# cslab-ntua/sparsex

Hardware: NVIDIA B200
Metric: csx_spmv_gflops (higher is better)
Workload: dtype f64

## Files before the change

### __graft_entry__.py

```python
import os
import subprocess
import sys

ROOT = os.path.dirname(os.path.abspath(__file__))
if ROOT not in sys.path:
    sys.path.insert(0, ROOT)


def build():
    csrc = os.path.join(ROOT, "sparsex_b200", "csrc")
    subprocess.check_call(["make", "-C", csrc, "-j4"])
    subprocess.check_call(["make", "-C", os.path.join(ROOT, "oracle"), "libcsx_oracle.so"])
    if os.path.isdir("/root/reference"):
        for script in ("build_ref.py", "build_refenc.py"):
            ref = os.path.join(ROOT, "oracle", script)
            if os.path.exists(ref):
                subprocess.check_call([sys.executable, ref])
    subprocess.check_call(["make", "-s", "-C", os.path.join(ROOT, "tests", "emul")], stderr=subprocess.DEVNULL)
    subprocess.check_call(["make", "-s", "-C", os.path.join(ROOT, "tests", "emul"), "-f", "trans.mk"], stderr=subprocess.DEVNULL)
    import sparsex_b200
    sparsex_b200.lib()
    if os.path.isdir("/root/reference/src/examples"):
        from tests.test_reference_examples import build_examples, build_test_program
        build_examples()
        build_test_program()


def smoke():
    import numpy as np
    import torch
    import sparsex_b200
    from oracle.pyoracle import OracleMatrix
    from tests.matrices import poisson2d

    assert torch.cuda.is_available(), "smoke() needs a GPU"
    rowptr, colind, values, n = poisson2d(96)
    rng = np.random.default_rng(0)
    x = rng.uniform(-1, 1, n)
    for opts in ({}, {"spx.preproc.xform": "none"}, {"spx.matrix.symmetric": "true"}):
        A = sparsex_b200.CsxMatrix.tune_csr(rowptr, colind, values, n, n, opts).upload(0)
        O = OracleMatrix.from_csr(rowptr, colind, values, n, n).tune(opts)
        for p in range(A.nparts):
            assert np.array_equal(A.partition(p).ctl, O.parts[p].ctl), "ctl mismatch vs oracle"
        dx = torch.from_numpy(x).cuda()
        dy = torch.empty(n, dtype=torch.float64, device="cuda")
        A.spmv(0.5, dx, dy)
        torch.cuda.synchronize()
        yref = O.spmv(0.5, x)
        err = np.abs(dy.cpu().numpy() - yref).max() / np.abs(yref).max()
        assert err < 1e-12, err
        print("smoke ok", opts, "rel err %.2e" % err)


if __name__ == "__main__":
    build()
    if len(sys.argv) > 1 and sys.argv[1] == "smoke":
        smoke()
```

### include/csx_b200.h

```cpp
#ifndef CSX_B200_H
#define CSX_B200_H

#include <stddef.h>
#include <stdint.h>

#ifdef __cplusplus
extern "C" {
#endif

typedef struct csxb_matrix csxb_matrix_t;

csxb_matrix_t *csxb_tune_csr(const int32_t *rowptr, const int32_t *colind, const double *values,
                             int64_t nrows, int64_t ncols, const char *options,
                             int part_lo, int part_hi, char *err, size_t errlen);
csxb_matrix_t *csxb_tune_mmf(const char *path, const char *options, int part_lo, int part_hi,
                             char *err, size_t errlen);
csxb_matrix_t *csxb_tune_csr_slab(const int32_t *rowptr, const int32_t *colind, const double *values,
                                  int64_t slab_rows, int64_t nrows_total, int64_t ncols, int64_t row_start,
                                  int part, const char *options, char *err, size_t errlen);
void csxb_destroy(csxb_matrix_t *m);

enum { CSXB_NROWS = 0, CSXB_NCOLS = 1, CSXB_NNZ = 2, CSXB_SYMMETRIC = 3, CSXB_NPARTS = 4,
       CSXB_NPARTS_TOTAL = 5, CSXB_PART_LO = 6, CSXB_FULL_COLIND = 7,
       CSXB_SYM_HALO_LO = 8, CSXB_SYM_HALO_HI = 9,
       CSXB_HOST_CAP = 10, CSXB_HOST_CALLS = 11,
       CSXB_DEVICE = 12  };
int64_t csxb_info(const csxb_matrix_t *m, int what);

enum { CSXB_P_NNZ = 0, CSXB_P_NROWS = 1, CSXB_P_NCOLS = 2, CSXB_P_ROW_START = 3, CSXB_P_CTL_SIZE = 4,
       CSXB_P_ROW_JUMPS = 5, CSXB_P_ID_MAP_LEN = 6, CSXB_P_MAP_LEN = 7, CSXB_P_DVALUES_LEN = 8,
       CSXB_P_ROWS_INFO_LEN = 9, CSXB_P_SAMPLING_UNDEFINED = 10,
       CSXB_P_COL_MIN = 11, CSXB_P_COL_MAX = 12  };
int64_t csxb_part_info(const csxb_matrix_t *m, int part, int what);
enum { CSXB_A_VALUES = 0, CSXB_A_CTL = 1, CSXB_A_ID_MAP = 2, CSXB_A_ROWS_INFO = 3, CSXB_A_DVALUES = 4,
       CSXB_A_MAP_CPUS = 5, CSXB_A_MAP_POS = 6 };
int csxb_part_copy(const csxb_matrix_t *m, int part, int what, void *dst);
const char *csxb_part_log(const csxb_matrix_t *m, int part);

int csxb_upload(csxb_matrix_t *m, int device, int free_host);
const char *csxb_last_error(void);
int csxb_layout_stats(csxb_matrix_t *m, int64_t *out, int max_owners);

enum { CSXB_B_VALUES = 0, CSXB_B_CTL = 1, CSXB_B_TABLES = 2, CSXB_B_X = 3, CSXB_B_Y = 4, CSXB_B_TOTAL = 5,
       CSXB_B_LAUNCHES = 6  };
int64_t csxb_traffic(const csxb_matrix_t *m, int what);

int csxb_spmv(csxb_matrix_t *m, double alpha, const double *d_x, double beta, double *d_y,
              int overwrite, void *stream);

int csxb_spmv_host(csxb_matrix_t *m, double alpha, const double *h_x, double beta, double *h_y,
                   int overwrite);

enum { CSXB_T_COL_LO = 0, CSXB_T_COL_HI = 1, CSXB_T_DEVICE_BYTES = 2, CSXB_T_ALG_BYTES = 3, CSXB_T_LAUNCHES = 4,
       CSXB_T_HEAVY_COLS = 5, CSXB_T_SEGMENTS = 6, CSXB_T_BUILD_US = 7 };
int csxb_transpose_prepare(csxb_matrix_t *m);
int csxb_spmv_t(csxb_matrix_t *m, double alpha, const double *d_x, double beta, double *d_y, int overwrite,
                void *stream);
int csxb_spmv_t_host(csxb_matrix_t *m, double alpha, const double *h_x, double beta, double *h_y, int overwrite);
int64_t csxb_transpose_info(const csxb_matrix_t *m, int what);
int csxb_decode_coords_t(const csxb_matrix_t *m, int32_t *rows, int32_t *cols);

int csxb_save(csxb_matrix_t *m, const char *path);
csxb_matrix_t *csxb_load(const char *path, char *err, size_t errlen);
int csxb_get_entry(csxb_matrix_t *m, int64_t row, int64_t col, double *value);
int csxb_set_entry(csxb_matrix_t *m, int64_t row, int64_t col, double value);

typedef struct csxb_group csxb_group_t;
csxb_group_t *csxb_group_create(csxb_matrix_t *whole, const int *devices, int ndev, int free_host, char *err, size_t errlen);
void csxb_group_destroy(csxb_group_t *g);
int csxb_group_size(const csxb_group_t *g);
csxb_matrix_t *csxb_group_member(csxb_group_t *g, int i);
int csxb_group_device(const csxb_group_t *g, int i);
int csxb_group_spmv(csxb_group_t *g, double alpha, const double *x, double beta, double *y, int overwrite);
int csxb_group_spmv_t(csxb_group_t *g, double alpha, const double *x, double beta, double *y, int overwrite);
int csxb_group_save(csxb_group_t *g, const char *path);
int csxb_group_get_entry(csxb_group_t *g, int64_t row, int64_t col, double *value);
int csxb_group_set_entry(csxb_group_t *g, int64_t row, int64_t col, double value);
int csxb_group_set_perm(csxb_group_t *g, const int32_t *perm, int64_t n);

int csxb_rcm_csr(const int32_t *rowptr, const int32_t *colind, int64_t nrows, int64_t ncols, int32_t *perm,
                 int64_t *bandwidth);
int csxb_rcm_edges(const int32_t *eu, const int32_t *ev, int64_t nedges, int64_t n, int64_t start, int32_t *perm,
                   int64_t *bandwidth);
int csxb_set_perm(csxb_matrix_t *m, const int32_t *perm, int64_t n);
int64_t csxb_get_perm(const csxb_matrix_t *m, int32_t *perm);
int csxb_permute_csr(const int32_t *rowptr, const int32_t *colind, const double *values, int64_t nrows,
                     const int32_t *perm, int32_t *out_rowptr, int32_t *out_colind, double *out_values);

int csxb_vec_axpby(double *d_out, const double *d_a, const double *d_b, double alpha, double beta, int64_t n, void *stream);
int csxb_vec_dot(const double *d_a, const double *d_b, int64_t n, double *result, void *stream);

typedef struct csxb_xchg csxb_xchg_t;
csxb_xchg_t *csxb_xchg_create(csxb_matrix_t *m, int rank, int world);
int csxb_xchg_handle(csxb_xchg_t *x, void *handle64);
int csxb_xchg_connect(csxb_xchg_t *x, const void *handles, const int64_t *row_lo, const int64_t *row_n,
                      const int64_t *win_lo, const int64_t *win_hi);
int csxb_xchg_connect_ptr(csxb_xchg_t *x, void *const *bases, const int64_t *row_lo, const int64_t *row_n,
                          const int64_t *win_lo, const int64_t *win_hi);
void *csxb_xchg_base(csxb_xchg_t *x);
double *csxb_xchg_vector(csxb_xchg_t *x, int which);
int csxb_xchg_spmv(csxb_xchg_t *x, double alpha, void *stream);
int64_t csxb_xchg_status(csxb_xchg_t *x, int what);
void csxb_xchg_destroy(csxb_xchg_t *x);

int csxb_decode_coords(const csxb_matrix_t *m, int part, int32_t *rows, int32_t *cols);

#ifdef __cplusplus
}
#endif
#endif
```

### sparsex_b200/csrc/engine.cu

```cuda
#include <cuda_runtime.h>

#include <chrono>
#include <memory>

#include <climits>
#include <cstdio>
#include <cstdlib>
#include <cstring>
#include <sstream>
#include <string>
#include <type_traits>
#include <vector>

#include "../../include/csx_b200.h"
#include "csx_host.hpp"
#include "gpu_layout.hpp"
#include "part_dev.cuh"
#include "stream_kernel.cuh"

#include "gather_kernel.cuh"

__device__ __forceinline__ unsigned long long ld_acquire_sys(const unsigned long long *p) {
  unsigned long long v;
  asm volatile("ld.acquire.sys.global.u64 %0, [%1];" : "=l"(v) : "l"(p) : "memory");
// ... 97 lines not shown
}
__global__ void csx_xchg_sync_kernel(const __grid_constant__ XchgDev X, int dbg) {
  const int lane = threadIdx.x;
  const unsigned long long k = *reinterpret_cast<const volatile unsigned long long *>(X.step);
  if (!(dbg & 2)) __threadfence_system();
  if (lane < X.nwait) st_release_sys(X.peer_flags[lane] + X.rank, k + 1);
  if (lane == 0) *reinterpret_cast<volatile unsigned long long *>(X.step) = k + 1;
  if (lane < X.nwait) {
    const unsigned long long *f = X.flags + X.wait_rank[lane];
    const long long t0 = clock64();
    while (ld_acquire_sys(f) < k + 1) {
      if (clock64() - t0 > 6000000000ll) { atomicExch(X.error, 1ull); break; }
    }
  }
}

struct DecodeGatherOp {
  int *rows, *cols;
  int myrow;
  __device__ __forceinline__ void add(uint32_t vi, int col) { rows[vi] = myrow; cols[vi] = col; }
};
__global__ void __launch_bounds__(CTA_THREADS) csx_decode_bt_kernel(const __grid_constant__ PartDev P, int *rows, int *cols) {
  const long long lrow = (long long)blockIdx.x * CTA_THREADS + threadIdx.x;
  if (lrow >= P.nrows) return;
  const long long g = P.row_start + lrow;
  for (int c = 0; c < P.nbt; c++) {
    const BtDev &T = P.bt[c];
    if (T.image) continue;
    const long long J = g / T.G;
    const int f = (int)(g - J * T.G) * T.sf;
    for (uint32_t e = T.ptr[J - T.j0]; e < T.ptr[J - T.j0 + 1]; e++) {
      const uint2 b = T.ent[e];
      if (b.y & BT_IMAGE) continue;
      for (int l = 0; l < T.nloop; l++) { rows[b.x + f + l * T.sl] = (int)g; cols[b.x + f + l * T.sl] = (int)b.y + l; }
    }
  }
}
__global__ void __launch_bounds__(CTA_THREADS) csx_decode_gather_kernel(const __grid_constant__ PartDev P, int *rows, int *cols) {
  const long long tile = blockIdx.x;
  const uint32_t b = __ldg(P.tile_xoff + tile), e = __ldg(P.tile_xoff + tile + 1);
  for (int k = 0; k < P.rpt; k++) {
    const long long lrow = (tile * P.rpt + k) * CTA_THREADS + threadIdx.x;
    if (lrow >= P.nrows) return;
    DecodeGatherOp op{rows, cols, (int)(P.row_start + lrow)};
    for (uint32_t j = b; j < e; j++) {
      const uint4 d = __ldg(P.xdesc + j);
      if (d.w & XD_TRANSPOSED) continue;
      gather_desc<false>(d, P.ktab, op.myrow, op);
    }
  }
}

__device__ __forceinline__ int sk_vectors(const SkIO &io, const double *&x, double *&y) {
  x = io.x; y = io.y;
  if (io.step) {
    const unsigned long long k = *reinterpret_cast<const volatile unsigned long long *>(io.step);
    x = io.vec[k & 1]; y = io.vec[(k & 1) ^ 1];
    return (int)((k & 1) ^ 1);
  }
  return 0;
}
template <int R, uint32_t KM, int BC, int BRC>
__global__ void __launch_bounds__(SK_WARPS * 32, 4) csx_stream_kernel(const __grid_constant__ PartDev P, const __grid_constant__ SkIO io,
                                                                     double alpha, double beta, int overwrite) {
  __shared__ double sacc[SK_WARPS][SK_WIN];
  __shared__ uint4 sid[64];
  const int lane = threadIdx.x & 31, warp = threadIdx.x >> 5;
  if (threadIdx.x < 64) {
    const IdEntry &ie = P.idtab[threadIdx.x];
    sid[threadIdx.x] = make_uint4(ie.kind_align, ie.delta, ie.sl, ie.recip);
  }
  __syncthreads();
  const uint32_t ch = P.sk_c0 + blockIdx.x * SK_WARPS + warp;
  if (ch >= P.sk_c1) return;
  const double *x; double *y;
  const int ypar = sk_vectors(io, x, y);
  sk_chunk<R, KM, BC, BRC, false>(P, ch, sacc[warp], sid, lane, x, y, alpha, beta, overwrite, nullptr, nullptr, &io, ypar);
}
__global__ void __launch_bounds__(SK_WARPS * 32) csx_stream_decode_kernel(const __grid_constant__ PartDev P, int *rows, int *cols) {
  __shared__ double sacc[SK_WARPS][SK_WIN];
  __shared__ uint4 sid[64];
  const int lane = threadIdx.x & 31, warp = threadIdx.x >> 5;
  if (threadIdx.x < 64) {
    const IdEntry &ie = P.idtab[threadIdx.x];
    sid[threadIdx.x] = make_uint4(ie.kind_align, ie.delta, ie.sl, ie.recip);
  }
  __syncthreads();
  const uint32_t ch = P.sk_c0 + blockIdx.x * SK_WARPS + warp;
  if (ch >= P.sk_c1) return;
  sk_chunk<8, SKM_ROWLOCAL | SKM_BROW | SKM_BCOL, 0, 0, true>(P, ch, sacc[warp], sid, lane, nullptr, nullptr, 0.0, 0.0, 1,
                                                               rows + P.val_base, cols + P.val_base);
}
__global__ void __launch_bounds__(256) csx_stream_fixup_kernel(const __grid_constant__ PartDev P, const __grid_constant__ SkIO io,
                                                                double alpha, double beta, int overwrite, long long clip_lo,
                                                                long long clip_hi) {
  const double *x; double *y;
  const int ypar = sk_vectors(io, x, y);
  const long long tid = (long long)blockIdx.x * blockDim.x + threadIdx.x, nth = (long long)gridDim.x * blockDim.x;
  for (long long i = P.sk_f0 + tid; i < P.sk_f1; i += nth) {
    double s = 0.0;
    for (uint32_t j = P.sk_fix_ptr[i]; j < P.sk_fix_ptr[i + 1]; j++) s += P.sk_scratch[P.sk_fix_idx[j]];
    const long long g = P.row_start + P.sk_fix_rows[i];
    const double v = y[g] + alpha * s;
    y[g] = v;
    sk_push(io, ypar, g, v);
  }
  for (uint32_t g = P.sk_g0 + blockIdx.x; g < P.sk_g1; g += gridDim.x) {
    const long long lo = max(P.sk_gaps[2 * g], clip_lo), hi = min(P.sk_gaps[2 * g + 1], clip_hi);
    for (long long r = lo + threadIdx.x; r < hi; r += blockDim.x) {
      double *yp = y + P.row_start + r;
      const double v = overwrite ? 0.0 : beta * *yp;
      *yp = v;
      sk_push(io, ypar, P.row_start + r, v);
    }
  }
}

__global__ void __launch_bounds__(256) csx_t_segment_kernel(const uint2 *__restrict__ ent, const uint32_t *__restrict__ seg,
                                                            uint32_t nseg, const double *__restrict__ values,
                                                            const double *__restrict__ x, double *__restrict__ scratch) {
  const uint32_t s = blockIdx.x * 8 + (threadIdx.x >> 5);
  if (s >= nseg) return;
  t_segment_warp(ent, seg, values, x, scratch, s, (int)(threadIdx.x & 31));
}

static thread_local std::string g_last_error;
static int fail(const std::string &m) { g_last_error = m; return -1; }
#define CUDA_TRY(call)                                                                         \
  do {                                                                                         \
    cudaError_t e_ = (call);                                                                   \
    if (e_ != cudaSuccess)                                                                     \
      return fail(std::string(#call) + ": " + cudaGetErrorString(e_));                         \
  } while (0)

struct TransState {
  TransLayout lay;
  PartDev P;
  const uint2 *hent = nullptr;
  const uint32_t *hseg = nullptr;
  int64_t dev_bytes = 0, alg_bytes = 0, launches = 0, build_us = 0;
  double *d_x = nullptr, *d_y = nullptr;
};

struct csxb_matrix {
  CsxMatrix host;
  DeviceLayout layout;
  bool uploaded = false;
  int device = -1;
  std::vector<void *> allocs;
  std::vector<PartDev> pdev;
  double *d_values = nullptr;
  double *d_x = nullptr, *d_y = nullptr;
  int64_t covered_rows_end = 0;
  int64_t sym_halo_lo = 0, sym_halo_hi = 0;
  struct Slab {
    int part; int64_t tile0, tile1;
    uint32_t chunk0, chunk1, f0, f1, g0, g1;
    int64_t x_lo, x_hi, row_lo, row_hi, y_lo, y_hi, yup_hi;
  };
  std::vector<Slab> slabs;
  std::vector<cudaEvent_t> slab_ev;
  cudaStream_t s_h2d = nullptr, s_run = nullptr, s_d2h = nullptr;
  int host_calls = 0;
  double host_tune_s[2] = {0.0, 0.0};
  size_t host_cap = 0;
  int64_t bytes[7] = {0, 0, 0, 0, 0, 0, 0};
  std::vector<std::string> logs;
  std::vector<RowIndex> row_index;
  std::unique_ptr<TransState> trans;
  ~csxb_matrix() {
    if (!allocs.empty() || d_x || d_y || s_h2d) {
      int cur = -1;
      cudaGetDevice(&cur);
      if (device >= 0) cudaSetDevice(device);
      for (void *p : allocs) cudaFree(p);
      if (d_x) cudaFree(d_x);
      if (d_y) cudaFree(d_y);
      for (cudaEvent_t e : slab_ev) cudaEventDestroy(e);
      if (s_h2d) { cudaStreamDestroy(s_h2d); cudaStreamDestroy(s_run); cudaStreamDestroy(s_d2h); }
      if (cur >= 0) cudaSetDevice(cur);
    }
  }
};

static std::string parse_options(const char *options, TuneOptions &o) {
  if (!options) return "";
  std::stringstream ss(options);
  std::string kv;
  while (std::getline(ss, kv, ';')) {
    if (kv.empty()) continue;
    size_t eq = kv.find('=');
    if (eq == std::string::npos) return "malformed option \"" + kv + "\"";
    std::string e = o.set(kv.substr(0, eq), kv.substr(eq + 1));
    if (!e.empty()) return e;
  }
  return "";
}
static void put_err(char *err, size_t n, const std::string &m) {
  g_last_error = m;
  if (err && n) { strncpy(err, m.c_str(), n - 1); err[n - 1] = 0; }
}

csxb_matrix_t *csxb_tune_coo_internal(const CooHost &coo, const char *options, int part_lo, int part_hi, char *err, size_t errlen) {
  TuneOptions o;
  std::string e = parse_options(options, o);
  if (!e.empty()) { put_err(err, errlen, e); return nullptr; }
  if (part_hi < 0) { part_lo = 0; part_hi = o.nr_threads; }
  csxb_matrix *m = new csxb_matrix;
  e = tune_coo(coo, o, part_lo, part_hi, m->host);
  if (!e.empty()) { put_err(err, errlen, e); delete m; return nullptr; }
  return m;
}

extern "C" {

csxb_matrix_t *csxb_tune_csr(const int32_t *rowptr, const int32_t *colind, const double *values, int64_t nrows,
                             int64_t ncols, const char *options, int part_lo, int part_hi, char *err, size_t errlen) {
  TuneOptions o;
  std::string e = parse_options(options, o);
  if (e.empty() && (!rowptr || !colind || !values || nrows < 0 || ncols < 0)) e = "invalid CSR arguments";
  if (e.empty() && rowptr[0] != 0) e = "CSR arrays must be zero-based";
  if (!e.empty()) { put_err(err, errlen, e); return nullptr; }
  if (part_hi < 0) { part_lo = 0; part_hi = o.nr_threads; }
  csxb_matrix *m = new csxb_matrix;
  CsrView v{rowptr, colind, values, nrows, ncols};
  e = tune_csr(v, o, part_lo, part_hi, m->host);
  if (!e.empty()) { put_err(err, errlen, e); delete m; return nullptr; }
  return m;
}

csxb_matrix_t *csxb_tune_csr_slab(const int32_t *rowptr, const int32_t *colind, const double *values, int64_t slab_rows,
                                  int64_t nrows_total, int64_t ncols, int64_t row_start, int part, const char *options, char *err,
                                  size_t errlen) {
  TuneOptions o;
  std::string e = parse_options(options, o);
  if (e.empty() && (!rowptr || !colind || !values || slab_rows < 0 || ncols < 0)) e = "invalid CSR arguments";
  if (e.empty() && rowptr[0] != 0) e = "CSR arrays must be zero-based";
  if (!e.empty()) { put_err(err, errlen, e); return nullptr; }
  csxb_matrix *m = new csxb_matrix;
  CsrView v{rowptr, colind, values, slab_rows, ncols};
  e = tune_csr_slab(v, nrows_total, row_start, part, o, m->host);
  if (!e.empty()) { put_err(err, errlen, e); delete m; return nullptr; }
  return m;
}

csxb_matrix_t *csxb_tune_mmf(const char *path, const char *options, int part_lo, int part_hi, char *err, size_t errlen) {
  TuneOptions o;
  std::string e = parse_options(options, o);
  CooHost coo;
  if (e.empty()) e = path ? read_mmf(path, coo) : "invalid file name";
  if (!e.empty()) { put_err(err, errlen, e); return nullptr; }
  if (part_hi < 0) { part_lo = 0; part_hi = o.nr_threads; }
  csxb_matrix *m = new csxb_matrix;
  e = tune_coo(coo, o, part_lo, part_hi, m->host);
  if (!e.empty()) { put_err(err, errlen, e); delete m; return nullptr; }
  return m;
}

void csxb_destroy(csxb_matrix_t *m) { delete m; }

int64_t csxb_info(const csxb_matrix_t *m, int what) {
  switch (what) {
    case CSXB_NROWS: return m->host.nrows;
    case CSXB_NCOLS: return m->host.ncols;
    case CSXB_NNZ: return m->host.nnz;
    case CSXB_SYMMETRIC: return m->host.symmetric;
    case CSXB_NPARTS: return (int64_t)m->host.parts.size();
    case CSXB_NPARTS_TOTAL: return m->host.nparts_total;
    case CSXB_PART_LO: return m->host.part_lo;
    case CSXB_FULL_COLIND: return m->host.full_colind;
    case CSXB_SYM_HALO_LO: return m->sym_halo_lo;
    case CSXB_SYM_HALO_HI: return m->sym_halo_hi;
    case CSXB_HOST_CAP: return (int64_t)m->host_cap;
    case CSXB_HOST_CALLS: return m->host_calls;
    case CSXB_DEVICE: return m->uploaded ? m->device : -1;
  }
  return -1;
}

int64_t csxb_part_info(const csxb_matrix_t *m, int part, int what) {
  if (part < 0 || (size_t)part >= m->host.parts.size()) return -1;
  const CsxPartition &p = m->host.parts[part];
  switch (what) {
    case CSXB_P_NNZ: return p.nnz;
    case CSXB_P_NROWS: return p.nrows;
    case CSXB_P_NCOLS: return p.ncols;
    case CSXB_P_ROW_START: return p.row_start;
    case CSXB_P_CTL_SIZE: return (int64_t)p.ctl.size();
    case CSXB_P_ROW_JUMPS: return p.row_jumps;
    case CSXB_P_ID_MAP_LEN: return (int64_t)p.id_map.size();
    case CSXB_P_MAP_LEN: return (int64_t)p.map_cpus.size();
    case CSXB_P_DVALUES_LEN: return (int64_t)p.dvalues.size();
    case CSXB_P_ROWS_INFO_LEN: return (int64_t)p.rows_info.size();
    case CSXB_P_SAMPLING_UNDEFINED: return p.sampling_undefined;
    case CSXB_P_COL_MIN: return p.col_min;
    case CSXB_P_COL_MAX: return p.col_max;
  }
  return -1;
}

int csxb_part_copy(const csxb_matrix_t *m, int part, int what, void *dst) {
  if (part < 0 || (size_t)part >= m->host.parts.size() || !dst) return fail("invalid argument");
  const CsxPartition &p = m->host.parts[part];
  switch (what) {
    case CSXB_A_VALUES:
      if (p.values.size() != (size_t)p.nnz) return fail("host values were released at upload");
      memcpy(dst, p.values.data(), p.values.size() * 8); break;
    case CSXB_A_CTL: memcpy(dst, p.ctl.data(), p.ctl.size()); break;
    case CSXB_A_ID_MAP: { int64_t *d = (int64_t *)dst; for (size_t i = 0; i < p.id_map.size(); i++) d[i] = p.id_map[i]; break; }
    case CSXB_A_ROWS_INFO: {
      struct R { int64_t rowptr, valptr; int32_t span, pad; } *d = (R *)dst;
      for (size_t i = 0; i < p.rows_info.size(); i++) d[i] = R{p.rows_info[i].rowptr, p.rows_info[i].valptr, p.rows_info[i].span, 0};
      break;
    }
    case CSXB_A_DVALUES: memcpy(dst, p.dvalues.data(), p.dvalues.size() * 8); break;
    case CSXB_A_MAP_CPUS: memcpy(dst, p.map_cpus.data(), p.map_cpus.size() * 4); break;
    case CSXB_A_MAP_POS: memcpy(dst, p.map_pos.data(), p.map_pos.size() * 4); break;
    default: return fail("unknown array");
  }
  return 0;
}

const char *csxb_part_log(const csxb_matrix_t *m, int part) {
  if (part < 0 || (size_t)part >= m->host.parts.size()) return "";
  return m->host.parts[part].encoding_log.c_str();
}

const char *csxb_last_error(void) { return g_last_error.c_str(); }

int csxb_layout_stats(csxb_matrix_t *m, int64_t *out, int max_owners) {
  CsxMatrix &H = m->host;
  std::vector<int64_t> saved;
  for (auto &p : H.parts) { saved.push_back(p.nrows); if (H.symmetric) p.nrows = (int64_t)p.dvalues.size(); }
  DeviceLayout L;
  std::string e = build_layout(H, L);
  for (size_t i = 0; i < H.parts.size(); i++) H.parts[i].nrows = saved[i];
  if (!e.empty()) return fail("layout: " + e);
  for (size_t q = 0; q < L.parts.size() && (int)q < max_owners; q++) {
    const PartLayout &pl = L.parts[q];
    int64_t *o = out + 12 * q;
    o[0] = pl.nrows; o[1] = pl.ntiles; o[2] = (int64_t)pl.xdesc.size(); o[3] = (int64_t)pl.sk_chunks.size();
    o[4] = (int64_t)pl.sk_uoffs.size(); o[5] = (int64_t)pl.sk_fix_idx.size(); o[6] = (int64_t)pl.sk_gaps.size();
    for (int t = 0; t < 5; t++) o[7 + t] = 0;
    for (const BlockTable &T : pl.bt) {
      int t = T.G == 1 && T.nloop == 1 ? 4 : (T.image ? (T.sl == 1 ? 3 : 1) : (T.sl == 1 ? 0 : 2));
      o[7 + t] += (int64_t)T.ent.size();
    }
  }
  return (int)L.parts.size();
}

}

template <class T>
static int dev_copy(csxb_matrix *m, const T *src, size_t n, T **dst, size_t extra_zero = 0) {
  void *p = nullptr;
  size_t bytes = (n + extra_zero) * sizeof(T);
  CUDA_TRY(cudaMalloc(&p, bytes ? bytes : 16));
  m->allocs.push_back(p);
  if (n) CUDA_TRY(cudaMemcpy(p, src, n * sizeof(T), cudaMemcpyHostToDevice));
  if (extra_zero) CUDA_TRY(cudaMemset((char *)p + n * sizeof(T), 0, extra_zero * sizeof(T)));
  *dst = (T *)p;
  return 0;
}

static void build_slabs(csxb_matrix *m) {
  m->slabs.clear();
  int64_t SLAB_ROWS = m->host.slab_rows;
  if (SLAB_ROWS <= 0) {
    int64_t total_rows = 0;
    for (const PartLayout &pl : m->layout.parts) if (pl.ntiles) total_rows += pl.nrows;
    SLAB_ROWS = int64_t(1) << 19;
    while (SLAB_ROWS < (int64_t(1) << 21) && SLAB_ROWS * 16 <= total_rows) SLAB_ROWS *= 2;
  }
  for (size_t i = 0; i < m->layout.parts.size(); i++) {
    const PartLayout &pl = m->layout.parts[i];
    if (!pl.ntiles) continue;
    const int64_t tr = pl.tile_rows();
    const int64_t tiles_per = std::max<int64_t>(1, SLAB_ROWS / tr);
    uint32_t c = 0, f = 0;
    const uint32_t nc = (uint32_t)pl.sk_chunks.size(), nf = (uint32_t)pl.sk_fix_rows.size(), ng = (uint32_t)pl.sk_gaps.size();
    int64_t xmax = -1, yup = 0;
    for (int64_t t0 = 0; t0 < pl.ntiles; t0 += tiles_per) {
      csxb_matrix::Slab sl;
      sl.part = (int)i; sl.tile0 = t0; sl.tile1 = std::min(pl.ntiles, t0 + tiles_per);
      const int64_t r0 = t0 * tr, r1 = std::min(pl.nrows, sl.tile1 * tr);
      sl.row_lo = pl.row_start + r0; sl.row_hi = pl.row_start + r1;
      for (int64_t t = sl.tile0; t < sl.tile1; t++)
        if (pl.tile_cmax[t] >= pl.tile_cmin[t]) xmax = std::max<int64_t>(xmax, pl.tile_cmax[t]);
      sl.chunk0 = c;
      while (c < nc && pl.sk_first_row[c] < r1) {
        xmax = std::max<int64_t>(xmax, pl.sk_cmax[c]);
        yup = std::max<int64_t>(yup, (int64_t)pl.sk_last_row[c] + 1);
        c++;
      }
      sl.chunk1 = c;
      sl.f0 = f;
      while (f < nf && pl.sk_fix_rows[f] < r1) f++;
      sl.f1 = f;
      sl.g0 = 0;
      while (sl.g0 < ng && pl.sk_gaps[sl.g0].hi <= r0) sl.g0++;
      sl.g1 = sl.g0;
      while (sl.g1 < ng && pl.sk_gaps[sl.g1].lo < r1) sl.g1++;
      sl.x_lo = 0; sl.x_hi = xmax + 1;
      sl.y_lo = sl.row_lo; sl.y_hi = sl.row_hi;
      sl.yup_hi = pl.row_start + std::max(r1, std::min(yup, pl.nrows));
      m->slabs.push_back(sl);
    }
  }
  int64_t lo = INT64_MAX;
  for (size_t i = 0; i < m->layout.parts.size(); i++)
    for (int32_t v : m->layout.parts[i].tile_cmin) if (v != INT32_MAX) lo = std::min<int64_t>(lo, v);
  if (lo == INT64_MAX) lo = 0;
  int64_t run = lo;
  for (auto &sl : m->slabs) { sl.x_lo = lo; run = std::max(run, sl.x_hi); sl.x_hi = run; }
}

extern "C" {

int csxb_upload(csxb_matrix_t *m, int device, int free_host) {
  if (m->uploaded) return fail("matrix already uploaded");
  CsxMatrix &H = m->host;
  std::vector<int64_t> saved_nrows;
  for (auto &p : H.parts) { saved_nrows.push_back(p.nrows); if (H.symmetric) p.nrows = (int64_t)p.dvalues.size(); }
  std::string e = build_layout(H, m->layout);
  for (size_t i = 0; i < H.parts.size(); i++) H.parts[i].nrows = saved_nrows[i];
  if (!e.empty()) return fail("layout: " + e);
  int ndev = 0;
  CUDA_TRY(cudaGetDeviceCount(&ndev));
  if (device < 0 || device >= ndev) return fail("invalid device");
  CUDA_TRY(cudaSetDevice(device));
  m->device = device;
  DeviceLayout &L = m->layout;
  void *dv = nullptr, *dc = nullptr;
  CUDA_TRY(cudaMalloc(&dv, std::max<uint64_t>(L.total_values, 1) * 8));
  m->allocs.push_back(dv);
  CUDA_TRY(cudaMalloc(&dc, std::max<uint64_t>(L.total_ctl, 16)));
  m->allocs.push_back(dc);
  CUDA_TRY(cudaMemset(dc, 0, std::max<uint64_t>(L.total_ctl, 16)));
  m->d_values = (double *)dv;
  KindEntry *d_ktab = nullptr;
  if (dev_copy(m, L.ktab.data(), L.ktab.size(), &d_ktab)) return -1;
  int64_t tables = (int64_t)L.ktab.size() * 8, nnz_stored = 0, ctl_bytes = 0, rows_owned = 0, launches = 0;
  m->pdev.resize(L.parts.size());
  for (size_t i = 0; i < L.parts.size(); i++) {
    PartLayout &pl = L.parts[i];
    static CsxPartition no_part;
    CsxPartition &hp = pl.is_halo ? no_part : H.parts[i];
    PartDev &P = m->pdev[i];
    memset(&P, 0, sizeof(P));
    if (hp.nnz) CUDA_TRY(cudaMemcpy(m->d_values + pl.val_base, hp.values.data(), (size_t)hp.nnz * 8, cudaMemcpyHostToDevice));
    if (!hp.ctl.empty()) CUDA_TRY(cudaMemcpy((uint8_t *)dc + pl.ctl_base, hp.ctl.data(), hp.ctl.size(), cudaMemcpyHostToDevice));
    P.ctl = (const uint8_t *)dc + pl.ctl_base;
    P.values = m->d_values;
    P.ctl_end = (const uint8_t *)dc + std::max<uint64_t>(L.total_ctl, 16);
    P.values_end = m->d_values + std::max<uint64_t>(L.total_values, 1);
    uint32_t *tx = nullptr; XDesc *xd = nullptr;
    if (dev_copy(m, pl.tile_xoff.data(), pl.tile_xoff.size(), &tx)) return -1;
    if (dev_copy(m, pl.xdesc.data(), pl.xdesc.size(), &xd)) return -1;
    for (size_t t = 0; t < pl.bt.size(); t++) {
      const BlockTable &T = pl.bt[t];
      uint32_t *bp = nullptr; BlockImage *bi = nullptr;
      if (dev_copy(m, T.ptr.data(), T.ptr.size(), &bp)) return -1;
      if (dev_copy(m, T.ent.data(), T.ent.size(), &bi)) return -1;
      static_assert(sizeof(BlockImage) == sizeof(uint2), "block table entry layout");
      P.bt[t] = BtDev{bp, (const uint2 *)bi, (long long)T.j0, T.G, T.nloop, T.sf, T.sl, T.image, (uint32_t)((0x100000000ull + T.G - 1) / T.G)};
      tables += (int64_t)T.ptr.size() * 4 + (int64_t)T.ent.size() * 8;
    }
    P.nbt = (int)pl.bt.size();
    if (!pl.sk_chunks.empty()) {
      SkEntry *se = nullptr; uint16_t *so = nullptr; int32_t *fr = nullptr; uint32_t *fp = nullptr, *fi = nullptr; long long *gp = nullptr;
      if (dev_copy(m, pl.sk_chunks.data(), pl.sk_chunks.size(), &se)) return -1;
      if (dev_copy(m, pl.sk_uoffs.data(), pl.sk_uoffs.size(), &so)) return -1;
      if (dev_copy(m, pl.sk_fix_rows.data(), pl.sk_fix_rows.size(), &fr)) return -1;
      if (dev_copy(m, pl.sk_fix_ptr.data(), pl.sk_fix_ptr.size(), &fp)) return -1;
      if (dev_copy(m, pl.sk_fix_idx.data(), pl.sk_fix_idx.size(), &fi)) return -1;
      static_assert(sizeof(SkGap) == 16, "gap layout");
      if (dev_copy(m, reinterpret_cast<const long long *>(pl.sk_gaps.data()), pl.sk_gaps.size() * 2, &gp)) return -1;
      void *sc = nullptr;
      CUDA_TRY(cudaMalloc(&sc, std::max<size_t>(pl.sk_scratch, 2) * 8));
      m->allocs.push_back(sc);
      P.sk_chunks = (const uint4 *)se; P.sk_uoffs = so; P.sk_scratch = (double *)sc;
      P.sk_fix_rows = fr; P.sk_fix_ptr = fp; P.sk_fix_idx = fi; P.sk_gaps = gp;
      P.sk_c0 = 0; P.sk_c1 = (uint32_t)pl.sk_chunks.size();
      P.sk_f0 = 0; P.sk_f1 = (uint32_t)pl.sk_fix_rows.size();
      P.sk_g0 = 0; P.sk_g1 = (uint32_t)pl.sk_gaps.size();
      tables += (int64_t)pl.sk_chunks.size() * (int64_t)sizeof(SkEntry) + (int64_t)pl.sk_uoffs.size() * 2 +
                (int64_t)pl.sk_fix_rows.size() * 8 + (int64_t)pl.sk_fix_idx.size() * 4 + (int64_t)pl.sk_scratch * 16;
    }
    P.tile_xoff = tx; P.xdesc = (const uint4 *)xd; P.ktab = d_ktab;
    if (H.symmetric && !pl.is_halo) {
      double *dd = nullptr;
      if (dev_copy(m, hp.dvalues.data(), hp.dvalues.size(), &dd)) return -1;
      P.dvalues = dd;
      tables += (int64_t)hp.dvalues.size() * 8;
    }
    P.nrows = pl.nrows; P.row_start = pl.row_start; P.val_base = (uint32_t)pl.val_base;
    P.full_colind = L.full_colind;
    P.rpt = pl.rpt;
    memcpy(P.idtab, pl.idtab, sizeof(P.idtab));
    nnz_stored += hp.nnz; rows_owned += pl.nrows;
    if (!pl.sk_chunks.empty()) ctl_bytes += (int64_t)hp.ctl.size();
    tables += (int64_t)pl.tile_xoff.size() * 4 + (int64_t)pl.xdesc.size() * 16;
    if (pl.nrows) {
      if (!pl.sk_chunks.empty())
        launches += 1 + ((pl.sk_fix_rows.empty() && pl.sk_gaps.empty()) ? 0 : 1) + ((pl.xdesc.empty() && pl.bt.empty() && !H.symmetric) ? 0 : 1);
      else launches += 1;
    }
    if (!pl.is_halo) m->covered_rows_end = std::max<int64_t>(m->covered_rows_end, pl.row_start + pl.nrows);
    if (free_host && !pl.is_halo) std::vector<double>().swap(hp.values);
  }
  m->sym_halo_lo = L.halo_lo; m->sym_halo_hi = L.halo_hi;
  if (!H.symmetric) build_slabs(m);
  m->bytes[CSXB_B_VALUES] = nnz_stored * 8;
  m->bytes[CSXB_B_CTL] = ctl_bytes;
  m->bytes[CSXB_B_TABLES] = tables;
  int64_t cmin = H.ncols, cmax = -1;
  for (auto &p : H.parts) if (p.col_max >= p.col_min) { cmin = std::min(cmin, p.col_min); cmax = std::max(cmax, p.col_max); }
  int64_t xcols = (int)H.parts.size() == H.nparts_total ? H.ncols : std::max<int64_t>(0, cmax - cmin + 1);
  if (H.symmetric) xcols = H.ncols;
  m->bytes[CSXB_B_X] = xcols * 8;
  m->bytes[CSXB_B_Y] = rows_owned * 8;
  m->bytes[CSXB_B_TOTAL] = nnz_stored * 8 + ctl_bytes + tables + xcols * 8 + rows_owned * 8;
  m->bytes[CSXB_B_LAUNCHES] = launches;
  m->uploaded = true;
  return 0;
}

int64_t csxb_traffic(const csxb_matrix_t *m, int what) {
  if (what < 0 || what > CSXB_B_LAUNCHES) return -1;
  return m->bytes[what];
}

}

static bool gather_cache_policies(const PartLayout &pl) {
  static const int forced = getenv("CSXB_GATHER_POLICY") ? atoi(getenv("CSXB_GATHER_POLICY")) : -1;
  return forced >= 0 ? forced != 0 : pl.nnz >= 12 * pl.nrows;
}

template <int RPT> struct BtMinB { static constexpr int value = RPT == 1 ? 6 : 5; };
static thread_local size_t t_gather_dyn = 0;
constexpr size_t HOST_CAP_SMEM = 40000;
template <class K>
static size_t gather_dyn(K kernel) {
  if (t_gather_dyn > 48 * 1024) cudaFuncSetAttribute(kernel, cudaFuncAttributeMaxDynamicSharedMemorySize, (int)t_gather_dyn);
  return t_gather_dyn;
}
template <bool SYM, int RPT, int KSET, class XP>
static void launch_gather_k(const PartDev &P, const PartLayout &pl, unsigned nt, const double *x, double *y, double alpha,
                            double beta, int overwrite, cudaStream_t s, const XP &X) {
  dim3 grid(nt), block(CTA_THREADS);
  if (!pl.bt.empty()) {
    if (!pl.xdesc.empty()) {
      auto k = csx_spmv_kernel<true, SYM, RPT, KSET_ANY, BtMinB<RPT>::value, 0, XP, true>;
      k<<<grid, block, gather_dyn(k), s>>>(P, x, y, alpha, beta, overwrite, X);
    } else {
      auto k = csx_spmv_kernel<false, SYM, RPT, KSET_ANY, BtMinB<RPT>::value, 0, XP, true>;
      k<<<grid, block, gather_dyn(k), s>>>(P, x, y, alpha, beta, overwrite, X);
    }
    return;
  }
  constexpr int MB = SYM ? 4 : 8;
  const size_t dyn = 0;
  if (!pl.xdesc.empty()) csx_spmv_kernel<true, SYM, RPT, KSET, MB, 0, XP><<<grid, block, dyn, s>>>(P, x, y, alpha, beta, overwrite, X);
  else csx_spmv_kernel<false, SYM, RPT, KSET_ANY, MB, 0, XP><<<grid, block, dyn, s>>>(P, x, y, alpha, beta, overwrite, X);
}
template <bool SYM, class XP>
static void launch_gather(const PartDev &P0, const PartLayout &pl, int64_t t0, int64_t t1, const double *x, double *y,
                          double alpha, double beta, int overwrite, cudaStream_t s, const XP &X) {
  if (t1 <= t0) return;
  PartDev P = P0;
  P.tile0 = (uint32_t)t0;
  const unsigned nt = (unsigned)(t1 - t0);
  const bool diag1 = !SYM && pl.xd_diag1_only && !pl.xdesc.empty() && pl.bt.empty();
  if (pl.rpt == 4) {
    if (diag1) {
      dim3 grid(nt), block(CTA_THREADS);
      if (gather_cache_policies(pl)) {
        auto k = csx_spmv_kernel<true, false, 4, KSET_DIAG1, 8, 3, XP>;
        k<<<grid, block, gather_dyn(k), s>>>(P, x, y, alpha, beta, overwrite, X);
      } else {
        auto k = csx_spmv_kernel<true, false, 4, KSET_DIAG1, 8, 1, XP>;
        k<<<grid, block, gather_dyn(k), s>>>(P, x, y, alpha, beta, overwrite, X);
      }
    }
    else launch_gather_k<SYM, 4, KSET_ANY>(P, pl, nt, x, y, alpha, beta, overwrite, s, X);
  } else {
    if (diag1) launch_gather_k<SYM, 1, SYM ? KSET_ANY : KSET_DIAG1>(P, pl, nt, x, y, alpha, beta, overwrite, s, X);
    else launch_gather_k<SYM, 1, KSET_ANY>(P, pl, nt, x, y, alpha, beta, overwrite, s, X);
  }
}
static void launch_gather_xe(const PartDev &P0, const PartLayout &pl, const double *x, double *y, double alpha, int ypar,
                             cudaStream_t s, const XchgDev &X) {
  if (!pl.ntiles) return;
  PartDev P = P0;
  P.tile0 = 0;
  dim3 grid((unsigned)(X.nb + (X.edge_hi_begin - X.edge_lo_end))), block(CTA_THREADS);
  const bool xd = !pl.xdesc.empty(), diag1 = pl.xd_diag1_only && xd && pl.bt.empty();
  if (!pl.bt.empty()) {
    if (pl.rpt == 4) {
      if (xd) csx_spmv_xe_kernel<true, 4, KSET_ANY, BtMinB<4>::value, 0, true><<<grid, block, 0, s>>>(P, x, y, alpha, ypar, X);
      else csx_spmv_xe_kernel<false, 4, KSET_ANY, BtMinB<4>::value, 0, true><<<grid, block, 0, s>>>(P, x, y, alpha, ypar, X);
    } else {
      if (xd) csx_spmv_xe_kernel<true, 1, KSET_ANY, BtMinB<1>::value, 0, true><<<grid, block, 0, s>>>(P, x, y, alpha, ypar, X);
      else csx_spmv_xe_kernel<false, 1, KSET_ANY, BtMinB<1>::value, 0, true><<<grid, block, 0, s>>>(P, x, y, alpha, ypar, X);
    }
    return;
  }
  const size_t dyn = 0;
  if (pl.rpt == 4) {
    if (diag1 && gather_cache_policies(pl)) csx_spmv_xe_kernel<true, 4, KSET_DIAG1, 8, 3><<<grid, block, dyn, s>>>(P, x, y, alpha, ypar, X);
    else if (diag1) csx_spmv_xe_kernel<true, 4, KSET_DIAG1, 8, 1><<<grid, block, dyn, s>>>(P, x, y, alpha, ypar, X);
    else if (xd) csx_spmv_xe_kernel<true, 4, KSET_ANY><<<grid, block, dyn, s>>>(P, x, y, alpha, ypar, X);
    else csx_spmv_xe_kernel<false, 4, KSET_ANY><<<grid, block, dyn, s>>>(P, x, y, alpha, ypar, X);
  } else {
    if (diag1) csx_spmv_xe_kernel<true, 1, KSET_DIAG1><<<grid, block, dyn, s>>>(P, x, y, alpha, ypar, X);
    else if (xd) csx_spmv_xe_kernel<true, 1, KSET_ANY><<<grid, block, dyn, s>>>(P, x, y, alpha, ypar, X);
    else csx_spmv_xe_kernel<false, 1, KSET_ANY><<<grid, block, dyn, s>>>(P, x, y, alpha, ypar, X);
  }
}
static int launch_stream(const PartDev &P0, const PartLayout &pl, uint32_t c0, uint32_t c1, const SkIO &io, double alpha, double beta,
                         int overwrite, cudaStream_t s) {
  if (c1 <= c0) return 0;
  PartDev P = P0;
  P.sk_c0 = c0; P.sk_c1 = c1;
  const unsigned grid = (unsigned)((c1 - c0 + SK_WARPS - 1) / SK_WARPS);
#define SK_TRY(RR, KK, BCC, BRR)                                                                                         \
  if (sk_instance_serves(RR, (KK), BCC, BRR, pl.sk_kmask, pl.sk_rows, pl.sk_bc, pl.sk_brc)) {                            \
    csx_stream_kernel<RR, (KK), BCC, BRR><<<grid, SK_WARPS * 32, 0, s>>>(P, io, alpha, beta, overwrite);                 \
    return 0;                                                                                                            \
  }
  SK_INSTANCES(SK_TRY)
#undef SK_TRY
  return -1;
}
static void launch_fixup(const PartDev &P0, uint32_t f0, uint32_t f1, uint32_t g0, uint32_t g1, int64_t r0, int64_t r1, const SkIO &io,
                         double alpha, double beta, int overwrite, cudaStream_t s) {
  if (f1 <= f0 && g1 <= g0) return;
  PartDev P = P0;
  P.sk_f0 = f0; P.sk_f1 = f1; P.sk_g0 = g0; P.sk_g1 = g1;
  const int64_t ctas = std::max<int64_t>(((int64_t)(f1 - f0) + 255) / 256, (int64_t)(g1 - g0));
  const unsigned grid = (unsigned)std::min<int64_t>(148 * 8, ctas);
  csx_stream_fixup_kernel<<<grid, 256, 0, s>>>(P, io, alpha, beta, overwrite, (long long)r0, (long long)r1);
}
template <bool SYM, class XP>
static int run_partition(const PartDev &P, const PartLayout &pl, const SkIO &io, double alpha, double beta, int overwrite,
                         cudaStream_t s, const XP &X) {
  if (pl.sk_chunks.empty()) {
    launch_gather<SYM>(P, pl, 0, pl.ntiles, io.x, io.y, alpha, beta, overwrite, s, X);
    return 0;
  }
  if (launch_stream(P, pl, 0, (uint32_t)pl.sk_chunks.size(), io, alpha, beta, overwrite, s)) return -1;
  launch_fixup(P, 0, (uint32_t)pl.sk_fix_rows.size(), 0, (uint32_t)pl.sk_gaps.size(), 0, pl.nrows, io, alpha, beta, overwrite, s);
  if (SYM || !pl.xdesc.empty() || !pl.bt.empty()) launch_gather<SYM>(P, pl, 0, pl.ntiles, io.x, io.y, alpha, 1.0, 0, s, X);
  return 0;
}

extern "C" {

static int on_matrix_device(const csxb_matrix *m) {
  int cur = -1;
  if (cudaGetDevice(&cur) != cudaSuccess) return fail("cudaGetDevice failed");
  if (cur != m->device && cudaSetDevice(m->device) != cudaSuccess) return fail("cudaSetDevice failed");
  return 0;
}

int csxb_spmv(csxb_matrix_t *m, double alpha, const double *d_x, double beta, double *d_y, int overwrite, void *stream) {
  if (!m->uploaded) return fail("matrix not uploaded (csxb_upload)");
  if (on_matrix_device(m)) return -1;
  cudaStream_t s = (cudaStream_t)stream;
  const bool sym = m->host.symmetric;
  SkIO io;
  io.x = d_x; io.y = d_y; io.step = nullptr; io.vec[0] = io.vec[1] = nullptr; io.npush = 0;
  for (size_t i = 0; i < m->pdev.size(); i++) {
    const PartLayout &pl = m->layout.parts[i];
    int rc;
    if (pl.is_halo) { launch_gather<true>(m->pdev[i], pl, 0, pl.ntiles, d_x, d_y, alpha, 0.0, 1, s, NoXchg()); rc = 0; }
    else if (sym) rc = run_partition<true>(m->pdev[i], pl, io, alpha, beta, overwrite, s, NoXchg());
    else rc = run_partition<false>(m->pdev[i], pl, io, alpha, beta, overwrite, s, NoXchg());
    if (rc) return fail("no stream kernel for the partition's pattern set");
  }
  if (overwrite && m->host.part_lo + (int)m->host.parts.size() == m->host.nparts_total && m->covered_rows_end < m->host.nrows)
    CUDA_TRY(cudaMemsetAsync(d_y + m->covered_rows_end, 0, (size_t)(m->host.nrows - m->covered_rows_end) * 8, s));
  CUDA_TRY(cudaGetLastError());
  return 0;
}

int csxb_spmv_host(csxb_matrix_t *m, double alpha, const double *h_x, double beta, double *h_y, int overwrite) {
  if (!m->uploaded) return fail("matrix not uploaded (csxb_upload)");
  int cur = -1;
  CUDA_TRY(cudaGetDevice(&cur));
  if (cur != m->device) CUDA_TRY(cudaSetDevice(m->device));
  size_t nx = (size_t)std::max<int64_t>(m->host.ncols, 1), ny = (size_t)std::max<int64_t>(m->host.nrows, 1);
  if (!m->d_x) CUDA_TRY(cudaMalloc((void **)&m->d_x, nx * 8));
  if (!m->d_y) CUDA_TRY(cudaMalloc((void **)&m->d_y, ny * 8));
  if (!m->s_h2d) {
    CUDA_TRY(cudaStreamCreateWithFlags(&m->s_h2d, cudaStreamNonBlocking));
    CUDA_TRY(cudaStreamCreateWithFlags(&m->s_run, cudaStreamNonBlocking));
    CUDA_TRY(cudaStreamCreateWithFlags(&m->s_d2h, cudaStreamNonBlocking));
  }
  const bool last_local = m->host.part_lo + (int)m->host.parts.size() == m->host.nparts_total;
  if (m->slabs.empty()) {
    CUDA_TRY(cudaMemcpyAsync(m->d_x, h_x, (size_t)m->host.ncols * 8, cudaMemcpyHostToDevice, m->s_run));
    if (!overwrite) CUDA_TRY(cudaMemcpyAsync(m->d_y, h_y, (size_t)m->host.nrows * 8, cudaMemcpyHostToDevice, m->s_run));
    if (csxb_spmv(m, alpha, m->d_x, beta, m->d_y, overwrite, m->s_run)) return -1;
    int64_t lo = m->layout.parts.empty() ? 0 : m->layout.parts.front().row_start;
    int64_t hi = last_local ? m->host.nrows : m->covered_rows_end;
    if (!overwrite) { lo = 0; hi = m->host.nrows; }
    if (hi > lo) CUDA_TRY(cudaMemcpyAsync(h_y + lo, m->d_y + lo, (size_t)(hi - lo) * 8, cudaMemcpyDeviceToHost, m->s_run));
    CUDA_TRY(cudaStreamSynchronize(m->s_run));
  } else {
    if (m->slab_ev.size() < 2 * m->slabs.size()) {
      size_t old = m->slab_ev.size();
      m->slab_ev.resize(2 * m->slabs.size());
      for (size_t i = old; i < m->slab_ev.size(); i++) CUDA_TRY(cudaEventCreateWithFlags(&m->slab_ev[i], cudaEventDisableTiming));
    }
    static const bool trace = getenv("CSXB_HOST_TRACE") != nullptr;
    std::vector<cudaEvent_t> tev;
    if (trace) {
      tev.resize(3 * m->slabs.size() + 1);
      for (auto &e : tev) CUDA_TRY(cudaEventCreate(&e));
      CUDA_TRY(cudaEventRecord(tev.back(), m->s_h2d));
    }
    auto issue_download = [&](size_t k) -> int {
      const csxb_matrix::Slab &sl = m->slabs[k];
      if (sl.y_hi > sl.y_lo) {
        CUDA_TRY(cudaStreamWaitEvent(m->s_d2h, m->slab_ev[2 * k + 1], 0));
        CUDA_TRY(cudaMemcpyAsync(h_y + sl.y_lo, m->d_y + sl.y_lo, (size_t)(sl.y_hi - sl.y_lo) * 8, cudaMemcpyDeviceToHost, m->s_d2h));
      }
      if (trace) CUDA_TRY(cudaEventRecord(tev[3 * k + 2], m->s_d2h));
      return 0;
    };
    const auto call_t0 = std::chrono::steady_clock::now();
    const int tune_call = m->host_calls < 5 ? m->host_calls : -1;
    {
      const char *v = getenv("CSXB_HOST_SMEM");
      if (v) t_gather_dyn = (size_t)atol(v);
      else if (tune_call > 0) t_gather_dyn = (tune_call % 2 == 0) ? HOST_CAP_SMEM : 0;
      else t_gather_dyn = m->host_cap;
    }
    struct DynReset { ~DynReset() { t_gather_dyn = 0; } } dyn_reset;
    int64_t x_done = m->slabs.front().x_lo;
    int64_t y_up = 0;
    for (size_t k = 0; k < m->slabs.size(); k++) {
      const csxb_matrix::Slab &sl = m->slabs[k];
      const PartLayout &pl = m->layout.parts[sl.part];
      if (sl.x_hi > x_done) {
        CUDA_TRY(cudaMemcpyAsync(m->d_x + x_done, h_x + x_done, (size_t)(sl.x_hi - x_done) * 8, cudaMemcpyHostToDevice, m->s_h2d));
        x_done = sl.x_hi;
      }
      if (!overwrite) {
        if (k == 0 || m->slabs[k - 1].part != sl.part) y_up = sl.row_lo;
        if (sl.yup_hi > y_up) {
          CUDA_TRY(cudaMemcpyAsync(m->d_y + y_up, h_y + y_up, (size_t)(sl.yup_hi - y_up) * 8, cudaMemcpyHostToDevice, m->s_h2d));
          y_up = sl.yup_hi;
        }
      }
      CUDA_TRY(cudaEventRecord(m->slab_ev[2 * k], m->s_h2d));
      if (trace) CUDA_TRY(cudaEventRecord(tev[3 * k], m->s_h2d));
      CUDA_TRY(cudaStreamWaitEvent(m->s_run, m->slab_ev[2 * k], 0));
      if (pl.sk_chunks.empty()) {
        launch_gather<false>(m->pdev[sl.part], pl, sl.tile0, sl.tile1, m->d_x, m->d_y, alpha, beta, overwrite, m->s_run, NoXchg());
      } else {
        SkIO io;
        io.x = m->d_x; io.y = m->d_y; io.step = nullptr; io.vec[0] = io.vec[1] = nullptr; io.npush = 0;
        if (launch_stream(m->pdev[sl.part], pl, sl.chunk0, sl.chunk1, io, alpha, beta, overwrite, m->s_run)) return fail("no stream kernel for the partition's pattern set");
        launch_fixup(m->pdev[sl.part], sl.f0, sl.f1, sl.g0, sl.g1, sl.row_lo - pl.row_start, sl.row_hi - pl.row_start, io, alpha, beta, overwrite, m->s_run);
        if (!pl.xdesc.empty() || !pl.bt.empty()) launch_gather<false>(m->pdev[sl.part], pl, sl.tile0, sl.tile1, m->d_x, m->d_y, alpha, 1.0, 0, m->s_run, NoXchg());
      }
      CUDA_TRY(cudaEventRecord(m->slab_ev[2 * k + 1], m->s_run));
      if (trace) CUDA_TRY(cudaEventRecord(tev[3 * k + 1], m->s_run));
      if (issue_download(k)) return -1;
    }
    if (trace) {
      CUDA_TRY(cudaStreamSynchronize(m->s_run));
      CUDA_TRY(cudaStreamSynchronize(m->s_d2h));
      for (size_t k = 0; k < m->slabs.size(); k++) {
        float a = 0, b = 0, c = 0;
        cudaEventElapsedTime(&a, tev.back(), tev[3 * k]);
        cudaEventElapsedTime(&b, tev.back(), tev[3 * k + 1]);
        cudaEventElapsedTime(&c, tev.back(), tev[3 * k + 2]);
        const csxb_matrix::Slab &sl = m->slabs[k];
        fprintf(stderr, "[host-trace] slab %3zu rows [%lld, %lld) x to %lld: up %.3f ms, run %.3f ms, down %.3f ms\n", k,
                (long long)sl.row_lo, (long long)sl.row_hi, (long long)sl.x_hi, a, b, c);
      }
      for (auto &e : tev) cudaEventDestroy(e);
    }
    CUDA_TRY(cudaGetLastError());
    CUDA_TRY(cudaStreamSynchronize(m->s_run));
    CUDA_TRY(cudaStreamSynchronize(m->s_d2h));
    if (overwrite && last_local && m->covered_rows_end < m->host.nrows)
      for (int64_t r = m->covered_rows_end; r < m->host.nrows; r++) h_y[r] = 0.0;
    if (tune_call >= 0) {
      const double dt = std::chrono::duration<double>(std::chrono::steady_clock::now() - call_t0).count();
      if (tune_call > 0) { double &best = m->host_tune_s[tune_call % 2]; best = best == 0.0 ? dt : std::min(best, dt); }
      if (tune_call == 4) m->host_cap = m->host_tune_s[0] < m->host_tune_s[1] ? HOST_CAP_SMEM : 0;
      m->host_calls++;
    }
  }
  if (cur != m->device && cur >= 0) CUDA_TRY(cudaSetDevice(cur));
  return 0;
}

struct DeviceGuard {
  int d = -1;
  DeviceGuard() { cudaGetDevice(&d); }
  ~DeviceGuard() { if (d >= 0) cudaSetDevice(d); }
};

int csxb_transpose_prepare(csxb_matrix_t *m) {
  if (!m) return fail("invalid argument");
  if (m->host.symmetric || m->trans) return 0;
  if (!m->uploaded) return fail("matrix not uploaded (csxb_upload)");
  DeviceGuard guard;
  const auto t0 = std::chrono::steady_clock::now();
  std::unique_ptr<TransState> T(new TransState);
  std::string e = build_transpose_layout(m->host, m->layout, T->lay);
  if (!e.empty()) return fail("transposed layout: " + e);
  CUDA_TRY(cudaSetDevice(m->device));
  const TransLayout &TL = T->lay;
  const PartLayout &pl = TL.part;
  PartDev &P = T->P;
  memset(&P, 0, sizeof(P));
  KindEntry *kt = nullptr; uint32_t *tx = nullptr; XDesc *xd = nullptr;
  if (dev_copy(m, TL.ktab.data(), TL.ktab.size(), &kt) || dev_copy(m, pl.tile_xoff.data(), pl.tile_xoff.size(), &tx) ||
      dev_copy(m, pl.xdesc.data(), pl.xdesc.size(), &xd))
    return -1;
  int64_t tables = (int64_t)TL.ktab.size() * 8 + (int64_t)pl.tile_xoff.size() * 4 + (int64_t)pl.xdesc.size() * 16;
  for (size_t t = 0; t < pl.bt.size(); t++) {
    const BlockTable &B = pl.bt[t];
    uint32_t *bp = nullptr; BlockImage *bi = nullptr;
    if (dev_copy(m, B.ptr.data(), B.ptr.size(), &bp) || dev_copy(m, B.ent.data(), B.ent.size(), &bi)) return -1;
    P.bt[t] = BtDev{bp, (const uint2 *)bi, (long long)B.j0, B.G, B.nloop, B.sf, B.sl, B.image, (uint32_t)((0x100000000ull + B.G - 1) / B.G)};
    tables += (int64_t)B.ptr.size() * 4 + (int64_t)B.ent.size() * 8;
  }
  P.nbt = (int)pl.bt.size();
  int launches = pl.nrows ? 1 : 0;
  if (!pl.sk_fix_rows.empty()) {
    BlockImage *he = nullptr; uint32_t *hs = nullptr, *fp = nullptr, *fi = nullptr; int32_t *fr = nullptr;
    if (dev_copy(m, TL.hent.data(), TL.hent.size(), &he) || dev_copy(m, TL.hseg.data(), TL.hseg.size(), &hs) ||
        dev_copy(m, pl.sk_fix_rows.data(), pl.sk_fix_rows.size(), &fr) || dev_copy(m, pl.sk_fix_ptr.data(), pl.sk_fix_ptr.size(), &fp) ||
        dev_copy(m, pl.sk_fix_idx.data(), pl.sk_fix_idx.size(), &fi))
      return -1;
    void *sc = nullptr;
    CUDA_TRY(cudaMalloc(&sc, std::max<size_t>(pl.sk_scratch, 2) * 8));
    m->allocs.push_back(sc);
    T->hent = (const uint2 *)he; T->hseg = hs;
    P.sk_scratch = (double *)sc; P.sk_fix_rows = fr; P.sk_fix_ptr = fp; P.sk_fix_idx = fi;
    P.sk_f0 = 0; P.sk_f1 = (uint32_t)pl.sk_fix_rows.size();
    tables += (int64_t)TL.hent.size() * 8 + (int64_t)TL.hseg.size() * 4 + (int64_t)pl.sk_fix_rows.size() * 8 +
              (int64_t)pl.sk_fix_idx.size() * 4 + (int64_t)pl.sk_scratch * 16;
    launches += 2;
  }
  P.values = m->d_values; P.tile_xoff = tx; P.xdesc = (const uint4 *)xd; P.ktab = kt;
  P.nrows = pl.nrows; P.row_start = pl.row_start; P.rpt = pl.rpt;
  P.values_end = m->d_values + std::max<uint64_t>(m->layout.total_values, 1);
  T->dev_bytes = (int64_t)TL.ktab.size() * 8 + (int64_t)pl.tile_xoff.size() * 4 + (int64_t)pl.xdesc.size() * 16 +
                 (int64_t)TL.hent.size() * 8 + (int64_t)TL.hseg.size() * 4 + (int64_t)pl.sk_fix_rows.size() * 4 +
                 (int64_t)pl.sk_fix_ptr.size() * 4 + (int64_t)pl.sk_fix_idx.size() * 4 + (int64_t)pl.sk_scratch * 8;
  for (const BlockTable &B : pl.bt) T->dev_bytes += (int64_t)B.ptr.size() * 4 + (int64_t)B.ent.size() * 8;
  int64_t xrows = 0;
  for (const CsxPartition &p : m->host.parts) xrows += p.nrows;
  T->alg_bytes = m->bytes[CSXB_B_VALUES] + tables + 8 * xrows + 8 * pl.nrows;
  T->launches = launches;
  T->build_us = (int64_t)(std::chrono::duration<double>(std::chrono::steady_clock::now() - t0).count() * 1e6);
  m->trans = std::move(T);
  return 0;
}

int csxb_spmv_t(csxb_matrix_t *m, double alpha, const double *d_x, double beta, double *d_y, int overwrite, void *stream) {
  if (m->host.symmetric) return csxb_spmv(m, alpha, d_x, beta, d_y, overwrite, stream);
  if (!m->trans && csxb_transpose_prepare(m)) return -1;
  if (on_matrix_device(m)) return -1;
  cudaStream_t s = (cudaStream_t)stream;
  const TransState &T = *m->trans;
  const PartLayout &pl = T.lay.part;
  if (!pl.nrows) return 0;
  const uint32_t nseg = (uint32_t)(T.lay.hseg.size() - 1);
  if (nseg) csx_t_segment_kernel<<<(nseg + 7) / 8, 256, 0, s>>>(T.hent, T.hseg, nseg, m->d_values, d_x, T.P.sk_scratch);
  if (T.lay.images) launch_gather<true>(T.P, pl, 0, pl.ntiles, d_x, d_y, alpha, beta, overwrite, s, NoXchg());
  else launch_gather<false>(T.P, pl, 0, pl.ntiles, d_x, d_y, alpha, beta, overwrite, s, NoXchg());
  if (nseg) {
    SkIO io;
    io.x = d_x; io.y = d_y; io.step = nullptr; io.vec[0] = io.vec[1] = nullptr; io.npush = 0;
    launch_fixup(T.P, 0, (uint32_t)pl.sk_fix_rows.size(), 0, 0, 0, pl.nrows, io, alpha, beta, overwrite, s);
  }
  CUDA_TRY(cudaGetLastError());
  return 0;
}

int csxb_spmv_t_host(csxb_matrix_t *m, double alpha, const double *h_x, double beta, double *h_y, int overwrite) {
  if (m->host.symmetric) return csxb_spmv_host(m, alpha, h_x, beta, h_y, overwrite);
  if (!m->trans && csxb_transpose_prepare(m)) return -1;
  DeviceGuard guard;
  CUDA_TRY(cudaSetDevice(m->device));
  TransState &T = *m->trans;
  const int64_t nr = m->host.nrows, lo = T.lay.part.row_start, n = T.lay.part.nrows;
  if (!T.d_x) {
    CUDA_TRY(cudaMalloc((void **)&T.d_x, (size_t)std::max<int64_t>(nr, 1) * 8));
    m->allocs.push_back(T.d_x);
    CUDA_TRY(cudaMalloc((void **)&T.d_y, (size_t)std::max<int64_t>(m->host.ncols, 1) * 8));
    m->allocs.push_back(T.d_y);
  }
  if (!m->s_run) {
    CUDA_TRY(cudaStreamCreateWithFlags(&m->s_h2d, cudaStreamNonBlocking));
    CUDA_TRY(cudaStreamCreateWithFlags(&m->s_run, cudaStreamNonBlocking));
    CUDA_TRY(cudaStreamCreateWithFlags(&m->s_d2h, cudaStreamNonBlocking));
  }
  CUDA_TRY(cudaMemcpyAsync(T.d_x, h_x, (size_t)nr * 8, cudaMemcpyDefault, m->s_run));
  if (!overwrite && n > 0) CUDA_TRY(cudaMemcpyAsync(T.d_y + lo, h_y + lo, (size_t)n * 8, cudaMemcpyDefault, m->s_run));
  if (csxb_spmv_t(m, alpha, T.d_x, beta, T.d_y, overwrite, m->s_run)) { cudaStreamSynchronize(m->s_run); return -1; }
  if (n > 0) CUDA_TRY(cudaMemcpyAsync(h_y + lo, T.d_y + lo, (size_t)n * 8, cudaMemcpyDefault, m->s_run));
  CUDA_TRY(cudaStreamSynchronize(m->s_run));
  return 0;
}

int64_t csxb_transpose_info(const csxb_matrix_t *m, int what) {
  if (!m || !m->trans) return -1;
  const TransState &T = *m->trans;
  switch (what) {
    case CSXB_T_COL_LO: return T.lay.part.row_start;
    case CSXB_T_COL_HI: return T.lay.part.row_start + T.lay.part.nrows;
    case CSXB_T_DEVICE_BYTES: return T.dev_bytes;
    case CSXB_T_ALG_BYTES: return T.alg_bytes;
    case CSXB_T_LAUNCHES: return T.launches;
    case CSXB_T_HEAVY_COLS: return T.lay.heavy_cols;
    case CSXB_T_SEGMENTS: return (int64_t)T.lay.hseg.size() - 1;
    case CSXB_T_BUILD_US: return T.build_us;
  }
  return -1;
}

int csxb_decode_coords_t(const csxb_matrix_t *mc, int32_t *rows, int32_t *cols) {
  csxb_matrix *m = const_cast<csxb_matrix *>(mc);
  if (!m || !rows || !cols) return fail("invalid argument");
  if (m->host.symmetric) return fail("CSX-Sym has no transposed tables (A^T = A)");
  TransLayout local;
  const TransLayout *TL = m->trans ? &m->trans->lay : nullptr;
  DeviceLayout fl;
  if (!TL) {
    std::string e = build_layout(m->host, fl);
    if (e.empty()) e = build_transpose_layout(m->host, fl, local);
    if (!e.empty()) return fail("transposed layout: " + e);
    TL = &local;
  }
  int64_t n = 0;
  for (const CsxPartition &p : m->host.parts) n += p.nnz;
  std::fill(rows, rows + n, -1);
  std::fill(cols, cols + n, -1);
  decode_transpose_coords(*TL, rows, cols);
  return 0;
}

struct csxb_xchg {
  csxb_matrix *m = nullptr;
  int rank = 0, world = 1;
  void *base = nullptr;
  size_t n = 0;
  std::vector<void *> peer_base;
  XchgDev dev;
  bool connected = false;
  int64_t tail_lo = 0, tail_hi = 0;
  int parity = 0;
  int64_t issued = 0;
};
static size_t xchg_vec_bytes(size_t n) { return ((n * 8 + 255) / 256) * 256; }
static void xchg_choose_mode(csxb_xchg *h, int64_t own_lo, int64_t own_hi);

csxb_xchg_t *csxb_xchg_create(csxb_matrix_t *m, int rank, int world) {
  if (!m || !m->uploaded) { fail("matrix not uploaded (csxb_upload)"); return nullptr; }
  if (m->host.symmetric) { fail("the peer-memory exchange covers non-symmetric CSX (CSX-Sym: SymHaloReduce)"); return nullptr; }
  if (world < 1 || rank < 0 || rank >= world || world - 1 > XCHG_MAX_PEERS) { fail("invalid rank / world size"); return nullptr; }
  if (m->host.nrows != m->host.ncols) { fail("repeated SpMV with exchange needs a square matrix"); return nullptr; }
  if (cudaSetDevice(m->device) != cudaSuccess) { fail("cudaSetDevice failed"); return nullptr; }
  csxb_xchg *h = new csxb_xchg;
  h->m = m; h->rank = rank; h->world = world; h->n = (size_t)m->host.nrows;
  const size_t vb = xchg_vec_bytes(h->n), total = 2 * vb + 4096;
  if (cudaMalloc(&h->base, total) != cudaSuccess || cudaMemset(h->base, 0, total) != cudaSuccess) {
    fail("device allocation for the exchange vectors failed");
    delete h;
    return nullptr;
  }
  memset(&h->dev, 0, sizeof(h->dev));
  h->dev.vec[0] = (double *)h->base;
  h->dev.vec[1] = (double *)((char *)h->base + vb);
  unsigned long long *ctrl = (unsigned long long *)((char *)h->base + 2 * vb);
  h->dev.step = ctrl; h->dev.error = ctrl + 1; h->dev.started = ctrl + 2; h->dev.bdone = ctrl + 3; h->dev.flags = ctrl + 16;
  h->dev.rank = rank;
  if (world == 1) {
    xchg_choose_mode(h, 0, (int64_t)h->n);
    h->connected = true;
    if (m->host.part_lo + (int)m->host.parts.size() == m->host.nparts_total) { h->tail_lo = m->covered_rows_end; h->tail_hi = (int64_t)h->n; }
  }
  return h;
}

int csxb_xchg_handle(csxb_xchg_t *h, void *handle64) {
  static_assert(sizeof(cudaIpcMemHandle_t) == 64, "IPC handle size");
  cudaIpcMemHandle_t ih;
  CUDA_TRY(cudaSetDevice(h->m->device));
  CUDA_TRY(cudaIpcGetMemHandle(&ih, h->base));
  memcpy(handle64, &ih, 64);
  return 0;
}

static void xchg_choose_mode(csxb_xchg *h, int64_t own_lo, int64_t own_hi) {
  XchgDev &D = h->dev;
// ... 52 lines not shown
  h->connected = true;
  return 0;
}

int csxb_xchg_connect(csxb_xchg_t *h, const void *handles, const int64_t *row_lo, const int64_t *row_n,
                      const int64_t *win_lo, const int64_t *win_hi) {
  if (h->connected) return fail("exchange already connected");
  CUDA_TRY(cudaSetDevice(h->m->device));
  h->peer_base.assign(h->world, nullptr);
  for (int q = 0; q < h->world; q++) {
    if (q == h->rank) continue;
    cudaIpcMemHandle_t ih;
    memcpy(&ih, (const char *)handles + (size_t)q * 64, 64);
    CUDA_TRY(cudaIpcOpenMemHandle(&h->peer_base[q], ih, cudaIpcMemLazyEnablePeerAccess));
  }
  std::vector<void *> bases = h->peer_base;
  bases[h->rank] = h->base;
  return xchg_plan(h, bases, row_lo, row_n, win_lo, win_hi);
}

int csxb_xchg_connect_ptr(csxb_xchg_t *h, void *const *bases, const int64_t *row_lo, const int64_t *row_n,
                          const int64_t *win_lo, const int64_t *win_hi) {
  if (h->connected) return fail("exchange already connected");
  std::vector<void *> b(bases, bases + h->world);
  return xchg_plan(h, b, row_lo, row_n, win_lo, win_hi);
}

void *csxb_xchg_base(csxb_xchg_t *h) { return h->base; }

double *csxb_xchg_vector(csxb_xchg_t *h, int which) { return h->dev.vec[which & 1]; }

int csxb_xchg_spmv(csxb_xchg_t *h, double alpha, void *stream) {
  if (!h->connected) return fail("exchange not connected (csxb_xchg_connect)");
  csxb_matrix *m = h->m;
  if (on_matrix_device(m)) return -1;
  cudaStream_t s = (cudaStream_t)stream;
  static const int dbg = getenv("CSXB_XCHG_DEBUG") ? atoi(getenv("CSXB_XCHG_DEBUG")) : 0;
  XchgDev X = h->dev;
  const bool copy_push = (dbg & 4) != 0;
  SkIO io;
  io.x = nullptr; io.y = nullptr; io.step = h->dev.step; io.vec[0] = h->dev.vec[0]; io.vec[1] = h->dev.vec[1];
  for (size_t i = 0; i < m->pdev.size(); i++) {
    const PartLayout &pl = m->layout.parts[i];
    if (X.mode == 1) { launch_gather_xe(m->pdev[i], pl, X.vec[h->parity], X.vec[h->parity ^ 1], alpha, h->parity ^ 1, s, X); continue; }
    const bool gather_last = pl.sk_chunks.empty() || !pl.xdesc.empty() || !pl.bt.empty();
    XchgDev Xp = X;
    io.npush = 0;
    if (copy_push) Xp.npush = 0;
    else if (!gather_last) {
      Xp.npush = 0;
      io.npush = X.npush;
      for (int p = 0; p < X.npush; p++) {
        io.push_lo[p] = X.push_lo[p]; io.push_hi[p] = X.push_hi[p];
        io.push_vec[p][0] = X.push_vec[p][0]; io.push_vec[p][1] = X.push_vec[p][1];
      }
    }
    if (run_partition<false>(m->pdev[i], pl, io, alpha, 0.0, 1, s, Xp)) return fail("no stream kernel for the partition's pattern set");
  }
  if (copy_push && h->dev.npush) csx_xchg_push_kernel<<<148 * 8, 256, 0, s>>>(h->dev);
  if (h->tail_hi > h->tail_lo)
    csx_xchg_zero_tail_kernel<<<(unsigned)std::min<int64_t>(148, (h->tail_hi - h->tail_lo + 255) / 256), 256, 0, s>>>(h->dev, h->tail_lo, h->tail_hi, h->dev.mode == 1 ? (h->parity ^ 1) : -1);
  if (!(dbg & 1) && h->dev.mode == 0) csx_xchg_sync_kernel<<<1, 32, 0, s>>>(h->dev, dbg);
  CUDA_TRY(cudaGetLastError());
  h->parity ^= 1;
  h->issued++;
  return 0;
}

int64_t csxb_xchg_status(csxb_xchg_t *h, int what) {
  unsigned long long v[2] = {0, 0};
  if (cudaSetDevice(h->m->device) != cudaSuccess) return -1;
  if (cudaMemcpy(v, h->dev.step, 16, cudaMemcpyDeviceToHost) != cudaSuccess) return -1;
  if (what == 0 && h->dev.mode == 1) { cudaDeviceSynchronize(); return h->issued; }
  if (what == 2) return h->dev.mode;
  if (what == 3) return h->dev.nb;
  return what == 0 ? (int64_t)v[0] : (int64_t)v[1];
}

void csxb_xchg_destroy(csxb_xchg_t *h) {
  if (!h) return;
  cudaSetDevice(h->m->device);
  cudaDeviceSynchronize();
  for (int q = 0; q < (int)h->peer_base.size(); q++)
    if (q != h->rank && h->peer_base[q]) cudaIpcCloseMemHandle(h->peer_base[q]);
  if (h->base) cudaFree(h->base);
  delete h;
}

__global__ void __launch_bounds__(256) csx_vec_axpby_kernel(double *__restrict__ out, const double *a, const double *b, double alpha,
                                                            double beta, long long n) {
  const long long stride = (long long)gridDim.x * blockDim.x;
  for (long long i = (long long)blockIdx.x * blockDim.x + threadIdx.x; i < n; i += stride) {
    const double bv = b ? b[i] : 0.0;
    out[i] = alpha * a[i] + beta * bv;
  }
}
__global__ void __launch_bounds__(256) csx_vec_dot_kernel(const double *__restrict__ a, const double *__restrict__ b, long long n,
                                                          double *__restrict__ partial) {
  __shared__ double warp_part[8];
  double s = 0.0;
  const long long stride = (long long)gridDim.x * blockDim.x;
  for (long long i = (long long)blockIdx.x * blockDim.x + threadIdx.x; i < n; i += stride) s = fma(a[i], b[i], s);
  s = warp_sum(s);
  if ((threadIdx.x & 31) == 0) warp_part[threadIdx.x >> 5] = s;
  __syncthreads();
  if (threadIdx.x == 0) {
    double t = 0.0;
    for (int w = 0; w < 8; w++) t += warp_part[w];
    partial[blockIdx.x] = t;
  }
}

int csxb_vec_axpby(double *d_out, const double *d_a, const double *d_b, double alpha, double beta, int64_t n, void *stream) {
  if (n <= 0) return 0;
  const unsigned grid = (unsigned)std::min<int64_t>((n + 255) / 256, 148 * 8);
  csx_vec_axpby_kernel<<<grid, 256, 0, (cudaStream_t)stream>>>(d_out, d_a, d_b, alpha, beta, (long long)n);
  CUDA_TRY(cudaGetLastError());
  return 0;
}

int csxb_vec_dot(const double *d_a, const double *d_b, int64_t n, double *result, void *stream) {
  *result = 0.0;
  if (n <= 0) return 0;
  const unsigned grid = (unsigned)std::min<int64_t>((n + 255) / 256, 148 * 4);
  static thread_local double *d_part[64] = {nullptr};
  static thread_local double *h_part[64] = {nullptr};
  int dev = 0;
  CUDA_TRY(cudaGetDevice(&dev));
  if (dev < 0 || dev >= 64) return fail("device index out of range");
  if (!d_part[dev]) {
    CUDA_TRY(cudaMalloc((void **)&d_part[dev], 148 * 4 * sizeof(double)));
    CUDA_TRY(cudaMallocHost((void **)&h_part[dev], 148 * 4 * sizeof(double)));
  }
  double *d_partial = d_part[dev], *h_partial = h_part[dev];
  cudaStream_t s = (cudaStream_t)stream;
  csx_vec_dot_kernel<<<grid, 256, 0, s>>>(d_a, d_b, (long long)n, d_partial);
  CUDA_TRY(cudaMemcpyAsync(h_partial, d_partial, grid * sizeof(double), cudaMemcpyDeviceToHost, s));
  CUDA_TRY(cudaStreamSynchronize(s));
  double t = 0.0;
  for (unsigned i = 0; i < grid; i++) t += h_partial[i];
  *result = t;
  return 0;
}

int csxb_save(csxb_matrix_t *m, const char *path) {
  if (!m || !path) return fail("invalid argument");
  CsxMatrix &H = m->host;
  for (size_t i = 0; i < H.parts.size(); i++) {
    CsxPartition &p = H.parts[i];
    if ((int64_t)p.values.size() == p.nnz) continue;
    if (!m->uploaded) return fail("partition values are neither on the host nor on a device");
    CUDA_TRY(cudaSetDevice(m->device));
    p.values.resize((size_t)p.nnz);
    CUDA_TRY(cudaMemcpy(p.values.data(), m->d_values + m->layout.parts[i].val_base, (size_t)p.nnz * 8, cudaMemcpyDeviceToHost));
  }
  std::string e = save_matrix(H, path);
  return e.empty() ? 0 : fail(e);
}

csxb_matrix_t *csxb_load(const char *path, char *err, size_t errlen) {
  if (!path) { put_err(err, errlen, "invalid file name"); return nullptr; }
  csxb_matrix *m = new csxb_matrix;
  std::string e;
  try { e = load_matrix(path, m->host); } catch (std::exception &ex) { e = std::string("cannot load the container: ") + ex.what(); }
  if (!e.empty()) { put_err(err, errlen, e); delete m; return nullptr; }
  return m;
}

int csxb_set_perm(csxb_matrix_t *m, const int32_t *perm, int64_t n) {
  if (!m || n < 0 || (n && (!perm || n != m->host.nrows))) return fail("invalid permutation");
  m->host.permutation.assign(perm, perm + n);
  return 0;
}
int64_t csxb_get_perm(const csxb_matrix_t *m, int32_t *perm) {
  if (!m) return -1;
  if (perm) std::copy(m->host.permutation.begin(), m->host.permutation.end(), perm);
  return (int64_t)m->host.permutation.size();
}

static int locate_entry(csxb_matrix *m, int64_t row, int64_t col, size_t &part, int64_t &idx, bool &diag) {
  CsxMatrix &H = m->host;
  if (row < 0 || row >= H.nrows || col < 0 || col >= H.ncols) return fail("index out of bounds");
  diag = false;
  if (H.symmetric) {
    if (col > row) std::swap(row, col);
    diag = row == col;
  }
  if (m->row_index.size() != H.parts.size()) m->row_index.assign(H.parts.size(), RowIndex());
  for (size_t i = 0; i < H.parts.size(); i++) {
    CsxPartition &p = H.parts[i];
    const int64_t owned = H.symmetric ? (int64_t)p.dvalues.size() : p.nrows;
    if (row < p.row_start || row >= p.row_start + owned) continue;
    part = i;
    if (diag) { idx = row - p.row_start; return 0; }
    RowIndex &ri = m->row_index[i];
    if (ri.ctl_off.empty()) {
      std::string e = build_row_index(p, H.full_colind, ri);
      if (!e.empty()) return fail(e);
    }
    idx = find_entry(p, H.full_colind, ri, row - p.row_start, col);
    return idx < 0 ? 1 : 0;
  }
  return 1;
}

int csxb_get_entry(csxb_matrix_t *m, int64_t row, int64_t col, double *value) {
  size_t part; int64_t idx; bool diag;
  const int rc = locate_entry(m, row, col, part, idx, diag);
  if (rc) return rc;
  CsxPartition &p = m->host.parts[part];
  if (diag) { *value = p.dvalues[(size_t)idx]; return 0; }
  if ((int64_t)p.values.size() == p.nnz) { *value = p.values[(size_t)idx]; return 0; }
  if (!m->uploaded) return fail("partition values are neither on the host nor on a device");
  CUDA_TRY(cudaSetDevice(m->device));
  CUDA_TRY(cudaMemcpy(value, m->d_values + m->layout.parts[part].val_base + idx, 8, cudaMemcpyDeviceToHost));
  return 0;
}

int csxb_set_entry(csxb_matrix_t *m, int64_t row, int64_t col, double value) {
  size_t part; int64_t idx; bool diag;
  const int rc = locate_entry(m, row, col, part, idx, diag);
  if (rc) return rc;
  CsxPartition &p = m->host.parts[part];
  if (diag) p.dvalues[(size_t)idx] = value;
  else if ((int64_t)p.values.size() == p.nnz) p.values[(size_t)idx] = value;
  if (m->uploaded) {
    CUDA_TRY(cudaSetDevice(m->device));
    double *dst = diag ? const_cast<double *>(m->pdev[part].dvalues) + idx : m->d_values + m->layout.parts[part].val_base + idx;
    CUDA_TRY(cudaMemcpy(dst, &value, 8, cudaMemcpyHostToDevice));
  }
  return 0;
}

int csxb_decode_coords(const csxb_matrix_t *mc, int part, int32_t *rows, int32_t *cols) {
  csxb_matrix *m = const_cast<csxb_matrix *>(mc);
  if (!m->uploaded) return fail("matrix not uploaded (csxb_upload)");
  if (part < 0 || (size_t)part >= m->pdev.size()) return fail("invalid partition");
  CUDA_TRY(cudaSetDevice(m->device));
  const PartLayout &pl = m->layout.parts[part];
  size_t n = (size_t)m->layout.total_values;
  int *dr = nullptr, *dcl = nullptr;
  CUDA_TRY(cudaMalloc((void **)&dr, std::max<size_t>(n, 1) * 4));
  CUDA_TRY(cudaMalloc((void **)&dcl, std::max<size_t>(n, 1) * 4));
  CUDA_TRY(cudaMemset(dr, 0xff, std::max<size_t>(n, 1) * 4));
  CUDA_TRY(cudaMemset(dcl, 0xff, std::max<size_t>(n, 1) * 4));
  if (pl.ntiles && !pl.xdesc.empty()) csx_decode_gather_kernel<<<(unsigned)pl.ntiles, CTA_THREADS>>>(m->pdev[part], dr, dcl);
  if (!pl.bt.empty()) csx_decode_bt_kernel<<<(unsigned)((pl.nrows + CTA_THREADS - 1) / CTA_THREADS), CTA_THREADS>>>(m->pdev[part], dr, dcl);
  if (!pl.sk_chunks.empty())
    csx_stream_decode_kernel<<<(unsigned)((pl.sk_chunks.size() + SK_WARPS - 1) / SK_WARPS), SK_WARPS * 32>>>(m->pdev[part], dr, dcl);
  CUDA_TRY(cudaGetLastError());
  CUDA_TRY(cudaMemcpy(rows, dr + pl.val_base, (size_t)pl.nnz * 4, cudaMemcpyDeviceToHost));
  CUDA_TRY(cudaMemcpy(cols, dcl + pl.val_base, (size_t)pl.nnz * 4, cudaMemcpyDeviceToHost));
  cudaFree(dr); cudaFree(dcl);
  return 0;
}

}

#include "device_group.inl"
```

### sparsex_b200/csrc/gather_kernel.cuh

```cuda
#pragma once
#include "part_dev.cuh"

template <bool SYM, class Op>
__device__ __forceinline__ void gather_desc(const uint4 d, const KindEntry *__restrict__ ktab, int myrow, Op &op) {
  const uint32_t meta = d.w, kind = (meta >> 24) & 0xf, size = (meta >> 16) & 0xff;
  const int r = (int)d.y, c = (int)d.z;
  const uint32_t voff = d.x;
  const uint32_t delta = (meta & XD_DELTA1) ? 1u : __ldg(&ktab[meta & 0xffff].delta);
  if (!SYM || !(meta & XD_TRANSPOSED)) {
    const int t = myrow - r;
    if (t < 0) return;
    const uint32_t k = (uint32_t)t / delta;
    if (k * delta != (uint32_t)t || k >= size) return;
    op.add(voff + k, kind == K_VERT ? c : (kind == K_DIAG ? c + t : c - t));
  } else if (kind == K_VERT) {
    if (myrow != c) return;
    for (uint32_t k = 0; k < size; k++) op.add(voff + k, r + (int)(k * delta));
  } else if (kind == K_HORIZ) {
    const int u = myrow - c;
    if (u < 0) return;
    const uint32_t k = (uint32_t)u / delta;
    if (k * delta != (uint32_t)u || k >= size) return;
    op.add(voff + k, r);
  } else if (kind == K_BCOL) {
    const uint32_t align = (__ldg(&ktab[meta & 0xffff].kind_align) >> 8) & 0xff;
    const uint32_t j = (uint32_t)(myrow - c);
    if (myrow < c || j >= align) return;
    for (uint32_t a = 0; a * align < size; a++) op.add(voff + a * align + j, r + (int)a);
  } else if (kind == K_BROW) {
    const uint32_t align = (__ldg(&ktab[meta & 0xffff].kind_align) >> 8) & 0xff;
    const uint32_t j = (uint32_t)(myrow - c);
    if (myrow < c || j * align >= size) return;
    for (uint32_t a = 0; a < align; a++) op.add(voff + j * align + a, r + (int)a);
  } else {
    const int u = kind == K_DIAG ? myrow - c : c - myrow;
    if (u < 0) return;
    const uint32_t k = (uint32_t)u / delta;
    if (k * delta != (uint32_t)u || k >= size) return;
    op.add(voff + k, r + u);
  }
}

template <bool SYM>
__device__ __forceinline__ bool desc_touches(const uint4 d, const KindEntry *__restrict__ ktab, int row_lo, int row_hi) {
  const uint32_t meta = d.w, kind = (meta >> 24) & 0xf, size = (meta >> 16) & 0xff;
  const int r = (int)d.y, c = (int)d.z;
  const uint32_t delta = (meta & XD_DELTA1) ? 1u : __ldg(&ktab[meta & 0xffff].delta);
  const int span = (int)((size - 1) * delta);
  int lo, hi;
  if (!SYM || !(meta & XD_TRANSPOSED)) { lo = r; hi = r + span; }
  else if (kind == K_VERT) { lo = hi = c; }
  else if (kind == K_DIAG || kind == K_HORIZ) { lo = c; hi = c + span; }
  else if (kind == K_ADIAG) { lo = c - span; hi = c; }
  else {
    const uint32_t align = (__ldg(&ktab[meta & 0xffff].kind_align) >> 8) & 0xff;
    lo = c; hi = c + (int)(kind == K_BCOL ? align : size / align) - 1;
  }
  return lo <= row_hi && hi >= row_lo;
}

template <bool SYM>
__device__ __forceinline__ bool linear_probe(const uint4 d, const KindEntry *__restrict__ ktab, int myrow, uint32_t &vi, int &xi) {
  const uint32_t meta = d.w, kind = (meta >> 24) & 0xf, size = (meta >> 16) & 0xff;
  const int r = (int)d.y, c = (int)d.z;
  const bool tr = SYM && (meta & XD_TRANSPOSED);
  int t = !tr ? myrow - r : (kind == K_ADIAG ? c - myrow : myrow - c);
  if (t < 0) return false;
  uint32_t k = (uint32_t)t;
  if (!(meta & XD_DELTA1)) {
    uint32_t delta = __ldg(&ktab[meta & 0xffff].delta);
    k = (uint32_t)t / delta;
    if (k * delta != (uint32_t)t) return false;
  }
  if (k >= size) return false;
  vi = d.x + k;
  xi = !tr ? (kind == K_VERT ? c : (kind == K_DIAG ? c + t : c - t)) : (kind == K_HORIZ ? r : r + t);
  return true;
}

template <bool COH>
__device__ __forceinline__ double ldx(const double *p) {
#ifndef CSXB_EMUL
  if (COH) return __ldcg(p);
#endif
  return __ldg(p);
}
template <bool COH>
struct SpmvGatherOp {
  const double *__restrict__ values;
  const double *x;
  double acc;
  __device__ __forceinline__ void add(uint32_t vi, int xi) { acc += __ldg(values + vi) * ldx<COH>(x + xi); }
};

template <int NL, bool COH>
__device__ __forceinline__ double bt_row(const BtDev &T, const double *__restrict__ vals, const double *__restrict__ x, uint32_t e0,
                                         uint32_t e1) {
  constexpr int N = NL > 0 ? NL : 1;
  const int sl = T.sl;
  double a0 = 0.0, a1 = 0.0;
  uint32_t e = e0;
  if (NL > 0) {
    uint2 n0{0u, 0u}, n1{0u, 0u};
    if (e + 1 < e1) { n0 = __ldg(T.ent + e); n1 = __ldg(T.ent + e + 1); }
    for (; e + 1 < e1; e += 2) {
      const uint2 b0 = n0, b1 = n1;
      if (e + 3 < e1) { n0 = __ldg(T.ent + e + 2); n1 = __ldg(T.ent + e + 3); }
      const double *v0 = vals + b0.x, *v1 = vals + b1.x, *x0 = x + (b0.y & ~BT_IMAGE), *x1 = x + (b1.y & ~BT_IMAGE);
      double va[N], xa[N], vb[N], xb[N];
#pragma unroll
      for (int l = 0; l < N; l++) { va[l] = __ldg(v0 + l * sl); xa[l] = ldx<COH>(x0 + l); vb[l] = __ldg(v1 + l * sl); xb[l] = ldx<COH>(x1 + l); }
#pragma unroll
      for (int l = 0; l < N; l++) { a0 += va[l] * xa[l]; a1 += vb[l] * xb[l]; }
    }
  }
  for (; e < e1; e++) {
    const uint2 b = __ldg(T.ent + e);
    const double *vp = vals + b.x, *xp = x + (b.y & ~BT_IMAGE);
    if (NL > 0) {
      double va[N], xa[N];
#pragma unroll
      for (int l = 0; l < N; l++) { va[l] = __ldg(vp + l * sl); xa[l] = ldx<COH>(xp + l); }
#pragma unroll
      for (int l = 0; l < N; l++) a0 += va[l] * xa[l];
    } else {
      for (int l = 0; l < T.nloop; l++) a0 += __ldg(vp + l * sl) * ldx<COH>(xp + l);
    }
  }
  return a0 + a1;
}

constexpr int XCHG_MAX_PEERS = 15;
struct XchgDev {
  double *vec[2];
  unsigned long long *step;
  unsigned long long *flags;
  unsigned long long *error;
  int rank, nwait, npush;
  int wait_rank[XCHG_MAX_PEERS];
  unsigned long long *peer_flags[XCHG_MAX_PEERS];
  long long push_lo[XCHG_MAX_PEERS], push_hi[XCHG_MAX_PEERS];
  double *push_vec[XCHG_MAX_PEERS][2];
  int mode;
  int nb;
  int split;
  int edge_lo_end, edge_hi_begin;
  unsigned long long *started, *bdone;
};
struct NoXchg {};

enum { KSET_ANY = 0, KSET_DIAG1 = 1 };
template <bool XD, bool SYM, int RPT, int KSET, int VAR, bool PUSH, class XP, bool BT = false, bool COH = false>
__device__ __forceinline__ void spmv_tile(const PartDev &P, const double *__restrict__ x, double *__restrict__ y, double alpha,
                                          double beta, int overwrite, const long long tile, const long long row_block, const XP &X,
                                          const unsigned long long xk) {
  const int lane = threadIdx.x & 31, warp = threadIdx.x >> 5;
  const long long lrow0 = ((row_block * (CTA_THREADS / 32) + warp) * RPT) * 32;
  if (lrow0 >= P.nrows) return;
  double acc[RPT];
#pragma unroll
  for (int k = 0; k < RPT; k++) acc[k] = 0.0;

  unsigned long long pol_stream = 0, pol_keep = 0;
#ifndef CSXB_EMUL
  if (VAR == 3) {
    asm volatile("createpolicy.fractional.L2::evict_first.b64 %0, 1.0;" : "=l"(pol_stream));
    asm volatile("createpolicy.fractional.L2::evict_last.b64 %0, 1.0;" : "=l"(pol_keep));
  }
#endif
  if (XD) {
    const uint32_t b = __ldg(P.tile_xoff + tile), e = __ldg(P.tile_xoff + tile + 1);
    const int grow0 = (int)(P.row_start + lrow0);
    const double *__restrict__ values = P.values;
    for (uint32_t base = b; base < e; base += 32) {
      const uint32_t j = base + lane;
      bool hit = false;
      if (j < e) {
        const uint4 d = __ldg(P.xdesc + j);
        if (KSET == KSET_DIAG1) hit = (int)d.y <= grow0 + 32 * RPT - 1 && (int)d.y + (int)((d.w >> 16) & 0xff) > grow0;
        else hit = desc_touches<SYM>(d, P.ktab, grow0, grow0 + 32 * RPT - 1);
      }
      uint32_t mask = __ballot_sync(FULL, hit);
      while (mask) {
        const uint4 d = __ldg(P.xdesc + base + __ffs(mask) - 1);
        mask &= mask - 1;
        if (KSET == KSET_DIAG1) {
          const int t0 = grow0 + lane - (int)d.y;
          const uint32_t size = (d.w >> 16) & 0xff;
          const double *__restrict__ vp = values + ((long long)d.x + t0);
          const double *__restrict__ xp = x + ((long long)(int)d.z + t0);
#ifndef CSXB_EMUL
          if (VAR == 3 && RPT == 4) {
            double v0, v1, v2, v3, x0, x1, x2, x3;
            asm volatile(
                "{\n\t.reg .pred p0, p1, p2, p3;\n\t"
                "setp.lt.u32 p0, %8, %12;\n\tsetp.lt.u32 p1, %9, %12;\n\tsetp.lt.u32 p2, %10, %12;\n\tsetp.lt.u32 p3, %11, %12;\n\t"
                "mov.f64 %0, 0d0000000000000000;\n\tmov.f64 %1, 0d0000000000000000;\n\t"
                "mov.f64 %2, 0d0000000000000000;\n\tmov.f64 %3, 0d0000000000000000;\n\t"
                "mov.f64 %4, 0d0000000000000000;\n\tmov.f64 %5, 0d0000000000000000;\n\t"
                "mov.f64 %6, 0d0000000000000000;\n\tmov.f64 %7, 0d0000000000000000;\n\t"
                "@p0 ld.global.nc.L1::no_allocate.L2::cache_hint.f64 %0, [%13], %15;\n\t@p0 ld.global.nc.L2::cache_hint.f64 %4, [%14], %16;\n\t"
                "@p1 ld.global.nc.L1::no_allocate.L2::cache_hint.f64 %1, [%13+256], %15;\n\t@p1 ld.global.nc.L2::cache_hint.f64 %5, [%14+256], %16;\n\t"
                "@p2 ld.global.nc.L1::no_allocate.L2::cache_hint.f64 %2, [%13+512], %15;\n\t@p2 ld.global.nc.L2::cache_hint.f64 %6, [%14+512], %16;\n\t"
                "@p3 ld.global.nc.L1::no_allocate.L2::cache_hint.f64 %3, [%13+768], %15;\n\t@p3 ld.global.nc.L2::cache_hint.f64 %7, [%14+768], %16;\n\t}"
                : "=d"(v0), "=d"(v1), "=d"(v2), "=d"(v3), "=d"(x0), "=d"(x1), "=d"(x2), "=d"(x3)
                : "r"((uint32_t)t0), "r"((uint32_t)(t0 + 32)), "r"((uint32_t)(t0 + 64)), "r"((uint32_t)(t0 + 96)), "r"(size),
                  "l"(vp), "l"(xp), "l"(pol_stream), "l"(pol_keep));
            acc[0] += v0 * x0; acc[1 % RPT] += v1 * x1; acc[2 % RPT] += v2 * x2; acc[3 % RPT] += v3 * x3;
            continue;
          }
          if (VAR == 1 && RPT == 4) {
            double v0, v1, v2, v3, x0, x1, x2, x3;
            asm volatile(
                "{\n\t.reg .pred p0, p1, p2, p3;\n\t"
                "setp.lt.u32 p0, %8, %12;\n\tsetp.lt.u32 p1, %9, %12;\n\tsetp.lt.u32 p2, %10, %12;\n\tsetp.lt.u32 p3, %11, %12;\n\t"
                "mov.f64 %0, 0d0000000000000000;\n\tmov.f64 %1, 0d0000000000000000;\n\t"
                "mov.f64 %2, 0d0000000000000000;\n\tmov.f64 %3, 0d0000000000000000;\n\t"
                "mov.f64 %4, 0d0000000000000000;\n\tmov.f64 %5, 0d0000000000000000;\n\t"
                "mov.f64 %6, 0d0000000000000000;\n\tmov.f64 %7, 0d0000000000000000;\n\t"
                "@p0 ld.global.nc.f64 %0, [%13];\n\t@p0 ld.global.nc.f64 %4, [%14];\n\t"
                "@p1 ld.global.nc.f64 %1, [%13+256];\n\t@p1 ld.global.nc.f64 %5, [%14+256];\n\t"
                "@p2 ld.global.nc.f64 %2, [%13+512];\n\t@p2 ld.global.nc.f64 %6, [%14+512];\n\t"
                "@p3 ld.global.nc.f64 %3, [%13+768];\n\t@p3 ld.global.nc.f64 %7, [%14+768];\n\t}"
                : "=d"(v0), "=d"(v1), "=d"(v2), "=d"(v3), "=d"(x0), "=d"(x1), "=d"(x2), "=d"(x3)
                : "r"((uint32_t)t0), "r"((uint32_t)(t0 + 32)), "r"((uint32_t)(t0 + 64)), "r"((uint32_t)(t0 + 96)), "r"(size),
                  "l"(vp), "l"(xp));
            acc[0] += v0 * x0; acc[1 % RPT] += v1 * x1; acc[2 % RPT] += v2 * x2; acc[3 % RPT] += v3 * x3;
            continue;
          }
#endif
          double v[RPT], xv[RPT];
#pragma unroll
          for (int k = 0; k < RPT; k++) {
            v[k] = 0.0; xv[k] = 0.0;
            if ((uint32_t)(t0 + k * 32) < size) { v[k] = __ldg(vp + k * 32); xv[k] = ldx<COH>(xp + k * 32); }
          }
#pragma unroll
          for (int k = 0; k < RPT; k++) acc[k] += v[k] * xv[k];
          continue;
        }
        if (!(SYM && (d.w & XD_TRANSPOSED) && (((d.w >> 24) & 0xf) == K_VERT || ((d.w >> 24) & 0xf) >= K_BROW))) {
          double v[RPT], xv[RPT];
#pragma unroll
          for (int k = 0; k < RPT; k++) {
            uint32_t vi; int xi;
            v[k] = 0.0; xv[k] = 0.0;
            if (linear_probe<SYM>(d, P.ktab, grow0 + k * 32 + lane, vi, xi)) { v[k] = __ldg(values + vi); xv[k] = ldx<COH>(x + xi); }
          }
#pragma unroll
          for (int k = 0; k < RPT; k++) acc[k] += v[k] * xv[k];
        } else {
#pragma unroll
          for (int k = 0; k < RPT; k++) {
            SpmvGatherOp<COH> op{values, x, 0.0};
            gather_desc<SYM>(d, P.ktab, grow0 + k * 32 + lane, op);
            acc[k] += op.acc;
          }
        }
      }
    }
  }

  for (int c = 0; BT && c < P.nbt; c++) {
    const BtDev &T = P.bt[c];
#pragma unroll 1
    for (int k = 0; k < RPT; k++) {
      const long long lrow = lrow0 + k * 32 + lane;
      if (lrow < P.nrows) {
        const uint32_t g = (uint32_t)(P.row_start + lrow);
        uint32_t J = g;
        if (T.G != 1) { J = __umulhi(g, T.magic); if (J * (uint32_t)T.G > g) J--; }
        const int f = (int)(g - J * (uint32_t)T.G) * T.sf;
        const uint32_t *pp = T.ptr + ((long long)J - T.j0);
        const uint32_t e0 = __ldg(pp), e1 = __ldg(pp + 1);
        switch (T.nloop) {
          case 1: acc[k] += bt_row<1, COH>(T, P.values + f, x, e0, e1); break;
          case 2: acc[k] += bt_row<2, COH>(T, P.values + f, x, e0, e1); break;
          case 3: acc[k] += bt_row<3, COH>(T, P.values + f, x, e0, e1); break;
          case 4: acc[k] += bt_row<4, COH>(T, P.values + f, x, e0, e1); break;
          default: acc[k] += bt_row<0, COH>(T, P.values + f, x, e0, e1);
        }
      }
    }
  }

#pragma unroll
  for (int k = 0; k < RPT; k++) {
    const long long lrow = lrow0 + k * 32 + lane;
    if (lrow < P.nrows) {
      const long long g = P.row_start + lrow;
      double a = acc[k];
      if (SYM && P.dvalues) a += __ldg(P.dvalues + lrow) * ldx<COH>(x + g);
      const double r = overwrite ? alpha * a : alpha * a + beta * y[g];
      y[g] = r;
      if constexpr (PUSH) {
        for (int p = 0; p < X.npush; p++)
          if (g >= X.push_lo[p] && g < X.push_hi[p]) X.push_vec[p][(xk & 1) ^ 1][g] = r;
      }
    }
  }
}


__device__ __forceinline__ void t_segment_warp(const uint2 *__restrict__ ent, const uint32_t *__restrict__ seg,
                                               const double *__restrict__ values, const double *__restrict__ x,
                                               double *__restrict__ scratch, uint32_t s, int lane) {
  const uint32_t e0 = __ldg(seg + s), e1 = __ldg(seg + s + 1);
  double a0 = 0.0, a1 = 0.0;
  uint32_t e = e0 + (uint32_t)lane;
  for (; e + 32 < e1; e += 64) {
    const uint2 b0 = __ldg(ent + e), b1 = __ldg(ent + e + 32);
    const double v0 = __ldg(values + b0.x), x0 = __ldg(x + (b0.y & ~BT_IMAGE));
    const double v1 = __ldg(values + b1.x), x1 = __ldg(x + (b1.y & ~BT_IMAGE));
    a0 += v0 * x0;
    a1 += v1 * x1;
  }
  if (e < e1) {
    const uint2 b = __ldg(ent + e);
    a0 += __ldg(values + b.x) * __ldg(x + (b.y & ~BT_IMAGE));
  }
  const double a = warp_sum(a0 + a1);
  if (lane == 0) scratch[s] = a;
}
```

### sparsex_b200/csrc/gpu_layout.cpp

```cpp
#include <algorithm>
#include <climits>
#include <cstring>
#include <map>

#include "gpu_layout.hpp"

namespace spxb {
namespace {

inline uint64_t get_varint(const uint8_t *ctl, uint64_t &p) {
  uint64_t v = 0;
  unsigned shift = 0;
  for (;;) {
    uint8_t b = ctl[p++];
    v |= (uint64_t)(b & 0x7f) << shift;
    if (!(b & 0x80)) break;
    shift += 7;
  }
  return v;
}

}

bool classify(long pid, KindEntry &ke) {
  int type = (int)(pid / PATTERN_ID_OFFSET);
  uint32_t d = (uint32_t)(pid % PATTERN_ID_OFFSET);
  uint32_t kind, align = 0, delta = d;
  if (type == T_NONE) {
    if (d == 8) kind = K_DELTA8; else if (d == 16) kind = K_DELTA16; else if (d == 32) kind = K_DELTA32;
    else if (d == 64) kind = K_DELTA64; else return false;
    delta = d / 8;
  } else if (type == T_HORIZ) kind = K_HORIZ;
  else if (type == T_VERT) kind = K_VERT;
  else if (type == T_DIAG) kind = K_DIAG;
  else if (type == T_ADIAG) kind = K_ADIAG;
  else if (is_brow(type)) {
    align = blk_align(type);
    if (align == 1) { kind = K_HORIZ; delta = 1; align = 0; }
    else kind = K_BROW;
  } else if (is_bcol(type)) {
    align = blk_align(type);
    if (align == 1) { kind = K_VERT; delta = 1; align = 0; }
    else kind = K_BCOL;
  } else return false;
  if (delta == 0) return false;
  ke.kind_align = kind | (align << 8);
  ke.delta = delta;
  return true;
}

namespace {

struct Pending { int64_t part; int64_t tile; XDesc d; };

inline int tile_rpt(int64_t nrows, int forced, bool block_tables) {
  return forced ? forced : ((nrows >= (int64_t(1) << 20) && !block_tables) ? 4 : 1);
}

struct SkUnit {
  uint64_t off, end;
  uint32_t size, ntasks;
  int64_t row, reach;
  int64_t cmin, cmax;
  int64_t val;
  int64_t cursor_before;
  bool multi_bcol;
  bool round_end;
};

class SkBuilder {
 public:
  SkBuilder(PartLayout &L, int64_t nrows) : L_(L), nrows_(nrows) {}
  void add(const SkUnit &u0) {
    SkUnit u = u0;
    u.round_end = false;
    while (!open_.empty() && !fits(u)) {
      std::vector<SkUnit> rest = split(u);
      for (const SkUnit &w : rest) add(w);
    }
    if (open_.empty()) { wrow_ = (first_ && u.row + u.reach <= 64) ? 0 : u.row; rounds_ = 1; round_start_ = 0; }
    else if (round_closes(u)) { open_.back().round_end = true; rounds_++; round_start_ = open_.size(); }
    open_.push_back(u);
  }
  void finish() {
    if (!open_.empty()) close(open_.size(), 0, false);
    open_.clear();
    std::stable_sort(fixes_.begin(), fixes_.end(),
                     [](const std::pair<int32_t, uint32_t> &a, const std::pair<int32_t, uint32_t> &b) { return a.first < b.first; });
    for (size_t i = 0; i < fixes_.size(); i++) {
      if (i == 0 || fixes_[i].first != fixes_[i - 1].first) { L_.sk_fix_rows.push_back(fixes_[i].first); L_.sk_fix_ptr.push_back((uint32_t)i); }
      L_.sk_fix_idx.push_back(fixes_[i].second);
    }
    L_.sk_fix_ptr.push_back((uint32_t)fixes_.size());
  }
  void discard() {
    open_.clear(); fixes_.clear();
    L_.sk_chunks.clear(); L_.sk_uoffs.clear(); L_.sk_gaps.clear(); L_.sk_scratch = 0;
    L_.sk_first_row.clear(); L_.sk_last_row.clear(); L_.sk_cmin.clear(); L_.sk_cmax.clear();
    L_.sk_fix_rows.clear(); L_.sk_fix_ptr.clear(); L_.sk_fix_idx.clear();
  }

 private:
  bool round_closes(const SkUnit &u) const {
    const size_t units = open_.size() - round_start_;
    uint32_t tasks = 0, elems = 0;
    for (size_t i = round_start_; i < open_.size(); i++) { tasks += open_[i].ntasks; elems += open_[i].size; }
    if (units == (size_t)SK_ROUND_UNITS || tasks + u.ntasks > (uint32_t)SK_MAX_TASKS || elems + u.size > (uint32_t)SK_MAX_ELEMS) return true;
    if (units < 16 || tasks == 0) return false;
    const uint32_t fill = tasks - 32 * ((tasks - 1) / 32);
    return fill >= 24 && fill + u.ntasks > 32 && (SK_ROUND_UNITS - units) * tasks < 8 * units;
  }
  bool fits(const SkUnit &u) const {
    if (rounds_ == SK_MAX_ROUNDS && round_closes(u)) return false;
    return u.end - open_.front().off <= (uint64_t)SK_MAX_BYTES && u.row + u.reach - wrow_ <= SK_WROWS - 1 &&
           u.row - wrow_ <= SK_WROWS - 2;
  }
  std::vector<SkUnit> split(const SkUnit &next) {
    size_t b = open_.size();
    if (next.row == open_.back().row) {
      for (size_t i = open_.size() - 1; i > 0; i--)
        if (open_[i].row != open_[i - 1].row) { if (4 * i >= 3 * open_.size()) b = i; break; }
    }
    close(b, b < open_.size() ? open_[b].row : next.row, true);
    std::vector<SkUnit> rest(open_.begin() + (long)b, open_.end());
    open_.clear();
    return rest;
  }
  void close(size_t b, int64_t next_row, bool has_next) {
    const int64_t ra = open_[0].row, rl = open_[b - 1].row;
    int64_t touch_hi = 0, cmin = INT64_MAX, cmax = -1;
    bool multib = false;
    for (size_t i = 0; i < b; i++) {
      touch_hi = std::max(touch_hi, open_[i].row + open_[i].reach);
      cmin = std::min(cmin, open_[i].cmin); cmax = std::max(cmax, open_[i].cmax);
      multib |= open_[i].multi_bcol;
    }
    int64_t own_lo = first_ ? 0 : prev_own_hi_;
    if (first_ && wrow_ != 0) { L_.sk_gaps.push_back(SkGap{0, ra}); own_lo = ra; }
    const int64_t own_hi = has_next ? (next_row > rl ? next_row : rl + 1) : nrows_;
    const bool head = !first_ && own_lo > ra;
    const int64_t f_lo = own_lo - wrow_, f_hi = std::min(own_hi, wrow_ + SK_WROWS) - wrow_;
    if (own_hi > wrow_ + SK_WROWS) L_.sk_gaps.push_back(SkGap{wrow_ + SK_WROWS, own_hi});
    const int64_t t_hi = touch_hi >= own_hi ? touch_hi - wrow_ + 1 : f_hi;
    const uint32_t slot = L_.sk_scratch;
    L_.sk_scratch += (uint32_t)(head ? 1 : 0) + (uint32_t)(t_hi - f_hi);
    if (head) fixes_.push_back(std::make_pair((int32_t)ra, slot));
    for (int64_t i = 0; i < t_hi - f_hi; i++) fixes_.push_back(std::make_pair((int32_t)(own_hi + i), slot + (head ? 1u : 0u) + (uint32_t)i));
    SkEntry e;
    const uint64_t off0 = open_[0].off;
    e.w[0] = (uint32_t)off0; e.w[1] = (uint32_t)open_[0].val; e.w[2] = (uint32_t)open_[0].cursor_before;
    e.w[3] = (uint32_t)(int32_t)wrow_; e.w[4] = (uint32_t)L_.sk_uoffs.size(); e.w[5] = slot;
    e.w[6] = (uint32_t)(b - 1) | ((uint32_t)(ra - wrow_) << 8) | ((uint32_t)f_lo << 16) | ((uint32_t)((off0 >> 32) & 0x3f) << 24) |
             ((uint32_t)head << 30) | ((uint32_t)multib << 31);
    e.w[7] = (uint32_t)f_hi | ((uint32_t)t_hi << 9);
    L_.sk_chunks.push_back(e);
    {
      uint32_t rt = 0;
      for (size_t i = 0; i < b; i++) {
        rt += open_[i].ntasks;
        L_.sk_stat[2] += open_[i].ntasks; L_.sk_stat[3] += open_[i].size;
        if (open_[i].round_end || i + 1 == b) { L_.sk_stat[0]++; L_.sk_stat[1] += (rt + 31) / 32; rt = 0; }
      }
    }
    for (size_t i = 0; i < b; i++)
      L_.sk_uoffs.push_back((uint16_t)((open_[i].off - off0) | ((open_[i].round_end || i + 1 == b) ? 0x8000u : 0u)));
    L_.sk_first_row.push_back((int32_t)wrow_);
    L_.sk_last_row.push_back((int32_t)std::max(touch_hi, wrow_ + f_hi - 1));
    L_.sk_cmin.push_back(cmin == INT64_MAX ? INT32_MAX : (int32_t)cmin);
    L_.sk_cmax.push_back((int32_t)cmax);
    prev_own_hi_ = own_hi;
    first_ = false;
  }
  PartLayout &L_;
  int64_t nrows_;
  std::vector<SkUnit> open_;
  std::vector<std::pair<int32_t, uint32_t>> fixes_;
  int64_t wrow_ = 0, prev_own_hi_ = 0;
  int rounds_ = 1;
  size_t round_start_ = 0;
  bool first_ = true;
};

struct BtEnt { int64_t q; int tab; int64_t grp; BlockImage b; };
bool block_table_shape(const DeviceLayout &L, int t, BlockTable &T) {
  if (t == 0) { T.G = L.bc_rows; T.nloop = L.bc_align; T.sf = L.bc_align; T.sl = 1; }
  else if (t == 1) { T.G = L.bc_align; T.nloop = L.bc_rows; T.sf = 1; T.sl = L.bc_align; T.image = 1; }
  else if (t == 2) { T.G = L.br_align; T.nloop = L.br_cols; T.sf = 1; T.sl = L.br_align; }
  else if (t == 3) { T.G = L.br_align ? std::max(L.br_img_cols, 1) : 0; T.nloop = L.br_align; T.sf = L.br_align; T.sl = 1; T.image = 1; }
  else { T.G = 1; T.nloop = 1; T.sf = 0; T.sl = 0; }
  if (T.G <= 0) { T.G = 1; return false; }
  return true;
}
void sort_block_tables(const DeviceLayout &shape, std::vector<PartLayout> &parts, const std::vector<BtEnt> &btents) {
  for (size_t q = 0; q < parts.size(); q++) {
    PartLayout &L = parts[q];
    if (!L.nrows) continue;
    L.bt.resize(BT_MAX);
    for (int t = 0; t < BT_MAX; t++) {
      BlockTable &T = L.bt[t];
      if (!block_table_shape(shape, t, T)) continue;
      T.j0 = L.row_start / T.G;
      T.ptr.assign((size_t)((L.row_start + L.nrows - 1) / T.G - T.j0 + 1) + 1, 0);
    }
  }
  for (const BtEnt &e : btents) {
    BlockTable &T = parts[e.q].bt[e.tab];
    T.ptr[(size_t)(e.grp - T.j0) + 1]++;
  }
  std::vector<std::vector<uint32_t>> at(parts.size() * BT_MAX);
  for (size_t q = 0; q < parts.size(); q++)
    for (int t = 0; t < BT_MAX && !parts[q].bt.empty(); t++) {
      BlockTable &T = parts[q].bt[t];
      for (size_t j = 1; j < T.ptr.size(); j++) T.ptr[j] += T.ptr[j - 1];
      if (!T.ptr.empty()) T.ent.resize(T.ptr.back());
      at[q * BT_MAX + t].assign(T.ptr.begin(), T.ptr.end());
    }
  for (const BtEnt &e : btents) {
    BlockTable &T = parts[e.q].bt[e.tab];
    T.ent[at[(size_t)e.q * BT_MAX + e.tab][(size_t)(e.grp - T.j0)]++] = e.b;
  }
  for (size_t q = 0; q < parts.size(); q++) {
    std::vector<BlockTable> keep;
    for (BlockTable &T : parts[q].bt) if (!T.ent.empty()) keep.push_back(std::move(T));
    parts[q].bt.swap(keep);
  }
}
std::string distribute_descs(std::vector<PartLayout> &parts, const std::vector<Pending> &pend) {
  std::vector<std::vector<uint32_t>> cnt(parts.size());
  for (size_t q = 0; q < parts.size(); q++) cnt[q].assign((size_t)parts[q].ntiles + 1, 0);
  for (const Pending &e : pend) cnt[e.part][e.tile + 1]++;
  for (size_t q = 0; q < parts.size(); q++) {
    PartLayout &L = parts[q];
    for (int64_t t = 0; t < L.ntiles; t++) cnt[q][t + 1] += cnt[q][t];
    if (cnt[q][L.ntiles] >= 0x80000000u) return "cross-row unit table too large";
    L.xdesc.resize(cnt[q][L.ntiles]);
    for (int64_t t = 0; t <= L.ntiles; t++) L.tile_xoff[t] = cnt[q][t];
  }
  std::vector<std::vector<uint32_t>> fill(cnt);
  for (const Pending &e : pend) {
    parts[e.part].xdesc[fill[e.part][e.tile]++] = e.d;
    if (((e.d.meta >> 24) & 0xf) != K_DIAG || !(e.d.meta & XD_DELTA1) || (e.d.meta & XD_TRANSPOSED))
      parts[e.part].xd_diag1_only = false;
  }
  return "";
}

bool block_image_fits(const DeviceLayout &L, uint32_t kind, int64_t delta, int64_t grow, int64_t start_col) {
  if (kind == K_BCOL) return delta % L.bc_rows == 0 && grow % L.bc_rows == 0 && start_col % L.bc_align == 0;
  return delta % L.br_cols == 0 && grow % L.br_align == 0 && (L.br_img_cols <= 1 || start_col % L.br_img_cols == 0);
}
template <class OwnerEnd, class Put>
bool block_images(const DeviceLayout &L, uint32_t kind, uint32_t voff, int64_t grow, int64_t start_col, int64_t delta,
                  OwnerEnd owner_end, Put put) {
  if (kind == K_BCOL) {
    const int64_t A = L.bc_align, R0 = L.bc_rows;
    for (int64_t k = 0; k * R0 < delta; k++)
      for (int64_t g = start_col; g < start_col + A;) {
        const int64_t e = owner_end(g, start_col + A);
        if (e < 0) return false;
        put(1, g / A, BlockImage{voff + (uint32_t)(k * R0 * A), (uint32_t)(grow + k * R0) | BT_IMAGE}, g);
        g = e;
      }
    return true;
  }
  const int64_t A = L.br_align, G = std::max(L.br_img_cols, 1);
  for (int64_t j = 0; j < delta; j += G)
    for (int64_t g = start_col + j; g < start_col + j + G;) {
      const int64_t e = owner_end(g, start_col + j + G);
      if (e < 0) return false;
      put(3, g / G, BlockImage{voff + (uint32_t)(j * A), (uint32_t)grow | BT_IMAGE}, g);
      g = e;
    }
  return true;
}

}

std::string build_layout(const CsxMatrix &m, DeviceLayout &out) {
  out = DeviceLayout();
  out.symmetric = m.symmetric;
  out.full_colind = m.full_colind;
  const size_t np = m.parts.size();
  if (m.symmetric && np && (int)np != m.nparts_total) {
    const int64_t first_row = m.parts.front().row_start;
    int64_t lo = first_row;
    for (auto &p : m.parts) if (p.col_max >= p.col_min) lo = std::min(lo, p.col_min);
    out.halo_lo = lo; out.halo_hi = first_row;
  }
  const bool has_halo = out.halo_hi > out.halo_lo;
  const size_t nq = np + (has_halo ? 1 : 0);
  out.parts.resize(nq);
  auto q_start = [&](size_t q) { return q < np ? m.parts[q].row_start : out.halo_lo; };
  auto q_rows = [&](size_t q) { return q < np ? m.parts[q].nrows : out.halo_hi - out.halo_lo; };
  auto q_tile = [&](size_t q) { return (int64_t)CTA_THREADS * tile_rpt(q_rows(q), m.rows_per_thread, out.bc_align || out.br_align); };
  auto owner_of = [&](int64_t grow) -> int64_t {
    for (size_t q = 0; q < nq; q++)
      if (grow >= q_start(q) && grow < q_start(q) + q_rows(q)) return (int64_t)q;
    return -1;
  };
  std::map<std::pair<uint32_t, uint32_t>, uint32_t> kindex;
  auto kind_index = [&](const KindEntry &ke) -> int64_t {
    auto key = std::make_pair(ke.kind_align, ke.delta);
    auto it = kindex.find(key);
    if (it == kindex.end()) {
      if (out.ktab.size() >= 65535) return -1;
      it = kindex.insert(std::make_pair(key, (uint32_t)out.ktab.size())).first;
      out.ktab.push_back(ke);
    }
    return it->second;
  };
  std::vector<Pending> pend;
  auto list_rows = [&](const XDesc &d, int64_t lo, int64_t hi, std::vector<Pending> &to) -> bool {
    int64_t g = lo;
    while (g <= hi) {
      const int64_t q = owner_of(g);
      if (q < 0) return false;
      const int64_t rel = g - q_start((size_t)q), qt = q_tile((size_t)q);
      to.push_back(Pending{q, rel / qt, d});
      g = std::min(q_start((size_t)q) + (rel / qt + 1) * qt, q_start((size_t)q) + q_rows((size_t)q));
    }
    return true;
  };
  {
    constexpr int CAND = 17;
    std::map<uint32_t, std::vector<int64_t>> bc_cov, br_cov, bri_cov;
    auto cov = [&](std::map<uint32_t, std::vector<int64_t>> &mp, uint32_t a) -> std::vector<int64_t> & {
      std::vector<int64_t> &v = mp[a];
      if (v.empty()) v.assign(CAND, 0);
      return v;
    };
    for (size_t pi = 0; pi < np; pi++) {
      const CsxPartition &cp = m.parts[pi];
      KindEntry tab[64];
      size_t nid = 0;
      bool any = false;
      for (; nid < cp.id_map.size() && cp.id_map[nid] != -1 && nid < 64; nid++) {
        if (!classify(cp.id_map[nid], tab[nid])) return "unsupported pattern id " + std::to_string(cp.id_map[nid]);
        any |= (tab[nid].kind_align & 0xff) >= K_BROW;
      }
      if (!any) continue;
      const uint8_t *ctl = cp.ctl.data();
      uint64_t p = 0, end = cp.ctl.size();
      int64_t row = 0, col = 0;
      while (p + 2 <= end) {
        const uint8_t flags = ctl[p++], size = ctl[p++];
        if (flags & 0x80) { row += (flags & 0x40) ? (int64_t)get_varint(ctl, p) : 1; col = 0; }
        if (m.full_colind) { uint32_t c; memcpy(&c, ctl + p, 4); p += 4; col = c; }
        else col = (int64_t)((uint64_t)col + get_varint(ctl, p));
        const uint32_t id = flags & 0x3f;
        if (id >= nid || size == 0) return "ctl stream uses an unmapped unit id";
        const uint32_t kind = tab[id].kind_align & 0xff, align = (tab[id].kind_align >> 8) & 0xff, delta = tab[id].delta;
        const int64_t grow = cp.row_start + row;
        if (kind <= K_DELTA64) {
          for (int k = 1; k < size; k++) { uint64_t d = 0; memcpy(&d, ctl + p, delta); p += delta; col += (int64_t)d; }
        } else if (kind == K_HORIZ) col += (int64_t)(size - 1) * delta;
        else if (kind == K_BCOL) {
          std::vector<int64_t> &v = cov(bc_cov, align);
          if (!m.symmetric || col % align == 0)
            for (int r = 2; r < CAND; r++) if (delta % r == 0 && grow % r == 0) v[r] += size;
        } else if (kind == K_BROW) {
          if (grow % align == 0) {
            std::vector<int64_t> &v = cov(br_cov, align), &vi = cov(bri_cov, align);
            for (int r = 1; r < CAND; r++) {
              if (delta % r == 0) v[r] += size;
              if (delta % r == 0 && col % r == 0) vi[r] += size;
            }
          }
        }
      }
    }
    auto pick = [&](std::map<uint32_t, std::vector<int64_t>> &mp, int rmin, int &A, int &R0) {
      int64_t best = 0;
      for (auto &kv : mp)
        for (int r = CAND - 1; r >= rmin; r--)
          if ((int64_t)r * kv.first >= 4 && kv.second[r] > best + best / 64) { best = kv.second[r]; A = (int)kv.first; R0 = r; }
    };
    pick(bc_cov, 2, out.bc_align, out.bc_rows);
    pick(br_cov, 1, out.br_align, out.br_cols);
    if (out.br_align) {
      const std::vector<int64_t> &vi = bri_cov[(uint32_t)out.br_align];
      out.br_img_cols = 1;
      for (int r = CAND - 1; r >= 2; r--)
        if (out.br_cols % r == 0 && vi[r] >= br_cov[(uint32_t)out.br_align][out.br_cols] - br_cov[(uint32_t)out.br_align][out.br_cols] / 64) { out.br_img_cols = r; break; }
    }
    if (getenv("CSXB_NO_BLOCK_TABLES")) out.bc_align = out.bc_rows = out.br_align = out.br_cols = out.br_img_cols = 0;
  }
  std::vector<BtEnt> btents;
  struct BlockTmp { XDesc d; uint32_t kind, align, other; int64_t cmin, cmax; };
  std::vector<BlockTmp> blocks;

  uint64_t vbase = 0, cbase = 0;
  for (size_t pi = 0; pi < nq; pi++) {
    PartLayout &L = out.parts[pi];
    L.nrows = q_rows(pi); L.row_start = q_start(pi);
    L.val_base = vbase; L.ctl_base = cbase;
    L.rpt = tile_rpt(L.nrows, m.rows_per_thread, out.bc_align || out.br_align);
    const int64_t TILE_ROWS = L.tile_rows();
    L.ntiles = (L.nrows + TILE_ROWS - 1) / TILE_ROWS;
    L.tile_xoff.assign((size_t)L.ntiles + 1, 0);
    L.tile_cmin.assign((size_t)L.ntiles, INT32_MAX);
    L.tile_cmax.assign((size_t)L.ntiles, -1);
    memset(L.idtab, 0, sizeof(L.idtab));
    if (pi >= np) { L.is_halo = true; continue; }
    const CsxPartition &cp = m.parts[pi];
    L.nnz = cp.nnz; L.ctl_size = (int64_t)cp.ctl.size();
    vbase += (uint64_t)cp.nnz;
    cbase += ((uint64_t)cp.ctl.size() + CTL_PAD + 15) & ~uint64_t(15);
    if (m.symmetric)
      for (int64_t t = 0; t < L.ntiles; t++) {
        L.tile_cmin[t] = (int32_t)(cp.row_start + t * TILE_ROWS);
        L.tile_cmax[t] = (int32_t)(cp.row_start + std::min<int64_t>(cp.nrows, (t + 1) * TILE_ROWS) - 1);
      }
    uint32_t id2k[64];
    KindEntry truetab[64];
    bool in_table[64];
    size_t nid = 0;
    for (; nid < cp.id_map.size() && cp.id_map[nid] != -1; nid++) {
      if (nid >= 64) return "too many unit kinds";
      KindEntry ke;
      if (!classify(cp.id_map[nid], ke)) return "unsupported pattern id " + std::to_string(cp.id_map[nid]);
      truetab[nid] = ke;
      const uint32_t kd = ke.kind_align & 0xff, al = (ke.kind_align >> 8) & 0xff;
      in_table[nid] = (kd == K_BCOL && (int)al == out.bc_align) || (kd == K_BROW && (int)al == out.br_align);
      L.idtab[nid] = in_table[nid] ? IdEntry{K_VERT, 1, 1, 65536} : IdEntry{ke.kind_align, ke.delta, 1, 65536};
      const int64_t ki = kind_index(ke);
      if (ki < 0) return "too many distinct unit kinds on one device";
      id2k[nid] = (uint32_t)ki;
    }
// ... 96 lines not shown
        for (int64_t t = row / TILE_ROWS; t <= (row + span) / TILE_ROWS; t++) {
          L.tile_cmin[t] = std::min<int32_t>(L.tile_cmin[t], (int32_t)wlo);
          L.tile_cmax[t] = std::max<int32_t>(L.tile_cmax[t], (int32_t)whi);
        }
      }

      const bool to_table = goes_to_xdt(kind) || in_table[id];
      {
        const IdEntry &ie = L.idtab[id];
        SkUnit su;
        su.off = unit_off; su.end = p; su.size = size;
        su.ntasks = sk_unit_tasks(ie.kind_align & 0xff, size, ie.delta, ie.sl, ie.recip);
        su.row = row; su.reach = to_table ? 0 : span;
        su.cmin = cmin; su.cmax = cmax; su.val = v; su.cursor_before = cursor_before;
        su.multi_bcol = kind == K_BCOL && su.ntasks > 1;
        su.round_end = false;
        if (L.sk_uoffs.size() >= 0xfffffff0ull) return "unit-offset table too large";
        sk.add(su);
      }
      XDesc d;
      d.voff = (uint32_t)(L.val_base + (uint64_t)v);
      d.row = (int32_t)(cp.row_start + row);
      d.col = (int32_t)start_col;
      d.meta = id2k[id] | ((uint32_t)size << 16) | (kind << 24);
      if (delta == 1) d.meta |= XD_DELTA1;
      if (!to_table) {
        L.has_flat = true;
        L.flat_elems += size;
        if (singles_ok && singles.size() + size <= element_cap) {
          for (int k = 0; k < size; k++) {
            int64_t er = row, ec = start_col;
            if (kind <= K_DELTA64) ec = ecols[k];
            else if (kind == K_HORIZ) ec = start_col + (int64_t)k * delta;
            else if (kind == K_BROW) { er = row + k % (int)align; ec = start_col + k / (int)align; }
            else { er = row + k / (int)align; ec = start_col + k % (int)align; }
            singles.push_back(Single{(int32_t)er, (int32_t)ec, (uint32_t)(v + k)});
          }
        } else {
          singles_ok = false;
        }
        if (m.symmetric) {
          XDesc td = d;
          td.meta |= XD_TRANSPOSED;
          if (kind <= K_DELTA64) {
            for (int k = 0; k < size; k++) {
              XDesc e;
              e.voff = d.voff + (uint32_t)k; e.row = d.row; e.col = (int32_t)ecols[k];
              e.meta = (uint32_t)k_single | (1u << 16) | ((uint32_t)K_DIAG << 24) | XD_DELTA1 | XD_TRANSPOSED;
              if (!list_rows(e, ecols[k], ecols[k], simg)) return "symmetric update targets a row that is not on this device";
            }
          } else if (kind == K_HORIZ) {
            if (!list_rows(td, cmin, cmax, simg)) return "symmetric update targets a row that is not on this device";
          } else {
            blocks.push_back(BlockTmp{td, kind, align, delta, cmin, cmax});
          }
        }
      } else if (in_table[id]) {
        const int64_t grow = cp.row_start + row;
        const bool fits = kind == K_BCOL ? (m.symmetric ? block_image_fits(out, kind, delta, grow, start_col)
                                                        : ((int64_t)delta % out.bc_rows == 0 && grow % out.bc_rows == 0))
                                         : ((int64_t)delta % out.br_cols == 0 && grow % out.br_align == 0);
        if (!fits) {
          for (int k = 0; k < size; k++) {
            const int64_t er = grow + (kind == K_BROW ? k % (int)align : k / (int)align);
            const int64_t ec = start_col + (kind == K_BROW ? k / (int)align : k % (int)align);
            btents.push_back(BtEnt{(int64_t)pi, 4, er, BlockImage{d.voff + (uint32_t)k, (uint32_t)ec}});
            if (m.symmetric) {
              const int64_t q = owner_of(ec);
              if (q < 0) return "symmetric update targets a row that is not on this device";
              btents.push_back(BtEnt{q, 4, ec, BlockImage{d.voff + (uint32_t)k, (uint32_t)er | BT_IMAGE}});
            }
          }
        } else {
          if (kind == K_BCOL) {
            const int64_t A = out.bc_align, R0 = out.bc_rows;
            for (int64_t k = 0; k * R0 < (int64_t)delta; k++)
              btents.push_back(BtEnt{(int64_t)pi, 0, (grow + k * R0) / R0, BlockImage{d.voff + (uint32_t)(k * R0 * A), (uint32_t)start_col}});
          } else {
            const int64_t A = out.br_align, C0 = out.br_cols;
            for (int64_t k = 0; k * C0 < (int64_t)delta; k++)
              btents.push_back(BtEnt{(int64_t)pi, 2, grow / A, BlockImage{d.voff + (uint32_t)(k * C0 * A), (uint32_t)(start_col + k * C0)}});
          }
          if (m.symmetric && kind == K_BROW && !block_image_fits(out, kind, delta, grow, start_col)) {
            XDesc td = d;
            td.meta |= XD_TRANSPOSED;
            if (!list_rows(td, cmin, cmax, pend)) return "symmetric update targets a row that is not on this device";
          } else if (m.symmetric) {
            auto owner_end = [&](int64_t g, int64_t hi) -> int64_t {
              const int64_t q = owner_of(g);
              return q < 0 ? -1 : std::min(hi, q_start((size_t)q) + q_rows((size_t)q));
            };
            auto put = [&](int tab, int64_t grp, BlockImage b, int64_t g) { btents.push_back(BtEnt{owner_of(g), tab, grp, b}); };
            if (!block_images(out, kind, d.voff, grow, start_col, delta, owner_end, put))
              return "symmetric update targets a row that is not on this device";
          }
        }
      } else {
        for (int64_t t = row / TILE_ROWS; t <= (row + span) / TILE_ROWS; t++) pend.push_back(Pending{(int64_t)pi, t, d});
        if (m.symmetric) {
          XDesc td = d;
          td.meta |= XD_TRANSPOSED;
          if (!list_rows(td, cmin, cmax, pend)) return "symmetric update targets a row that is not on this device";
        }
      }
      v += size;
    }
    if (v != cp.nnz) return "ctl stream covers " + std::to_string(v) + " values, expected " + std::to_string(cp.nnz);
    if (L.has_flat) sk.finish(); else sk.discard();
    if (L.has_flat && singles_ok && (int64_t)singles.size() == L.flat_elems && singles.size() > single_cap) {
      for (const Single &sg : singles) {
        const uint32_t vo = (uint32_t)(L.val_base + (uint64_t)sg.v);
        const int64_t grow = cp.row_start + sg.row;
        btents.push_back(BtEnt{(int64_t)pi, 4, grow, BlockImage{vo, (uint32_t)sg.col}});
        if (m.symmetric) {
          const int64_t q = owner_of(sg.col);
          if (q < 0) return "symmetric update targets a row that is not on this device";
          btents.push_back(BtEnt{q, 4, sg.col, BlockImage{vo, (uint32_t)grow | BT_IMAGE}});
        }
      }
      sk.discard();
      simg.clear();
      blocks.resize(blocks_before);
      L.has_flat = false;
      L.flat_elems = 0;
    } else if (L.has_flat && singles_ok && (int64_t)singles.size() == L.flat_elems) {
      for (const Single &sg : singles) {
        XDesc d;
        d.voff = (uint32_t)(L.val_base + (uint64_t)sg.v);
        d.row = (int32_t)(cp.row_start + sg.row);
        d.col = (int32_t)sg.col;
        d.meta = (uint32_t)k_single | (1u << 16) | ((uint32_t)K_DIAG << 24) | XD_DELTA1;
        pend.push_back(Pending{(int64_t)pi, sg.row / TILE_ROWS, d});
        if (m.symmetric) {
          XDesc td = d;
          td.meta |= XD_TRANSPOSED;
          if (!list_rows(td, sg.col, sg.col, pend)) return "symmetric update targets a row that is not on this device";
        }
      }
      sk.discard();
      simg.clear();
      blocks.resize(blocks_before);
      L.has_flat = false;
      L.flat_elems = 0;
    }
    pend.insert(pend.end(), simg.begin(), simg.end());
  }
  out.total_values = vbase;
  out.total_ctl = cbase;
  if (vbase >= (uint64_t(1) << 32)) return "more than 2^32 values on one device";

  for (const BlockTmp &b : blocks)
    if (!list_rows(b.d, b.cmin, b.cmax, pend)) return "symmetric update targets a row that is not on this device";
  if (!btents.empty()) sort_block_tables(out, out.parts, btents);
  return distribute_descs(out.parts, pend);
}

std::string build_transpose_layout(const CsxMatrix &m, const DeviceLayout &fwd, TransLayout &out) {
  out = TransLayout();
  if (m.symmetric) return "CSX-Sym needs no transposed tables (A^T = A)";
  const size_t np = m.parts.size();
  if (fwd.parts.size() != np) return "the forward layout does not belong to this matrix";
  if (const char *v = getenv("CSXB_T_HEAVY")) out.heavy_min = std::max(1, atoi(v));
  if (const char *v = getenv("CSXB_T_SEG")) out.seg_len = std::max(32, atoi(v));
  int64_t clo = INT64_MAX, chi = -1;
  for (const CsxPartition &p : m.parts) if (p.col_max >= p.col_min) { clo = std::min(clo, p.col_min); chi = std::max(chi, p.col_max); }
  if ((int)np == m.nparts_total) { clo = 0; chi = m.ncols - 1; }
  if (chi < clo) { clo = 0; chi = -1; }
  out.ktab = fwd.ktab;
  std::map<std::pair<uint32_t, uint32_t>, uint32_t> kindex;
  for (size_t i = 0; i < out.ktab.size(); i++) kindex.insert(std::make_pair(std::make_pair(out.ktab[i].kind_align, out.ktab[i].delta), (uint32_t)i));
  auto kind_index = [&](uint32_t kind_align, uint32_t delta) -> int64_t {
    auto it = kindex.find(std::make_pair(kind_align, delta));
    if (it == kindex.end()) {
      if (out.ktab.size() >= 65535) return -1;
      it = kindex.insert(std::make_pair(std::make_pair(kind_align, delta), (uint32_t)out.ktab.size())).first;
      out.ktab.push_back(KindEntry{kind_align, delta});
    }
    return it->second;
  };
  const int64_t k_single = kind_index(K_DIAG, 1);
  if (k_single < 0) return "too many distinct unit kinds on one device";
  struct Emit { XDesc d; int64_t lo, hi; };
  std::vector<Emit> em;
  std::vector<BtEnt> btents;
  struct Single { int64_t row, col; uint32_t voff; };
  std::vector<Single> singles;
  for (size_t pi = 0; pi < np; pi++) {
    const CsxPartition &cp = m.parts[pi];
    KindEntry truetab[64];
    uint32_t id2k[64];
    size_t nid = 0;
    for (; nid < cp.id_map.size() && cp.id_map[nid] != -1; nid++) {
      if (nid >= 64) return "too many unit kinds";
      if (!classify(cp.id_map[nid], truetab[nid])) return "unsupported pattern id " + std::to_string(cp.id_map[nid]);
      const int64_t ki = kind_index(truetab[nid].kind_align, truetab[nid].delta);
      if (ki < 0) return "too many distinct unit kinds on one device";
      id2k[nid] = (uint32_t)ki;
    }
    const uint64_t vbase = fwd.parts[pi].val_base;
    const uint8_t *ctl = cp.ctl.data();
    uint64_t p = 0;
    const uint64_t end = cp.ctl.size();
    int64_t row = 0, col = 0, v = 0;
    singles.clear();
    while (p < end) {
      if (p + 2 > end) return "ctl stream truncated";
      const uint8_t flags = ctl[p++], size = ctl[p++];
      if (flags & 0x80) { row += (flags & 0x40) ? (int64_t)get_varint(ctl, p) : 1; col = 0; }
      if (m.full_colind) { uint32_t c; memcpy(&c, ctl + p, 4); p += 4; col = c; }
      else col = (int64_t)((uint64_t)col + get_varint(ctl, p));
      if (row >= cp.nrows) return "ctl stream leaves the partition (row " + std::to_string(row) + ")";
      const uint32_t id = flags & 0x3f;
      if (id >= nid) return "ctl stream uses an unmapped unit id";
      if (size == 0) return "ctl unit of size 0";
      const uint32_t kind = truetab[id].kind_align & 0xff, align = (truetab[id].kind_align >> 8) & 0xff, delta = truetab[id].delta;
      const int64_t start_col = col, grow = cp.row_start + row, span = (int64_t)(size - 1) * delta;
      const uint32_t voff = (uint32_t)(vbase + (uint64_t)v);
      XDesc d;
      d.voff = voff;
      d.meta = id2k[id] | ((uint32_t)size << 16) | (kind << 24) | (delta == 1 ? XD_DELTA1 : 0u);
      if (kind <= K_DELTA64) {
        if (p + (uint64_t)(size - 1) * delta > end) return "ctl stream truncated";
        singles.push_back(Single{grow, col, voff});
        for (int k = 1; k < size; k++) {
          uint64_t dd = 0;
          memcpy(&dd, ctl + p, delta);
          p += delta;
          col += (int64_t)dd;
          singles.push_back(Single{grow, col, voff + (uint32_t)k});
        }
      } else if (kind == K_HORIZ) {
        const int64_t ki = kind_index(K_VERT, delta);
        if (ki < 0) return "too many distinct unit kinds on one device";
        d.row = (int32_t)start_col; d.col = (int32_t)grow;
        d.meta = (uint32_t)ki | ((uint32_t)size << 16) | ((uint32_t)K_VERT << 24) | (delta == 1 ? XD_DELTA1 : 0u);
        em.push_back(Emit{d, start_col, start_col + span});
        col += span;
      } else if (kind == K_DIAG) {
        d.row = (int32_t)start_col; d.col = (int32_t)grow;
        em.push_back(Emit{d, start_col, start_col + span});
      } else if (kind == K_VERT || kind == K_ADIAG) {
        d.row = (int32_t)grow; d.col = (int32_t)start_col;
        d.meta |= XD_TRANSPOSED;
        em.push_back(kind == K_VERT ? Emit{d, start_col, start_col} : Emit{d, start_col - span, start_col});
      } else {
        if (size % align || size / align != delta) return "inconsistent block unit";
        const bool in_table = (kind == K_BCOL && (int)align == fwd.bc_align) || (kind == K_BROW && (int)align == fwd.br_align);
        if (in_table && block_image_fits(fwd, kind, delta, grow, start_col)) {
          auto owner_end = [](int64_t, int64_t hi) -> int64_t { return hi; };
          auto put = [&](int tab, int64_t grp, BlockImage b, int64_t) { btents.push_back(BtEnt{0, tab, grp, b}); };
          block_images(fwd, kind, voff, grow, start_col, delta, owner_end, put);
        } else {
          for (int k = 0; k < size; k++) {
            const int64_t er = grow + (kind == K_BROW ? k % (int)align : k / (int)align);
            const int64_t ec = start_col + (kind == K_BROW ? k / (int)align : k % (int)align);
            singles.push_back(Single{er, ec, voff + (uint32_t)k});
          }
        }
      }
      v += size;
    }
    if (v != cp.nnz) return "ctl stream covers " + std::to_string(v) + " values, expected " + std::to_string(cp.nnz);
    const bool as_desc = singles.size() <= (size_t)(cp.nnz / 256);
    for (const Single &sg : singles) {
      if (sg.col < clo || sg.col > chi) return "unit leaves the column range";
      if (as_desc) {
        XDesc e;
        e.voff = sg.voff; e.row = (int32_t)sg.col; e.col = (int32_t)sg.row;
        e.meta = (uint32_t)k_single | (1u << 16) | ((uint32_t)K_DIAG << 24) | XD_DELTA1;
        em.push_back(Emit{e, sg.col, sg.col});
      } else {
        btents.push_back(BtEnt{0, 4, sg.col, BlockImage{sg.voff, (uint32_t)sg.row | BT_IMAGE}});
      }
    }
  }
  std::vector<PartLayout> parts(1);
  PartLayout &L = parts[0];
  L.row_start = clo; L.nrows = chi - clo + 1;
  L.rpt = tile_rpt(L.nrows, m.rows_per_thread, !btents.empty());
  const int64_t TILE_ROWS = L.tile_rows();
  L.ntiles = (L.nrows + TILE_ROWS - 1) / TILE_ROWS;
  L.tile_xoff.assign((size_t)L.ntiles + 1, 0);
  memset(L.idtab, 0, sizeof(L.idtab));
  std::vector<Pending> pend;
  for (const Emit &e : em) {
    if (e.lo < clo || e.hi > chi) return "unit leaves the column range";
    for (int64_t t = (e.lo - clo) / TILE_ROWS; t <= (e.hi - clo) / TILE_ROWS; t++) pend.push_back(Pending{0, t, e.d});
    out.images |= (e.d.meta & XD_TRANSPOSED) != 0;
  }
  if (!btents.empty()) sort_block_tables(fwd, parts, btents);
  std::string err = distribute_descs(parts, pend);
  if (!err.empty()) return err;
  for (size_t ti = 0; ti < L.bt.size(); ti++) {
    BlockTable &T = L.bt[ti];
    if (T.G != 1 || T.nloop != 1) continue;
    std::vector<uint32_t> ptr(1, 0);
    std::vector<BlockImage> ent;
    L.sk_fix_ptr.assign(1, 0);
    for (size_t j = 0; j + 1 < T.ptr.size(); j++) {
      const uint32_t e0 = T.ptr[j], e1 = T.ptr[j + 1];
      if (e1 - e0 > (uint32_t)out.heavy_min) {
        L.sk_fix_rows.push_back((int32_t)(T.j0 + (int64_t)j - L.row_start));
        for (uint32_t e = e0; e < e1; e += (uint32_t)out.seg_len) {
          L.sk_fix_idx.push_back((uint32_t)out.hseg.size());
          out.hseg.push_back((uint32_t)out.hent.size());
          out.hent.insert(out.hent.end(), T.ent.begin() + e, T.ent.begin() + std::min(e1, e + (uint32_t)out.seg_len));
        }
        L.sk_fix_ptr.push_back((uint32_t)L.sk_fix_idx.size());
      } else {
        ent.insert(ent.end(), T.ent.begin() + e0, T.ent.begin() + e1);
      }
      ptr.push_back((uint32_t)ent.size());
    }
    out.hseg.push_back((uint32_t)out.hent.size());
    out.heavy_cols = (int64_t)L.sk_fix_rows.size();
    L.sk_scratch = (uint32_t)(out.hseg.size() - 1);
    T.ptr.swap(ptr);
    T.ent.swap(ent);
    if (T.ent.empty()) L.bt.erase(L.bt.begin() + (long)ti);
    break;
  }
  if (out.hseg.empty()) out.hseg.push_back(0);
  out.part = std::move(L);
  return "";
}

void decode_transpose_coords(const TransLayout &t, int32_t *rows, int32_t *cols) {
  const PartLayout &L = t.part;
  auto put = [&](uint64_t vi, int64_t r, int64_t c) { rows[vi] = (int32_t)r; cols[vi] = (int32_t)c; };
  for (const XDesc &d : L.xdesc) {
    const uint32_t kind = (d.meta >> 24) & 0xf, size = (d.meta >> 16) & 0xff;
    const int64_t delta = (d.meta & XD_DELTA1) ? 1 : t.ktab[d.meta & 0xffff].delta;
    for (uint32_t k = 0; k < size; k++) {
      const int64_t s = (int64_t)k * delta;
      if (!(d.meta & XD_TRANSPOSED))
        put(d.voff + k, kind == K_VERT ? d.col : (kind == K_DIAG ? d.col + s : d.col - s), d.row + s);
      else
        put(d.voff + k, d.row + s, kind == K_ADIAG ? d.col - s : d.col);
    }
  }
  for (const BlockTable &T : L.bt)
    for (size_t j = 0; j + 1 < T.ptr.size(); j++)
      for (uint32_t e = T.ptr[j]; e < T.ptr[j + 1]; e++)
        for (int64_t i = 0; i < T.G; i++) {
          const int64_t g = (T.j0 + (int64_t)j) * T.G + i;
          if (g < L.row_start || g >= L.row_start + L.nrows) continue;
          for (int l = 0; l < T.nloop; l++)
            put((uint64_t)T.ent[e].voff + (uint64_t)(i * T.sf + l * T.sl), (int64_t)(T.ent[e].other & ~BT_IMAGE) + l, g);
        }
  for (size_t i = 0; i < L.sk_fix_rows.size(); i++)
    for (uint32_t j = L.sk_fix_ptr[i]; j < L.sk_fix_ptr[i + 1]; j++)
      for (uint32_t e = t.hseg[L.sk_fix_idx[j]]; e < t.hseg[L.sk_fix_idx[j] + 1]; e++)
        put(t.hent[e].voff, (int64_t)(t.hent[e].other & ~BT_IMAGE), L.row_start + L.sk_fix_rows[i]);
}

}
```

### sparsex_b200/csrc/gpu_layout.hpp

```cpp
#pragma once
#include <cstdint>
#include <string>
#include <vector>

#include "csx_host.hpp"

#ifdef __CUDACC__
#define SPXB_HD __host__ __device__
#else
#define SPXB_HD
#endif

namespace spxb {

constexpr int CTA_THREADS = 256;
constexpr int CTL_PAD = 32;

enum Kind : uint32_t {
  K_DELTA8 = 0, K_DELTA16 = 1, K_DELTA32 = 2, K_DELTA64 = 3, K_HORIZ = 4,
  K_VERT = 5, K_DIAG = 6, K_ADIAG = 7, K_BROW = 8, K_BCOL = 9
};
inline bool kind_row_local(uint32_t k) { return k <= K_HORIZ; }
inline bool goes_to_xdt(uint32_t kind) { return kind >= K_VERT && kind <= K_ADIAG; }

struct XDesc {
  uint32_t voff;
  int32_t row;
  int32_t col;
  uint32_t meta;
};
constexpr uint32_t XD_TRANSPOSED = 1u << 28;
constexpr uint32_t XD_DELTA1 = 1u << 29;

struct KindEntry { uint32_t kind_align; uint32_t delta; };
struct IdEntry { uint32_t kind_align; uint32_t delta; uint32_t sl; uint32_t recip; };

constexpr int SK_ROUND_UNITS = 32;
constexpr int SK_MAX_ROUNDS = 4;
constexpr int SK_MAX_UNITS = SK_ROUND_UNITS * SK_MAX_ROUNDS;
constexpr int SK_MAX_TASKS = 224;
constexpr int SK_MAX_ELEMS = 1023;
constexpr int SK_MAX_BYTES = 8191;
constexpr int SK_WROWS = 256;
constexpr int SK_RL_E = 4;
constexpr int SK_BLK_E = 12;
constexpr int SK_BLK_LINES = 4;
struct SkEntry { uint32_t w[8]; };
struct SkGap { int64_t lo, hi; };

SPXB_HD inline uint32_t sk_unit_tasks(uint32_t kind, uint32_t size, uint32_t delta, uint32_t sl, uint32_t recip) {
  if (kind <= 4u) return (size + SK_RL_E - 1) / SK_RL_E;
  if (kind >= 8u) return ((delta + sl - 1) * recip) >> 16;
  return 1;
}

struct BlockImage { uint32_t voff; uint32_t other; };
constexpr uint32_t BT_IMAGE = 0x80000000u;
struct BlockTable {
  int G = 1, nloop = 0, sf = 0, sl = 0;
  int image = 0;
  int64_t j0 = 0;
  std::vector<uint32_t> ptr;
  std::vector<BlockImage> ent;
};
constexpr int BT_MAX = 5;

struct PartLayout {
  int64_t nrows = 0, row_start = 0, nnz = 0, ctl_size = 0;
  std::vector<SkEntry> sk_chunks;
  std::vector<uint16_t> sk_uoffs;
  std::vector<int32_t> sk_fix_rows;
  std::vector<uint32_t> sk_fix_ptr;
  std::vector<uint32_t> sk_fix_idx;
  std::vector<SkGap> sk_gaps;
  uint32_t sk_scratch = 0;
  uint32_t sk_kmask = 0;
  int sk_rows = 1;
  int sk_bc = 0;
  int sk_brc = 0;
  int64_t sk_stat[4] = {0, 0, 0, 0};
  std::vector<int32_t> sk_first_row, sk_last_row, sk_cmin, sk_cmax;
  uint64_t val_base = 0, ctl_base = 0;
  bool has_flat = false;
  bool is_halo = false;
  bool xd_diag1_only = true;
  int64_t ntiles = 0;
  int rpt = 1;
  int64_t tile_rows() const { return (int64_t)CTA_THREADS * rpt; }
  IdEntry idtab[64];
  std::vector<int32_t> tile_cmin, tile_cmax;
  std::vector<uint32_t> tile_xoff;
  std::vector<XDesc> xdesc;
  int64_t flat_elems = 0;
  std::vector<BlockTable> bt;
};

struct DeviceLayout {
  std::vector<KindEntry> ktab;
  std::vector<PartLayout> parts;
  uint64_t total_values = 0, total_ctl = 0;
  bool symmetric = false, full_colind = false;
  int bc_align = 0, bc_rows = 0, br_align = 0, br_cols = 0;
  int br_img_cols = 0;
  int64_t halo_lo = 0, halo_hi = 0;
};

std::string build_layout(const CsxMatrix &m, DeviceLayout &out);

constexpr int T_HEAVY_MIN = 128;
constexpr int T_SEG_LEN = 256;
struct TransLayout {
  PartLayout part;
  std::vector<KindEntry> ktab;
  bool images = false;
  std::vector<BlockImage> hent;
  std::vector<uint32_t> hseg;
  int64_t heavy_cols = 0;
  int heavy_min = T_HEAVY_MIN, seg_len = T_SEG_LEN;
};
std::string build_transpose_layout(const CsxMatrix &m, const DeviceLayout &fwd, TransLayout &out);
void decode_transpose_coords(const TransLayout &t, int32_t *rows, int32_t *cols);
bool classify(long pid, KindEntry &ke);

struct RowIndex {
  std::vector<uint64_t> ctl_off;
  std::vector<uint64_t> val_off;
  std::vector<int32_t> span;
  int32_t max_span = 0;
};
std::string build_row_index(const CsxPartition &cp, bool full_colind, RowIndex &ri);
int64_t find_entry(const CsxPartition &cp, bool full_colind, const RowIndex &ri, int64_t prow, int64_t col);
std::string save_matrix(const CsxMatrix &m, const char *path);
std::string load_matrix(const char *path, CsxMatrix &m);

}
```

### sparsex_b200/csrc/part_dev.cuh

```cuda
#pragma once
#include "gpu_layout.hpp"

using namespace spxb;

struct BtDev {
  const uint32_t *ptr;
  const uint2 *ent;
  long long j0;
  int G, nloop, sf, sl, image;
  uint32_t magic;
};
struct PartDev {
  const uint8_t *ctl;
  const double *values;
  const uint32_t *tile_xoff;
  const uint4 *xdesc;
  const KindEntry *ktab;
  const double *dvalues;
  long long nrows, row_start;
  uint32_t val_base;
  int full_colind;
  int rpt;
  uint32_t tile0;
  BtDev bt[BT_MAX];
  int nbt;
  const uint4 *sk_chunks;
  const uint16_t *sk_uoffs;
  double *sk_scratch;
  const int32_t *sk_fix_rows;
  const uint32_t *sk_fix_ptr, *sk_fix_idx;
  const long long *sk_gaps;
  uint32_t sk_c0, sk_c1;
  uint32_t sk_f0, sk_f1;
  uint32_t sk_g0, sk_g1;
  const uint8_t *ctl_end;
  const double *values_end;
  IdEntry idtab[64];
};

constexpr unsigned FULL = 0xffffffffu;

__device__ __forceinline__ double warp_sum(double v) {
#pragma unroll
  for (int o = 16; o; o >>= 1) v += __shfl_xor_sync(FULL, v, o);
  return v;
}
```

### sparsex_b200/engine.py

```python
import ctypes as C
import os

import numpy as np

_HERE = os.path.dirname(os.path.abspath(__file__))
_LIB = None


class EngineError(RuntimeError):
    pass


def lib_path():
    return os.environ.get("SPARSEX_B200_LIB") or os.path.join(_HERE, "libsparsex_b200.so")


def lib():
    global _LIB
    if _LIB is not None:
        return _LIB
    path = lib_path()
    if not os.path.exists(path):
        raise EngineError("%s is missing: run `python -c 'import __graft_entry__ as g; g.build()'` "
                          "(the engine has no CPU fallback)" % path)
# ... 53 lines not shown
    L.csxb_get_perm.argtypes = [vp, vp]
    L.csxb_group_create.restype = vp
    L.csxb_group_create.argtypes = [vp, vp, i32, i32, cp, C.c_size_t]
    L.csxb_group_destroy.argtypes = [vp]
    L.csxb_group_size.restype = i32
    L.csxb_group_size.argtypes = [vp]
    L.csxb_group_member.restype = vp
    L.csxb_group_member.argtypes = [vp, i32]
    L.csxb_group_device.restype = i32
    L.csxb_group_device.argtypes = [vp, i32]
    L.csxb_group_spmv.restype = i32
    L.csxb_group_spmv.argtypes = [vp, dbl, vp, dbl, vp, i32]
    L.csxb_group_spmv_t.restype = i32
    L.csxb_group_spmv_t.argtypes = [vp, dbl, vp, dbl, vp, i32]
    L.csxb_group_save.restype = i32
    L.csxb_group_save.argtypes = [vp, cp]
    L.csxb_group_get_entry.restype = i32
    L.csxb_group_get_entry.argtypes = [vp, i64, i64, C.POINTER(dbl)]
    L.csxb_group_set_entry.restype = i32
    L.csxb_group_set_entry.argtypes = [vp, i64, i64, dbl]
    L.csxb_xchg_create.restype = vp
    L.csxb_xchg_create.argtypes = [vp, i32, i32]
    L.csxb_xchg_handle.restype = i32
    L.csxb_xchg_handle.argtypes = [vp, vp]
    L.csxb_xchg_connect.restype = i32
    L.csxb_xchg_connect.argtypes = [vp, vp, vp, vp, vp, vp]
    L.csxb_xchg_connect_ptr.restype = i32
    L.csxb_xchg_connect_ptr.argtypes = [vp, vp, vp, vp, vp, vp]
    L.csxb_xchg_base.restype = vp
    L.csxb_xchg_base.argtypes = [vp]
    L.csxb_xchg_vector.restype = vp
    L.csxb_xchg_vector.argtypes = [vp, i32]
    L.csxb_xchg_spmv.restype = i32
    L.csxb_xchg_spmv.argtypes = [vp, dbl, vp]
    L.csxb_xchg_status.restype = i64
    L.csxb_xchg_status.argtypes = [vp, i32]
    L.csxb_xchg_destroy.argtypes = [vp]
    _LIB = L
    return L


def rcm_csr(rowptr, colind, n):
    rowptr = np.ascontiguousarray(rowptr, dtype=np.int32)
    colind = np.ascontiguousarray(colind, dtype=np.int32)
    perm = np.empty(n, dtype=np.int32)
    bw = np.zeros(2, dtype=np.int64)
    rc = lib().csxb_rcm_csr(rowptr.ctypes.data, colind.ctypes.data, n, n, perm.ctypes.data, bw.ctypes.data)
    if rc == 1:
        return None, None
    if rc != 0:
        raise EngineError("csxb_rcm_csr: invalid arguments")
    return perm, (int(bw[0]), int(bw[1]))


def permute_csr(rowptr, colind, values, perm):
    rowptr = np.ascontiguousarray(rowptr, dtype=np.int32)
    colind = np.ascontiguousarray(colind, dtype=np.int32)
    values = np.ascontiguousarray(values, dtype=np.float64)
    perm = np.ascontiguousarray(perm, dtype=np.int32)
    n = len(rowptr) - 1
    orp, oci, ova = np.empty_like(rowptr), np.empty_like(colind), np.empty_like(values)
    if lib().csxb_permute_csr(rowptr.ctypes.data, colind.ctypes.data, values.ctypes.data, n, perm.ctypes.data,
                              orp.ctypes.data, oci.ctypes.data, ova.ctypes.data) != 0:
        raise EngineError("csxb_permute_csr: invalid arguments")
    return orp, oci, ova


def _opts(opts):
    return ";".join("%s=%s" % (k, v) for k, v in (opts or {}).items()).encode()


class Partition(object):
    pass


class CsxMatrix(object):

    NROWS, NCOLS, NNZ, SYMMETRIC, NPARTS, NPARTS_TOTAL, PART_LO, FULL_COLIND = range(8)
    B_VALUES, B_CTL, B_TABLES, B_X, B_Y, B_TOTAL, B_LAUNCHES = range(7)

    def __init__(self, handle, keepalive=None):
        self._h = handle
        self._keep = keepalive
        L = lib()
        self.nrows = L.csxb_info(handle, self.NROWS)
        self.ncols = L.csxb_info(handle, self.NCOLS)
        self.nnz = L.csxb_info(handle, self.NNZ)
        self.symmetric = bool(L.csxb_info(handle, self.SYMMETRIC))
        self.nparts = L.csxb_info(handle, self.NPARTS)
        self.nparts_total = L.csxb_info(handle, self.NPARTS_TOTAL)
        self.part_lo = L.csxb_info(handle, self.PART_LO)
        self.uploaded = False

    @classmethod
    def tune_csr(cls, rowptr, colind, values, nrows, ncols, opts=None, part_lo=0, part_hi=-1):
        rowptr = np.ascontiguousarray(rowptr, dtype=np.int32)
        colind = np.ascontiguousarray(colind, dtype=np.int32)
        values = np.ascontiguousarray(values, dtype=np.float64)
        err = C.create_string_buffer(1024)
        h = lib().csxb_tune_csr(rowptr.ctypes.data, colind.ctypes.data, values.ctypes.data, nrows, ncols,
                                _opts(opts), part_lo, part_hi, err, 1024)
        if not h:
            raise EngineError(err.value.decode())
        return cls(h)

    @classmethod
    def tune_csr_slab(cls, rowptr, colind, values, nrows_total, ncols, row_start, part, opts=None):
        rowptr = np.ascontiguousarray(rowptr, dtype=np.int32)
        colind = np.ascontiguousarray(colind, dtype=np.int32)
        values = np.ascontiguousarray(values, dtype=np.float64)
        err = C.create_string_buffer(1024)
        h = lib().csxb_tune_csr_slab(rowptr.ctypes.data, colind.ctypes.data, values.ctypes.data, rowptr.size - 1, nrows_total,
                                     ncols, row_start, part, _opts(opts), err, 1024)
        if not h:
            raise EngineError(err.value.decode())
        return cls(h)

    @classmethod
    def tune_mmf(cls, path, opts=None, part_lo=0, part_hi=-1):
        err = C.create_string_buffer(1024)
        h = lib().csxb_tune_mmf(path.encode(), _opts(opts), part_lo, part_hi, err, 1024)
        if not h:
            raise EngineError(err.value.decode())
        return cls(h)

    def partition(self, p):
        L = lib()
        P = Partition()
        info = [L.csxb_part_info(self._h, p, w) for w in range(11)]
        (P.nnz, P.nrows, P.ncols, P.row_start, P.ctl_size, P.row_jumps, idl, mapl, dvl, ril, P.sampling_undefined) = info

        def grab(what, n, dt):
            a = np.empty(n, dt)
            if n and L.csxb_part_copy(self._h, p, what, a.ctypes.data) != 0:
                raise EngineError(L.csxb_last_error().decode())
            return a
        P.values = grab(0, P.nnz, np.float64)
        P.ctl = grab(1, P.ctl_size, np.uint8)
        P.id_map = grab(2, idl, np.int64)
        ri = grab(3, ril * 3, np.int64).reshape(-1, 3)
        P.rows_info = np.stack([ri[:, 0], ri[:, 1], ri[:, 2] & 0xffffffff], axis=1) if ril else ri
        P.dvalues = grab(4, dvl, np.float64)
        P.map_cpus = grab(5, mapl, np.uint32)
        P.map_pos = grab(6, mapl, np.uint32)
        P.log = L.csxb_part_log(self._h, p).decode()
        return P

    def upload(self, device=0, free_host=False):
        if lib().csxb_upload(self._h, device, int(free_host)) != 0:
            raise EngineError(lib().csxb_last_error().decode())
        self.uploaded = True
        return self

    def traffic(self):
        L = lib()
        keys = ["values", "ctl", "tables", "x", "y", "total", "launches"]
        return {k: L.csxb_traffic(self._h, i) for i, k in enumerate(keys)}

    def spmv_ptr(self, alpha, x_ptr, beta, y_ptr, overwrite, stream=0):
        if lib().csxb_spmv(self._h, alpha, x_ptr, beta, y_ptr, int(overwrite), stream) != 0:
            raise EngineError(lib().csxb_last_error().decode())

    def spmv(self, alpha, x, y, beta=0.0, overwrite=True, stream=None):
        import torch
        assert x.is_cuda and y.is_cuda and x.dtype == torch.float64 and y.dtype == torch.float64
        assert x.numel() == self.ncols and y.numel() == self.nrows and x.is_contiguous() and y.is_contiguous()
        s = torch.cuda.current_stream().cuda_stream if stream is None else stream
        self.spmv_ptr(alpha, x.data_ptr(), beta, y.data_ptr(), overwrite, s)
        return y

    def spmv_host(self, alpha, x, y, beta=0.0, overwrite=True):
        assert x.dtype == np.float64 and y.dtype == np.float64 and x.flags.c_contiguous and y.flags.c_contiguous
        if lib().csxb_spmv_host(self._h, alpha, x.ctypes.data, beta, y.ctypes.data, int(overwrite)) != 0:
            raise EngineError(lib().csxb_last_error().decode())
        return y

    def prepare_transpose(self):
        if lib().csxb_transpose_prepare(self._h) != 0:
            raise EngineError(lib().csxb_last_error().decode())
        return self

    def spmv_t(self, alpha, x, y, beta=0.0, overwrite=True, stream=None):
        import torch
        assert x.is_cuda and y.is_cuda and x.dtype == torch.float64 and y.dtype == torch.float64
        assert x.numel() == self.nrows and y.numel() == self.ncols and x.is_contiguous() and y.is_contiguous()
        s = torch.cuda.current_stream().cuda_stream if stream is None else stream
        if lib().csxb_spmv_t(self._h, alpha, x.data_ptr(), beta, y.data_ptr(), int(overwrite), s) != 0:
            raise EngineError(lib().csxb_last_error().decode())
        return y

    def spmv_t_host(self, alpha, x, y, beta=0.0, overwrite=True):
        assert x.dtype == np.float64 and y.dtype == np.float64 and x.flags.c_contiguous and y.flags.c_contiguous
        assert x.size == self.nrows and y.size == self.ncols
        if lib().csxb_spmv_t_host(self._h, alpha, x.ctypes.data, beta, y.ctypes.data, int(overwrite)) != 0:
            raise EngineError(lib().csxb_last_error().decode())
        return y

    def transpose_info(self):
        keys = ["col_lo", "col_hi", "device_bytes", "alg_bytes", "launches", "heavy_cols", "segments", "build_us"]
        return {k: lib().csxb_transpose_info(self._h, i) for i, k in enumerate(keys)}

    def decode_coords_t(self):
        n = sum(lib().csxb_part_info(self._h, p, 0) for p in range(self.nparts))
        r = np.empty(n, np.int32)
        c = np.empty(n, np.int32)
        if lib().csxb_decode_coords_t(self._h, r.ctypes.data, c.ctypes.data) != 0:
            raise EngineError(lib().csxb_last_error().decode())
        return r, c

    def save(self, path):
        if lib().csxb_save(self._h, path.encode()) != 0:
            raise EngineError(lib().csxb_last_error().decode())

    @classmethod
    def load(cls, path):
        err = C.create_string_buffer(1024)
        h = lib().csxb_load(path.encode(), err, 1024)
        if not h:
            raise EngineError(err.value.decode())
        return cls(h)

    def get_entry(self, row, col):
        v = C.c_double()
        rc = lib().csxb_get_entry(self._h, row, col, C.byref(v))
        if rc < 0:
            raise EngineError(lib().csxb_last_error().decode())
        return v.value if rc == 0 else None

    def set_entry(self, row, col, value):
        rc = lib().csxb_set_entry(self._h, row, col, value)
        if rc < 0:
            raise EngineError(lib().csxb_last_error().decode())
        return rc == 0

    def decode_coords(self, p):
        n = lib().csxb_part_info(self._h, p, 0)
        r = np.empty(n, np.int32)
        c = np.empty(n, np.int32)
        if lib().csxb_decode_coords(self._h, p, r.ctypes.data, c.ctypes.data) != 0:
            raise EngineError(lib().csxb_last_error().decode())
        return r, c

    def close(self):
        if self._h:
            lib().csxb_destroy(self._h)
            self._h = None

    def __del__(self):
        try:
            self.close()
        except Exception:
            pass


def _vec_ptr(v, n):
    if isinstance(v, np.ndarray):
        assert v.dtype == np.float64 and v.flags.c_contiguous and v.size == n
        return v.ctypes.data
    assert v.is_contiguous() and v.numel() == n
    return v.data_ptr()


class DeviceGroup(object):

    def __init__(self, matrix, devices, free_host=False):
        dev = np.ascontiguousarray(devices, dtype=np.int32)
        err = C.create_string_buffer(1024)
        self.nrows, self.ncols = matrix.nrows, matrix.ncols
        self._h = lib().csxb_group_create(matrix._h, dev.ctypes.data, len(dev), int(free_host), err, 1024)
        if not self._h:
            raise EngineError(err.value.decode())
        matrix._h = None
        self.size = lib().csxb_group_size(self._h)

    def member_info(self, i, what):
        return lib().csxb_info(lib().csxb_group_member(self._h, i), what)

    def spmv(self, alpha, x, y, beta=0.0, overwrite=True):
        if lib().csxb_group_spmv(self._h, alpha, _vec_ptr(x, self.ncols), beta, _vec_ptr(y, self.nrows), int(overwrite)) != 0:
            raise EngineError(lib().csxb_last_error().decode())
        return y

    def spmv_t(self, alpha, x, y, beta=0.0, overwrite=True):
        if lib().csxb_group_spmv_t(self._h, alpha, _vec_ptr(x, self.nrows), beta, _vec_ptr(y, self.ncols), int(overwrite)) != 0:
            raise EngineError(lib().csxb_last_error().decode())
        return y

    def save(self, path):
        if lib().csxb_group_save(self._h, path.encode()) != 0:
            raise EngineError(lib().csxb_last_error().decode())

    def get_entry(self, row, col):
        v = C.c_double()
        rc = lib().csxb_group_get_entry(self._h, row, col, C.byref(v))
        if rc < 0:
            raise EngineError(lib().csxb_last_error().decode())
        return v.value if rc == 0 else None

    def set_entry(self, row, col, value):
        rc = lib().csxb_group_set_entry(self._h, row, col, value)
        if rc < 0:
            raise EngineError(lib().csxb_last_error().decode())
        return rc == 0

    def close(self):
        if self._h:
# ... 147 lines not shown
```

Baseline: 1378.

## Split f64 values into byte planes and drop shared exponent head for uniform units

After: 1324, median of 6. -3.9%, worse.

```diff
diff --git a/__graft_entry__.py b/__graft_entry__.py
--- a/__graft_entry__.py
+++ b/__graft_entry__.py
@@ -18,6 +18,7 @@
                 subprocess.check_call([sys.executable, ref])
     subprocess.check_call(["make", "-s", "-C", os.path.join(ROOT, "tests", "emul")], stderr=subprocess.DEVNULL)
     subprocess.check_call(["make", "-s", "-C", os.path.join(ROOT, "tests", "emul"), "-f", "trans.mk"], stderr=subprocess.DEVNULL)
+    subprocess.check_call(["make", "-s", "-C", os.path.join(ROOT, "tests", "emul"), "-f", "planes.mk"], stderr=subprocess.DEVNULL)
     import sparsex_b200
     sparsex_b200.lib()
     if os.path.isdir("/root/reference/src/examples"):
diff --git a/include/csx_b200.h b/include/csx_b200.h
--- a/include/csx_b200.h
+++ b/include/csx_b200.h
@@ -24,7 +24,8 @@
        CSXB_NPARTS_TOTAL = 5, CSXB_PART_LO = 6, CSXB_FULL_COLIND = 7,
        CSXB_SYM_HALO_LO = 8, CSXB_SYM_HALO_HI = 9,
        CSXB_HOST_CAP = 10, CSXB_HOST_CALLS = 11,
-       CSXB_DEVICE = 12  };
+       CSXB_DEVICE = 12 ,
+       CSXB_PACKED_VALUES = 13, CSXB_UNPACKED_VALUES = 14 };
 int64_t csxb_info(const csxb_matrix_t *m, int what);
 
 enum { CSXB_P_NNZ = 0, CSXB_P_NROWS = 1, CSXB_P_NCOLS = 2, CSXB_P_ROW_START = 3, CSXB_P_CTL_SIZE = 4,
diff --git a/sparsex_b200/csrc/engine.cu b/sparsex_b200/csrc/engine.cu
--- a/sparsex_b200/csrc/engine.cu
+++ b/sparsex_b200/csrc/engine.cu
@@ -273,6 +273,7 @@
   double *d_values = nullptr;
   double *d_x = nullptr, *d_y = nullptr;
   int64_t covered_rows_end = 0;
+  int64_t nnz_local = 0;
   int64_t sym_halo_lo = 0, sym_halo_hi = 0;
   struct Slab {
     int part; int64_t tile0, tile1;
@@ -395,6 +396,8 @@
     case CSXB_HOST_CAP: return (int64_t)m->host_cap;
     case CSXB_HOST_CALLS: return m->host_calls;
     case CSXB_DEVICE: return m->uploaded ? m->device : -1;
+    case CSXB_PACKED_VALUES: return m->uploaded && m->layout.planes ? (int64_t)m->layout.packed_values : 0;
+    case CSXB_UNPACKED_VALUES: return m->uploaded && m->layout.planes ? m->nnz_local - (int64_t)m->layout.packed_values : 0;
   }
   return -1;
 }
@@ -483,6 +486,46 @@
   if (extra_zero) CUDA_TRY(cudaMemset((char *)p + n * sizeof(T), 0, extra_zero * sizeof(T)));
   *dst = (T *)p;
   return 0;
+}
+
+constexpr size_t PLANE_PIECE = size_t(1) << 20;
+static int values_to_device(csxb_matrix *m, uint64_t i0, size_t n, const double *src) {
+  if (!m->layout.planes) { CUDA_TRY(cudaMemcpy(m->d_values + i0, src, n * 8, cudaMemcpyHostToDevice)); return 0; }
+  const uint64_t N = m->layout.total_values;
+  char *base = (char *)m->d_values;
+  std::vector<uint32_t> lo(std::min(n, PLANE_PIECE));
+  std::vector<uint16_t> mid(lo.size()), hi(lo.size());
+  for (size_t o = 0; o < n; o += PLANE_PIECE) {
+    const size_t k = std::min(PLANE_PIECE, n - o);
+    split_values(src + o, k, lo.data(), mid.data(), hi.data());
+    CUDA_TRY(cudaMemcpy(base + 4 * (i0 + o), lo.data(), k * 4, cudaMemcpyHostToDevice));
+    CUDA_TRY(cudaMemcpy(base + plane_mid(N, i0 + o), mid.data(), k * 2, cudaMemcpyHostToDevice));
+    CUDA_TRY(cudaMemcpy(base + plane_hi(N, i0 + o), hi.data(), k * 2, cudaMemcpyHostToDevice));
+  }
+  return 0;
+}
+static int values_from_device(csxb_matrix *m, uint64_t i0, size_t n, double *dst) {
+  if (!m->layout.planes) { CUDA_TRY(cudaMemcpy(dst, m->d_values + i0, n * 8, cudaMemcpyDeviceToHost)); return 0; }
+  const uint64_t N = m->layout.total_values;
+  const char *base = (const char *)m->d_values;
+  std::vector<uint32_t> lo(std::min(n, PLANE_PIECE));
+  std::vector<uint16_t> mid(lo.size()), hi(lo.size());
+  for (size_t o = 0; o < n; o += PLANE_PIECE) {
+    const size_t k = std::min(PLANE_PIECE, n - o);
+    CUDA_TRY(cudaMemcpy(lo.data(), base + 4 * (i0 + o), k * 4, cudaMemcpyDeviceToHost));
+    CUDA_TRY(cudaMemcpy(mid.data(), base + plane_mid(N, i0 + o), k * 2, cudaMemcpyDeviceToHost));
+    CUDA_TRY(cudaMemcpy(hi.data(), base + plane_hi(N, i0 + o), k * 2, cudaMemcpyDeviceToHost));
+    join_values(lo.data(), mid.data(), hi.data(), k, dst + o);
+  }
+  return 0;
+}
+static void set_planes(const csxb_matrix *m, PartDev &P) {
+  if (!m->layout.planes) return;
+  const uint64_t N = m->layout.total_values;
+  const char *base = (const char *)m->d_values;
+  P.vlo = (const uint32_t *)base;
+  P.vmid = (const uint16_t *)(base + plane_mid(N, 0));
+  P.vhi = (const uint16_t *)(base + plane_hi(N, 0));
 }
 
 static void build_slabs(csxb_matrix *m) {
@@ -570,10 +613,11 @@
     CsxPartition &hp = pl.is_halo ? no_part : H.parts[i];
     PartDev &P = m->pdev[i];
     memset(&P, 0, sizeof(P));
-    if (hp.nnz) CUDA_TRY(cudaMemcpy(m->d_values + pl.val_base, hp.values.data(), (size_t)hp.nnz * 8, cudaMemcpyHostToDevice));
+    if (hp.nnz && values_to_device(m, pl.val_base, (size_t)hp.nnz, hp.values.data())) return -1;
     if (!hp.ctl.empty()) CUDA_TRY(cudaMemcpy((uint8_t *)dc + pl.ctl_base, hp.ctl.data(), hp.ctl.size(), cudaMemcpyHostToDevice));
     P.ctl = (const uint8_t *)dc + pl.ctl_base;
     P.values = m->d_values;
+    set_planes(m, P);
     P.ctl_end = (const uint8_t *)dc + std::max<uint64_t>(L.total_ctl, 16);
     P.values_end = m->d_values + std::max<uint64_t>(L.total_values, 1);
     uint32_t *tx = nullptr; XDesc *xd = nullptr;
@@ -633,7 +677,9 @@
   }
   m->sym_halo_lo = L.halo_lo; m->sym_halo_hi = L.halo_hi;
   if (!H.symmetric) build_slabs(m);
-  m->bytes[CSXB_B_VALUES] = nnz_stored * 8;
+  m->nnz_local = nnz_stored;
+  const int64_t value_bytes = nnz_stored * 8 - (L.planes ? 2 * (int64_t)L.packed_values : 0);
+  m->bytes[CSXB_B_VALUES] = value_bytes;
   m->bytes[CSXB_B_CTL] = ctl_bytes;
   m->bytes[CSXB_B_TABLES] = tables;
   int64_t cmin = H.ncols, cmax = -1;
@@ -642,7 +688,7 @@
   if (H.symmetric) xcols = H.ncols;
   m->bytes[CSXB_B_X] = xcols * 8;
   m->bytes[CSXB_B_Y] = rows_owned * 8;
-  m->bytes[CSXB_B_TOTAL] = nnz_stored * 8 + ctl_bytes + tables + xcols * 8 + rows_owned * 8;
+  m->bytes[CSXB_B_TOTAL] = value_bytes + ctl_bytes + tables + xcols * 8 + rows_owned * 8;
   m->bytes[CSXB_B_LAUNCHES] = launches;
   m->uploaded = true;
   return 0;
@@ -939,6 +985,8 @@
   std::unique_ptr<TransState> T(new TransState);
   std::string e = build_transpose_layout(m->host, m->layout, T->lay);
   if (!e.empty()) return fail("transposed layout: " + e);
+  if (m->layout.planes && (!T->lay.part.xd_diag1_only || !T->lay.part.bt.empty() || T->lay.images || !T->lay.hent.empty()))
+    return fail("transposed layout: value planes need stride-1 diagonal units only");
   CUDA_TRY(cudaSetDevice(m->device));
   const TransLayout &TL = T->lay;
   const PartLayout &pl = TL.part;
@@ -975,6 +1023,7 @@
     launches += 2;
   }
   P.values = m->d_values; P.tile_xoff = tx; P.xdesc = (const uint4 *)xd; P.ktab = kt;
+  set_planes(m, P);
   P.nrows = pl.nrows; P.row_start = pl.row_start; P.rpt = pl.rpt;
   P.values_end = m->d_values + std::max<uint64_t>(m->layout.total_values, 1);
   T->dev_bytes = (int64_t)TL.ktab.size() * 8 + (int64_t)pl.tile_xoff.size() * 4 + (int64_t)pl.xdesc.size() * 16 +
@@ -1333,7 +1382,7 @@
     if (!m->uploaded) return fail("partition values are neither on the host nor on a device");
     CUDA_TRY(cudaSetDevice(m->device));
     p.values.resize((size_t)p.nnz);
-    CUDA_TRY(cudaMemcpy(p.values.data(), m->d_values + m->layout.parts[i].val_base, (size_t)p.nnz * 8, cudaMemcpyDeviceToHost));
+    if (values_from_device(m, m->layout.parts[i].val_base, (size_t)p.nnz, p.values.data())) return -1;
   }
   std::string e = save_matrix(H, path);
   return e.empty() ? 0 : fail(e);
@@ -1394,8 +1443,7 @@
   if ((int64_t)p.values.size() == p.nnz) { *value = p.values[(size_t)idx]; return 0; }
   if (!m->uploaded) return fail("partition values are neither on the host nor on a device");
   CUDA_TRY(cudaSetDevice(m->device));
-  CUDA_TRY(cudaMemcpy(value, m->d_values + m->layout.parts[part].val_base + idx, 8, cudaMemcpyDeviceToHost));
-  return 0;
+  return values_from_device(m, m->layout.parts[part].val_base + idx, 1, value);
 }
 
 int csxb_set_entry(csxb_matrix_t *m, int64_t row, int64_t col, double value) {
@@ -1407,8 +1455,27 @@
   else if ((int64_t)p.values.size() == p.nnz) p.values[(size_t)idx] = value;
   if (m->uploaded) {
     CUDA_TRY(cudaSetDevice(m->device));
-    double *dst = diag ? const_cast<double *>(m->pdev[part].dvalues) + idx : m->d_values + m->layout.parts[part].val_base + idx;
-    CUDA_TRY(cudaMemcpy(dst, &value, 8, cudaMemcpyHostToDevice));
+    if (diag) {
+      CUDA_TRY(cudaMemcpy(const_cast<double *>(m->pdev[part].dvalues) + idx, &value, 8, cudaMemcpyHostToDevice));
+      return 0;
+    }
+    const uint32_t vi = (uint32_t)(m->layout.parts[part].val_base + idx);
+    if (values_to_device(m, vi, 1, &value)) return -1;
+    if (m->layout.planes) {
+      uint32_t size = 0;
+      for (size_t j : unpack_unit(m->layout.parts[part], vi, row, value_head(value), &size))
+        CUDA_TRY(cudaMemcpy((char *)m->pdev[part].xdesc + 16 * j + 12, &m->layout.parts[part].xdesc[j].meta, 4, cudaMemcpyHostToDevice));
+      m->layout.packed_values -= size;
+      m->bytes[CSXB_B_VALUES] += 2 * (int64_t)size;
+      m->bytes[CSXB_B_TOTAL] += 2 * (int64_t)size;
+      if (m->trans) {
+        TransState &T = *m->trans;
+        uint32_t tsize = 0;
+        for (size_t j : unpack_unit(T.lay.part, vi, col, value_head(value), &tsize))
+          CUDA_TRY(cudaMemcpy((char *)T.P.xdesc + 16 * j + 12, &T.lay.part.xdesc[j].meta, 4, cudaMemcpyHostToDevice));
+        T.alg_bytes += 2 * (int64_t)tsize;
+      }
+    }
   }
   return 0;
 }
diff --git a/sparsex_b200/csrc/gather_kernel.cuh b/sparsex_b200/csrc/gather_kernel.cuh
--- a/sparsex_b200/csrc/gather_kernel.cuh
+++ b/sparsex_b200/csrc/gather_kernel.cuh
@@ -1,5 +1,16 @@
 #pragma once
 #include "part_dev.cuh"
+
+#ifdef CSXB_EMUL
+#include <cmath>
+inline double __fma_rn(double a, double b, double c) { return std::fma(a, b, c); }
+inline double __hiloint2double(int hi, int lo) {
+  const uint64_t b = (uint64_t)(uint32_t)hi << 32 | (uint32_t)lo;
+  double v;
+  memcpy(&v, &b, 8);
+  return v;
+}
+#endif
 
 template <bool SYM, class Op>
 __device__ __forceinline__ void gather_desc(const uint4 d, const KindEntry *__restrict__ ktab, int myrow, Op &op) {
@@ -187,8 +198,94 @@
         if (KSET == KSET_DIAG1) {
           const int t0 = grow0 + lane - (int)d.y;
           const uint32_t size = (d.w >> 16) & 0xff;
+          const double *__restrict__ xp = x + ((long long)(int)d.z + t0);
+          if (P.vlo && (d.w & XD_PACKED)) {
+            const uint32_t head = d.w << 16;
+            const uint32_t *__restrict__ lp = P.vlo + ((long long)d.x + t0);
+            const uint16_t *__restrict__ mp = P.vmid + ((long long)d.x + t0);
+#ifndef CSXB_EMUL
+            if ((VAR == 3 || VAR == 1) && RPT == 4) {
+              uint32_t l0, l1, l2, l3, m0, m1, m2, m3;
+              double x0, x1, x2, x3;
+              if (VAR == 3)
+                asm volatile(
+                    "{\n\t.reg .pred p0, p1, p2, p3;\n\t"
+                    "setp.lt.u32 p0, %12, %16;\n\tsetp.lt.u32 p1, %13, %16;\n\tsetp.lt.u32 p2, %14, %16;\n\tsetp.lt.u32 p3, %15, %16;\n\t"
+                    "mov.b32 %0, 0;\n\tmov.b32 %1, 0;\n\tmov.b32 %2, 0;\n\tmov.b32 %3, 0;\n\t"
+                    "mov.b32 %4, 0;\n\tmov.b32 %5, 0;\n\tmov.b32 %6, 0;\n\tmov.b32 %7, 0;\n\t"
+                    "mov.f64 %8, 0d0000000000000000;\n\tmov.f64 %9, 0d0000000000000000;\n\t"
+                    "mov.f64 %10, 0d0000000000000000;\n\tmov.f64 %11, 0d0000000000000000;\n\t"
+                    "@p0 ld.global.nc.L1::no_allocate.L2::cache_hint.u32 %0, [%17], %21;\n\t"
+                    "@p0 ld.global.nc.L1::no_allocate.L2::cache_hint.u16 %4, [%18], %21;\n\t"
+                    "@p0 ld.global.nc.L2::cache_hint.f64 %8, [%19], %22;\n\t"
+                    "@p1 ld.global.nc.L1::no_allocate.L2::cache_hint.u32 %1, [%17+128], %21;\n\t"
+                    "@p1 ld.global.nc.L1::no_allocate.L2::cache_hint.u16 %5, [%18+64], %21;\n\t"
+                    "@p1 ld.global.nc.L2::cache_hint.f64 %9, [%19+256], %22;\n\t"
+                    "@p2 ld.global.nc.L1::no_allocate.L2::cache_hint.u32 %2, [%17+256], %21;\n\t"
+                    "@p2 ld.global.nc.L1::no_allocate.L2::cache_hint.u16 %6, [%18+128], %21;\n\t"
+                    "@p2 ld.global.nc.L2::cache_hint.f64 %10, [%19+512], %22;\n\t"
+                    "@p3 ld.global.nc.L1::no_allocate.L2::cache_hint.u32 %3, [%17+384], %21;\n\t"
+                    "@p3 ld.global.nc.L1::no_allocate.L2::cache_hint.u16 %7, [%18+192], %21;\n\t"
+                    "@p3 ld.global.nc.L2::cache_hint.f64 %11, [%19+768], %22;\n\t"
+                    "@p0 or.b32 %4, %4, %20;\n\t@p1 or.b32 %5, %5, %20;\n\t@p2 or.b32 %6, %6, %20;\n\t@p3 or.b32 %7, %7, %20;\n\t}"
+                    : "=r"(l0), "=r"(l1), "=r"(l2), "=r"(l3), "=r"(m0), "=r"(m1), "=r"(m2), "=r"(m3),
+                      "=d"(x0), "=d"(x1), "=d"(x2), "=d"(x3)
+                    : "r"((uint32_t)t0), "r"((uint32_t)(t0 + 32)), "r"((uint32_t)(t0 + 64)), "r"((uint32_t)(t0 + 96)), "r"(size),
+                      "l"(lp), "l"(mp), "l"(xp), "r"(head), "l"(pol_stream), "l"(pol_keep));
+              else
+                asm volatile(
+                    "{\n\t.reg .pred p0, p1, p2, p3;\n\t"
+                    "setp.lt.u32 p0, %12, %16;\n\tsetp.lt.u32 p1, %13, %16;\n\tsetp.lt.u32 p2, %14, %16;\n\tsetp.lt.u32 p3, %15, %16;\n\t"
+                    "mov.b32 %0, 0;\n\tmov.b32 %1, 0;\n\tmov.b32 %2, 0;\n\tmov.b32 %3, 0;\n\t"
+                    "mov.b32 %4, 0;\n\tmov.b32 %5, 0;\n\tmov.b32 %6, 0;\n\tmov.b32 %7, 0;\n\t"
+                    "mov.f64 %8, 0d0000000000000000;\n\tmov.f64 %9, 0d0000000000000000;\n\t"
+                    "mov.f64 %10, 0d0000000000000000;\n\tmov.f64 %11, 0d0000000000000000;\n\t"
+                    "@p0 ld.global.nc.u32 %0, [%17];\n\t@p0 ld.global.nc.u16 %4, [%18];\n\t@p0 ld.global.nc.f64 %8, [%19];\n\t"
+                    "@p1 ld.global.nc.u32 %1, [%17+128];\n\t@p1 ld.global.nc.u16 %5, [%18+64];\n\t@p1 ld.global.nc.f64 %9, [%19+256];\n\t"
+                    "@p2 ld.global.nc.u32 %2, [%17+256];\n\t@p2 ld.global.nc.u16 %6, [%18+128];\n\t@p2 ld.global.nc.f64 %10, [%19+512];\n\t"
+                    "@p3 ld.global.nc.u32 %3, [%17+384];\n\t@p3 ld.global.nc.u16 %7, [%18+192];\n\t@p3 ld.global.nc.f64 %11, [%19+768];\n\t"
+                    "@p0 or.b32 %4, %4, %20;\n\t@p1 or.b32 %5, %5, %20;\n\t@p2 or.b32 %6, %6, %20;\n\t@p3 or.b32 %7, %7, %20;\n\t}"
+                    : "=r"(l0), "=r"(l1), "=r"(l2), "=r"(l3), "=r"(m0), "=r"(m1), "=r"(m2), "=r"(m3),
+                      "=d"(x0), "=d"(x1), "=d"(x2), "=d"(x3)
+                    : "r"((uint32_t)t0), "r"((uint32_t)(t0 + 32)), "r"((uint32_t)(t0 + 64)), "r"((uint32_t)(t0 + 96)), "r"(size),
+                      "l"(lp), "l"(mp), "l"(xp), "r"(head));
+              acc[0] = __fma_rn(__hiloint2double((int)m0, (int)l0), x0, acc[0]);
+              acc[1 % RPT] = __fma_rn(__hiloint2double((int)m1, (int)l1), x1, acc[1 % RPT]);
+              acc[2 % RPT] = __fma_rn(__hiloint2double((int)m2, (int)l2), x2, acc[2 % RPT]);
+              acc[3 % RPT] = __fma_rn(__hiloint2double((int)m3, (int)l3), x3, acc[3 % RPT]);
+              continue;
+            }
+#endif
+            double v[RPT], xv[RPT];
+#pragma unroll
+            for (int k = 0; k < RPT; k++) {
+              v[k] = 0.0; xv[k] = 0.0;
+              if ((uint32_t)(t0 + k * 32) < size) {
+                v[k] = __hiloint2double((int)(head | __ldg(mp + k * 32)), (int)__ldg(lp + k * 32));
+                xv[k] = ldx<COH>(xp + k * 32);
+              }
+            }
+#pragma unroll
+            for (int k = 0; k < RPT; k++) acc[k] = __fma_rn(v[k], xv[k], acc[k]);
+            continue;
+          }
+          if (P.vhi) {
+            const long long i0 = (long long)d.x + t0;
+            double v[RPT], xv[RPT];
+#pragma unroll
+            for (int k = 0; k < RPT; k++) {
+              v[k] = 0.0; xv[k] = 0.0;
+              if ((uint32_t)(t0 + k * 32) < size) {
+                const long long i = i0 + k * 32;
+                v[k] = __hiloint2double((int)((uint32_t)__ldg(P.vhi + i) << 16 | __ldg(P.vmid + i)), (int)__ldg(P.vlo + i));
+                xv[k] = ldx<COH>(xp + k * 32);
+              }
+            }
+#pragma unroll
+            for (int k = 0; k < RPT; k++) acc[k] = __fma_rn(v[k], xv[k], acc[k]);
+            continue;
+          }
           const double *__restrict__ vp = values + ((long long)d.x + t0);
-          const double *__restrict__ xp = x + ((long long)(int)d.z + t0);
 #ifndef CSXB_EMUL
           if (VAR == 3 && RPT == 4) {
             double v0, v1, v2, v3, x0, x1, x2, x3;
@@ -206,7 +303,8 @@
                 : "=d"(v0), "=d"(v1), "=d"(v2), "=d"(v3), "=d"(x0), "=d"(x1), "=d"(x2), "=d"(x3)
                 : "r"((uint32_t)t0), "r"((uint32_t)(t0 + 32)), "r"((uint32_t)(t0 + 64)), "r"((uint32_t)(t0 + 96)), "r"(size),
                   "l"(vp), "l"(xp), "l"(pol_stream), "l"(pol_keep));
-            acc[0] += v0 * x0; acc[1 % RPT] += v1 * x1; acc[2 % RPT] += v2 * x2; acc[3 % RPT] += v3 * x3;
+            acc[0] = __fma_rn(v0, x0, acc[0]); acc[1 % RPT] = __fma_rn(v1, x1, acc[1 % RPT]);
+            acc[2 % RPT] = __fma_rn(v2, x2, acc[2 % RPT]); acc[3 % RPT] = __fma_rn(v3, x3, acc[3 % RPT]);
             continue;
           }
           if (VAR == 1 && RPT == 4) {
@@ -225,7 +323,8 @@
                 : "=d"(v0), "=d"(v1), "=d"(v2), "=d"(v3), "=d"(x0), "=d"(x1), "=d"(x2), "=d"(x3)
                 : "r"((uint32_t)t0), "r"((uint32_t)(t0 + 32)), "r"((uint32_t)(t0 + 64)), "r"((uint32_t)(t0 + 96)), "r"(size),
                   "l"(vp), "l"(xp));
-            acc[0] += v0 * x0; acc[1 % RPT] += v1 * x1; acc[2 % RPT] += v2 * x2; acc[3 % RPT] += v3 * x3;
+            acc[0] = __fma_rn(v0, x0, acc[0]); acc[1 % RPT] = __fma_rn(v1, x1, acc[1 % RPT]);
+            acc[2 % RPT] = __fma_rn(v2, x2, acc[2 % RPT]); acc[3 % RPT] = __fma_rn(v3, x3, acc[3 % RPT]);
             continue;
           }
 #endif
@@ -236,7 +335,7 @@
             if ((uint32_t)(t0 + k * 32) < size) { v[k] = __ldg(vp + k * 32); xv[k] = ldx<COH>(xp + k * 32); }
           }
 #pragma unroll
-          for (int k = 0; k < RPT; k++) acc[k] += v[k] * xv[k];
+          for (int k = 0; k < RPT; k++) acc[k] = __fma_rn(v[k], xv[k], acc[k]);
           continue;
         }
         if (!(SYM && (d.w & XD_TRANSPOSED) && (((d.w >> 24) & 0xf) == K_VERT || ((d.w >> 24) & 0xf) >= K_BROW))) {
diff --git a/sparsex_b200/csrc/gpu_layout.cpp b/sparsex_b200/csrc/gpu_layout.cpp
--- a/sparsex_b200/csrc/gpu_layout.cpp
+++ b/sparsex_b200/csrc/gpu_layout.cpp
@@ -2,6 +2,7 @@
 #include <climits>
 #include <cstring>
 #include <map>
+#include <unordered_map>
 
 #include "gpu_layout.hpp"
 
@@ -274,6 +275,70 @@
   return true;
 }
 
+void mark_planes(const CsxMatrix &m, DeviceLayout &out) {
+  if (m.symmetric || out.parts.empty()) return;
+  for (const PartLayout &L : out.parts)
+    if (L.is_halo || !L.xd_diag1_only || !L.bt.empty() || L.has_flat) return;
+  out.planes = true;
+  for (size_t pi = 0; pi < out.parts.size(); pi++) {
+    PartLayout &L = out.parts[pi];
+    const std::vector<double> &vals = m.parts[pi].values;
+    if ((int64_t)vals.size() != m.parts[pi].nnz) continue;
+    for (int64_t t = 0; t < L.ntiles; t++)
+      for (uint32_t j = L.tile_xoff[t]; j < L.tile_xoff[t + 1]; j++) {
+        XDesc &d = L.xdesc[j];
+        const uint32_t size = (d.meta >> 16) & 0xff;
+        const double *v = vals.data() + (d.voff - L.val_base);
+        const uint16_t head = value_head(v[0]);
+        uint32_t k = 1;
+        while (k < size && value_head(v[k]) == head) k++;
+        if (k < size) continue;
+        d.meta = (d.meta & ~(XD_PACKED | 0xffffu)) | XD_PACKED | head;
+        if (((int64_t)d.row - L.row_start) / L.tile_rows() == t) out.packed_values += size;
+      }
+  }
+}
+
+}
+
+void split_values(const double *v, size_t n, uint32_t *lo, uint16_t *mid, uint16_t *hi) {
+  for (size_t i = 0; i < n; i++) {
+    uint64_t b;
+    memcpy(&b, v + i, 8);
+    lo[i] = (uint32_t)b; mid[i] = (uint16_t)(b >> 32); hi[i] = (uint16_t)(b >> 48);
+  }
+}
+void join_values(const uint32_t *lo, const uint16_t *mid, const uint16_t *hi, size_t n, double *v) {
+  for (size_t i = 0; i < n; i++) {
+    const uint64_t b = (uint64_t)hi[i] << 48 | (uint64_t)mid[i] << 32 | lo[i];
+    memcpy(v + i, &b, 8);
+  }
+}
+
+std::vector<size_t> unpack_unit(PartLayout &L, uint32_t vi, int64_t grow, uint16_t head, uint32_t *size_out) {
+  std::vector<size_t> changed;
+  *size_out = 0;
+  const int64_t tr = L.tile_rows(), t = (grow - L.row_start) / tr;
+  if (t < 0 || t >= L.ntiles) return changed;
+  uint32_t voff = 0, size = 0;
+  int64_t lo = 0, hi = -1;
+  for (uint32_t j = L.tile_xoff[t]; j < L.tile_xoff[t + 1] && !size; j++) {
+    const XDesc &d = L.xdesc[j];
+    const uint32_t s = (d.meta >> 16) & 0xff;
+    if (vi < d.voff || vi - d.voff >= s) continue;
+    if (!(d.meta & XD_PACKED) || (uint16_t)d.meta == head) return changed;
+    voff = d.voff; size = s;
+    lo = (d.row - L.row_start) / tr; hi = (d.row + (int64_t)s - 1 - L.row_start) / tr;
+  }
+  for (int64_t u = std::max<int64_t>(lo, 0); u <= std::min<int64_t>(hi, L.ntiles - 1); u++)
+    for (size_t j = L.tile_xoff[u]; j < L.tile_xoff[u + 1]; j++) {
+      XDesc &d = L.xdesc[j];
+      if (d.voff != voff || !(d.meta & XD_PACKED)) continue;
+      d.meta &= ~XD_PACKED;
+      changed.push_back(j);
+    }
+  *size_out = size;
+  return changed;
 }
 
 std::string build_layout(const CsxMatrix &m, DeviceLayout &out) {
@@ -676,7 +741,9 @@
   for (const BlockTmp &b : blocks)
     if (!list_rows(b.d, b.cmin, b.cmax, pend)) return "symmetric update targets a row that is not on this device";
   if (!btents.empty()) sort_block_tables(out, out.parts, btents);
-  return distribute_descs(out.parts, pend);
+  std::string err = distribute_descs(out.parts, pend);
+  if (err.empty()) mark_planes(m, out);
+  return err;
 }
 
 std::string build_transpose_layout(const CsxMatrix &m, const DeviceLayout &fwd, TransLayout &out) {
@@ -785,7 +852,7 @@
       v += size;
     }
     if (v != cp.nnz) return "ctl stream covers " + std::to_string(v) + " values, expected " + std::to_string(cp.nnz);
-    const bool as_desc = singles.size() <= (size_t)(cp.nnz / 256);
+    const bool as_desc = fwd.planes || singles.size() <= (size_t)(cp.nnz / 256);
     for (const Single &sg : singles) {
       if (sg.col < clo || sg.col > chi) return "unit leaves the column range";
       if (as_desc) {
@@ -845,6 +912,16 @@
     break;
   }
   if (out.hseg.empty()) out.hseg.push_back(0);
+  if (fwd.planes) {
+    std::unordered_map<uint32_t, uint32_t> packed;
+    for (const PartLayout &F : fwd.parts)
+      for (const XDesc &d : F.xdesc)
+        if (d.meta & XD_PACKED) packed[d.voff] = d.meta & (XD_PACKED | 0xffffu);
+    for (XDesc &d : L.xdesc) {
+      auto it = packed.find(d.voff);
+      if (it != packed.end()) d.meta = (d.meta & ~0xffffu) | it->second;
+    }
+  }
   out.part = std::move(L);
   return "";
 }
diff --git a/sparsex_b200/csrc/gpu_layout.hpp b/sparsex_b200/csrc/gpu_layout.hpp
--- a/sparsex_b200/csrc/gpu_layout.hpp
+++ b/sparsex_b200/csrc/gpu_layout.hpp
@@ -1,5 +1,6 @@
 #pragma once
 #include <cstdint>
+#include <cstring>
 #include <string>
 #include <vector>
 
@@ -31,6 +32,7 @@
 };
 constexpr uint32_t XD_TRANSPOSED = 1u << 28;
 constexpr uint32_t XD_DELTA1 = 1u << 29;
+constexpr uint32_t XD_PACKED = 1u << 30;
 
 struct KindEntry { uint32_t kind_align; uint32_t delta; };
 struct IdEntry { uint32_t kind_align; uint32_t delta; uint32_t sl; uint32_t recip; };
@@ -103,9 +105,18 @@
   int bc_align = 0, bc_rows = 0, br_align = 0, br_cols = 0;
   int br_img_cols = 0;
   int64_t halo_lo = 0, halo_hi = 0;
+  bool planes = false;
+  uint64_t packed_values = 0;
 };
 
 std::string build_layout(const CsxMatrix &m, DeviceLayout &out);
+
+void split_values(const double *v, size_t n, uint32_t *lo, uint16_t *mid, uint16_t *hi);
+void join_values(const uint32_t *lo, const uint16_t *mid, const uint16_t *hi, size_t n, double *v);
+inline uint16_t value_head(double v) { uint64_t b; memcpy(&b, &v, 8); return (uint16_t)(b >> 48); }
+inline uint64_t plane_mid(uint64_t N, uint64_t i) { return 4 * N + 2 * i; }
+inline uint64_t plane_hi(uint64_t N, uint64_t i) { return 6 * N + 2 * i; }
+std::vector<size_t> unpack_unit(PartLayout &L, uint32_t vi, int64_t grow, uint16_t head, uint32_t *size);
 
 constexpr int T_HEAVY_MIN = 128;
 constexpr int T_SEG_LEN = 256;
diff --git a/sparsex_b200/csrc/part_dev.cuh b/sparsex_b200/csrc/part_dev.cuh
--- a/sparsex_b200/csrc/part_dev.cuh
+++ b/sparsex_b200/csrc/part_dev.cuh
@@ -13,6 +13,8 @@
 struct PartDev {
   const uint8_t *ctl;
   const double *values;
+  const uint32_t *vlo;
+  const uint16_t *vmid, *vhi;
   const uint32_t *tile_xoff;
   const uint4 *xdesc;
   const KindEntry *ktab;
diff --git a/sparsex_b200/engine.py b/sparsex_b200/engine.py
--- a/sparsex_b200/engine.py
+++ b/sparsex_b200/engine.py
@@ -229,6 +229,10 @@
         self.uploaded = True
         return self
 
+    def value_planes(self):
+        L = lib()
+        return L.csxb_info(self._h, 13), L.csxb_info(self._h, 14)
+
     def traffic(self):
         L = lib()
         keys = ["values", "ctl", "tables", "x", "y", "total", "launches"]
```
